# BartvLaatum/GreenLight-Gym2

Hardware: AMD Instinct MI355X
Metric: TomatoEnv env-steps/sec (higher is better)
Workload: dtype f32

## Files before the change

greenlight-gym2_amd/csrc/glgym.hip:

```cpp
#include <hip/hip_runtime.h>

#include <cmath>
#include <cstdio>
#include <cstdlib>
#include <cstring>
#include <new>
#include <string>
#include <vector>

#include "glgym.h"
#include "gl_model.hpp"
#include "gl_model_quad.hpp"
#include "gl_reward.hpp"
#include "glgym_bdf.h"
#include "glgym_rng.h"
#include "glgym_plan.h"

using namespace glm;

namespace {

thread_local std::string g_err;

#define HIPCHK(expr)                                                                                   \
    do {                                                                                               \
        hipError_t e_ = (expr);                                                                        \
        if (e_ != hipSuccess) {                                                                        \
            g_err = std::string(#expr) + ": " + hipGetErrorString(e_);                                 \
            return GLGYM_EHIP;                                                                         \
        }                                                                                              \
    } while (0)

constexpr int WAVE = 64;

#include "gl_default_const.inc"
static_assert(sizeof(ModelConst<float>) == sizeof(kDefaultConstF32_image), "regenerate gl_default_const.inc");
static_assert(sizeof(ModelConst<double>) == sizeof(kDefaultConstF64_image), "regenerate gl_default_const.inc");
template <class T> struct DefaultConst;
template <> struct DefaultConst<float> {
    static constexpr ModelConst<float> value = __builtin_bit_cast(ModelConst<float>, kDefaultConstF32_bits);
};
template <> struct DefaultConst<double> {
    static constexpr ModelConst<double> value = __builtin_bit_cast(ModelConst<double>, kDefaultConstF64_bits);
};
__constant__ const ModelConst<float> g_default_f32 = __builtin_bit_cast(ModelConst<float>, kDefaultConstF32_bits);
__constant__ const ModelConst<double> g_default_f64 = __builtin_bit_cast(ModelConst<double>, kDefaultConstF64_bits);
template <class T> __device__ __forceinline__ const ModelConst<T>& device_default();
template <> __device__ __forceinline__ const ModelConst<float>& device_default<float>() { return g_default_f32; }
template <> __device__ __forceinline__ const ModelConst<double>& device_default<double>() { return g_default_f64; }

template <class T> struct RewardConst : RewardConstBase<T> {};

template <class T> struct StepArgsT {
    int B, ld;
    T* x; T* u;
    const float* action; const T* control;
    const T* weather; int weather_rows;
    const int* w_off; int* timestep;
    const T* crop_p;
    int N;
    T* reward; T* info; unsigned char* done; float* metrics; int* step_flags;
    T dt; int n_sub;
    T gasR, tCanMin;
    int nd;
    float du, u_min[NU], u_max[NU];
    int verify;
    int pipe;
    int window;
};

template <class T> __device__ __forceinline__ T wave_sum(T v)
{
#pragma unroll
    for (int o = 32; o > 0; o >>= 1) v += __shfl_xor(v, o, WAVE);
    return v;
}

#ifndef GL_STEP_WAVES_PER_SIMD
#define GL_STEP_WAVES_PER_SIMD 1
#endif
#ifndef GL_RK4_WIN_F32
#define GL_RK4_WIN_F32 4
#endif
#ifndef GL_RK4_WIN_F64
#define GL_RK4_WIN_F64 4
#endif
template <class T> struct RK4_WINDOW { static constexpr int value = sizeof(T) == 4 ? GL_RK4_WIN_F32 : GL_RK4_WIN_F64; };
constexpr int gl_order(int sch) { return sch == 0 ? 4 : sch == 1 ? 2 : sch == 2 ? 3 : 5; }
template <class T, int SCH> struct SchemeWin { static constexpr int value = SCH == 0 ? RK4_WINDOW<T>::value : SCH == 1 ? 4 : SCH == 2 ? 3 : 2; };

template <class T, bool PER_ENV_CROP, bool DEFAULT_P, bool PIPE = false, int SCH = 0, int OCC = GL_STEP_WAVES_PER_SIMD>
__global__ __launch_bounds__(WAVE, OCC) void step_kernel(StepArgsT<T> a, ModelConst<T> m_arg, RewardConst<T> rw)
{
    const ModelConst<T>& m = DEFAULT_P ? device_default<T>() : m_arg;
    constexpr bool WBUF = OCC == 2;
    constexpr int WSTRIDE = (2 * NX + GL_N_SLOW) | 1;
    __shared__ float sh_w[WBUF ? WAVE * WSTRIDE : WAVE * NU];
    float* sh_act = sh_w;
    const int lane = threadIdx.x;
    const int b0 = blockIdx.x * WAVE;
    const int b = b0 + lane;
    const bool live = b < a.B;
    const int bb = live ? b : a.B - 1;

    T u[NU];
    if (a.action) {
        const int n_tile = min(WAVE, a.B - b0) * NU;
        for (int i = lane; i < n_tile; i += WAVE) sh_act[i] = a.action[(size_t)b0 * NU + i];
        __syncthreads();
        const int l = live ? lane : (a.B - 1 - b0);
#pragma unroll
        for (int j = 0; j < NU; ++j) {
            const float inc = sh_act[l * NU + j] * a.du;
            const T v = a.u[(size_t)j * a.ld + bb] + T(inc);
            u[j] = Math<T>::min(Math<T>::max(v, T(a.u_min[j])), T(a.u_max[j]));
        }
    } else {
#pragma unroll
        for (int j = 0; j < NU; ++j) u[j] = a.control[(size_t)j * a.ld + bb];
    }

    T x0[NX];
#pragma unroll
    for (int i = 0; i < NX; ++i) x0[i] = a.x[(size_t)i * a.ld + bb];
    const int ts = a.timestep[bb];
    int row = a.w_off[bb] + ts;
    row = row < 0 ? 0 : (row >= a.weather_rows ? a.weather_rows - 1 : row);
    T d[7];
#pragma unroll
    for (int j = 0; j < 7; ++j) d[j] = a.weather[(size_t)row * a.nd + j];

    CropConst<T> crLocal;
    if (PER_ENV_CROP) {
        T pc[NCROP];
#pragma unroll
        for (int i = 0; i < NCROP; ++i) pc[i] = a.crop_p[(size_t)i * a.ld + bb];
        make_crop_const<T, T>(pc, a.gasR, a.tCanMin, crLocal);
    }
    const CropConst<T>& cr = PER_ENV_CROP ? crLocal : m.crop;
    StepCoef<T> s_reg;
    precompute(u, d, m, cr, s_reg);
    if (PIPE) {
        const T tPipe = a.weather[(size_t)row * a.nd + 10], swOff = a.weather[(size_t)row * a.nd + 12];
        s_reg.pipeTrack = ((tPipe < T(1)) || (swOff > T(0))) ? T(0) : T(1);
        s_reg.tPipeSet = tPipe;
    }
    const StepCoef<T>& s = s_reg;
    if (live) {
#pragma unroll
        for (int j = 0; j < NU; ++j) a.u[(size_t)j * a.ld + b] = u[j];
    }
    T del_reg[WBUF ? 1 : NX];
    T* wb = reinterpret_cast<T*>(sh_w) + (size_t)lane * WSTRIDE;
    T* del = WBUF ? wb + NX + GL_N_SLOW : del_reg;
    if (WBUF) {
        __syncthreads();
#pragma unroll
        for (int i = 0; i < NX; ++i) wb[i] = x0[i];
        wb[5] = x0[3] - x0[5]; wb[7] = x0[2] - x0[7]; wb[20] = x0[2] - x0[20]; wb[6] = x0[5] - x0[6];
    }
    bool bad;
    int extra_steps, first_flags = 0;
    const int retries = rk4_delta_guarded<T, PIPE, gl_order(SCH), SchemeWin<T, SCH>::value, WBUF>(x0, s, m, cr, a.dt, a.n_sub, del, &bad, &extra_steps, a.verify != 0, &first_flags, a.window, wb);
    const T uBoil = a.u[(size_t)0 * a.ld + bb], uCo2 = a.u[(size_t)1 * a.ld + bb], uLamp = a.u[(size_t)4 * a.ld + bb];
    if (WBUF) {
#pragma unroll
        for (int i = 0; i < NX; ++i) x0[i] = a.x[(size_t)i * a.ld + bb];
    }

    T x1[NX];
#pragma unroll
    for (int i = 0; i < NX; ++i) x1[i] = bad ? x0[i] : x0[i] + del[i];
    {
        const double per_step = (double)a.dt / 86400.0;
        double t_start = (double)x0[NX - 1] - (double)ts * per_step;
        if (fabs(t_start) < 5e-4) t_start = 0.0;
        if (!bad) x1[NX - 1] = T(t_start + ((double)ts + 1.0) * per_step);
    }

    const T co2ppm = rw.kPpm * (x1[2] + T(273.15)) * x1[0];
    const T rh = Math<T>::min(Math<T>::max(T(100) * x1[15] / sat_vp_exact(x1[2]), T(0)), T(100));
    const T o3[3] = {co2ppm, x1[2], rh};
    T viol[3], pen = T(0);
#pragma unroll
    for (int i = 0; i < 3; ++i) {
        viol[i] = Math<T>::max(rw.lo[i] - o3[i], T(0)) + Math<T>::max(o3[i] - rw.hi[i], T(0));
        pen += viol[i] * rw.invMaxViol[i];
    }
    const T heat = uBoil * rw.heatK, elec = uLamp * rw.elecK, co2c = uCo2 * rw.co2K;
    const T varc = heat + co2c + elec;
    const T gains = (bad ? T(0) : del[25]) * rw.gainK;
    const T profit = gains - varc;
    const T reward = (profit - rw.minProfit) * rw.invRange - pen;
    const bool term = bad || (ts >= a.N);

    if (live) {
#pragma unroll
        for (int i = 0; i < NX; ++i) a.x[(size_t)i * a.ld + b] = x1[i];
        a.timestep[b] = ts + 1;
        a.reward[b] = reward;
        a.done[b] = term ? 1 : 0;
        if (a.step_flags) a.step_flags[b] = first_flags | (retries << 8) | (bad ? GLGYM_SF_FAILED : 0) | (min(extra_steps, 32767) << 16);
        if (a.info) {
            const T inf[GLGYM_NINFO] = {profit, gains, varc, rw.fixedCosts, co2c, heat, elec, viol[1], viol[0], viol[2], T(0)};
#pragma unroll
            for (int i = 0; i < GLGYM_NINFO; ++i) a.info[(size_t)i * a.ld + b] = inf[i];
        }
    }
    if (a.metrics) {
        const float w = live ? 1.f : 0.f;
        float mv[GLGYM_NMETRIC] = {w * (float)reward, w * (float)profit, (live && term) ? 1.f : 0.f,
                                   (live && bad) ? 1.f : 0.f, w * (float)viol[0], w * (float)viol[1],
                                   w * (float)viol[2], w, w * (float)retries, w * (float)extra_steps,
                                   (live && (first_flags & SC_FLAG_ERR)) ? 1.f : 0.f, (live && (first_flags & SC_FLAG_BRANCH)) ? 1.f : 0.f,
                                   (live && (first_flags & (SC_FLAG_CAP | SC_FLAG_NONFINITE))) ? 1.f : 0.f,
                                   (live && (first_flags & 16)) ? 1.f : 0.f};
        float* mrep = a.metrics + (size_t)(blockIdx.x % GLGYM_METRIC_REPLICAS) * GLGYM_METRIC_STRIDE;
#pragma unroll
        for (int i = 0; i < GLGYM_NMETRIC; ++i) {
            const float sum = wave_sum(mv[i]);
            if (lane == 0) atomicAdd(mrep + i, sum);
        }
    }
}


template <class T, bool DEFAULT_P, int SCH = 0, bool PIPE = false, bool CROP = false, bool PAIR = false>
__global__ __launch_bounds__(WAVE) void step_kernel_quad(StepArgsT<T> a, ModelConst<T> m_arg, RewardConst<T> rw)
{
    static_assert(!(PAIR && CROP), "the two-rungs ladder is instantiated for shared crop constants only");
    constexpr bool LDSM = sizeof(T) == 8 && !DEFAULT_P;
    __shared__ ModelConst<T> sh_m[1];
    if (LDSM) {
        static_assert(sizeof(ModelConst<T>) % 4 == 0, "word copy");
        const unsigned* src = reinterpret_cast<const unsigned*>(&m_arg);
        unsigned* dst = reinterpret_cast<unsigned*>(&sh_m[0]);
        for (int i = threadIdx.x; i < (int)(sizeof(ModelConst<T>) / 4); i += WAVE) dst[i] = src[i];
        __syncthreads();
    }
    const ModelConst<T>& m = LDSM ? sh_m[0] : DEFAULT_P ? device_default<T>() : m_arg;
    const int gl = blockIdx.x * WAVE + threadIdx.x, role = gl & 3;
    const int b = PAIR ? gl >> 3 : gl >> 2, half = PAIR ? (gl >> 2) & 1 : 0;
    const bool live = b < a.B;
    const int bb = live ? b : a.B - 1;
    T u[NU];
    if (a.action) {
#pragma unroll
        for (int j = 0; j < NU; ++j) {
            const float inc = a.action[(size_t)bb * NU + j] * a.du;
            const T v = a.u[(size_t)j * a.ld + bb] + T(inc);
            u[j] = Math<T>::min(Math<T>::max(v, T(a.u_min[j])), T(a.u_max[j]));
        }
    } else {
#pragma unroll
        for (int j = 0; j < NU; ++j) u[j] = a.control[(size_t)j * a.ld + bb];
    }
    const int ts = a.timestep[bb];
    int row = a.w_off[bb] + ts;
    row = row < 0 ? 0 : (row >= a.weather_rows ? a.weather_rows - 1 : row);
    T d[7];
#pragma unroll
    for (int j = 0; j < 7; ++j) d[j] = a.weather[(size_t)row * a.nd + j];
    constexpr bool LDSQ = sizeof(T) == 8;
    struct SRec { StepCoef<T> s; T pad[(sizeof(StepCoef<T>) / sizeof(T)) % 2 == 0 ? 1 : 2]; };
    struct KRec { LaneK<T> k; T pad[(sizeof(LaneK<T>) / sizeof(T)) % 2 == 0 ? 1 : 2]; };
    struct CRec { CropConst<T> c; T pad[(sizeof(CropConst<T>) / sizeof(T)) % 2 == 0 ? 1 : 2]; };
    __shared__ SRec sh_s[LDSQ ? WAVE / 4 : 1];
    __shared__ KRec sh_k[LDSQ ? WAVE : 1];
    __shared__ CRec sh_c[(LDSQ && CROP) ? WAVE / 4 : 1];
    StepCoef<T> s_reg;
    LaneK<T> k_reg;
    CropConst<T> cr_reg;
    if (CROP && (!LDSQ || role == 0)) {
        T pc[NCROP];
#pragma unroll
        for (int i = 0; i < NCROP; ++i) pc[i] = a.crop_p[(size_t)i * a.ld + bb];
        make_crop_const<T, T>(pc, a.gasR, a.tCanMin, cr_reg);
    }
    if (!LDSQ || role == 0) {
        precompute(u, d, m, CROP ? cr_reg : m.crop, s_reg);
        if (PIPE && a.pipe) {
            const T tPipe = a.weather[(size_t)row * a.nd + 10], swOff = a.weather[(size_t)row * a.nd + 12];
            s_reg.pipeTrack = ((tPipe < T(1)) || (swOff > T(0))) ? T(0) : T(1);
            s_reg.tPipeSet = tPipe;
            s_reg.pipeOde = T(1);
        }
    }
    if (LDSQ) {
        if (role == 0) { sh_s[threadIdx.x >> 2].s = s_reg; if (CROP) sh_c[threadIdx.x >> 2].c = cr_reg; }
        __syncthreads();
    }
    const CropConst<T>& cr = !CROP ? m.crop : LDSQ ? sh_c[threadIdx.x >> 2].c : cr_reg;
    const StepCoef<T>& s = LDSQ ? sh_s[threadIdx.x >> 2].s : s_reg;
    LaneK<T>& K = LDSQ ? sh_k[threadIdx.x].k : k_reg;
    auto X = [&](int i) { return a.x[(size_t)i * a.ld + bb]; };
    QVec<T> x0, z0, del;
#pragma unroll
    for (int i = 0; i < 6; ++i) x0.sh[i] = X(role == 0 ? gq_sh_ix(i) : role == 1 ? gq_sh_ix(i) : role == 2 ? gq_sh_ix(i) : gq_sh_ix(i));
    x0.p = gq_mk<T>(X(role == 0 ? 4 : role == 1 ? 8 : role == 2 ? 7 : 5), X(role == 0 ? 9 : role == 1 ? 17 : role == 2 ? 20 : 6));
#pragma unroll
    for (int j = 0; j < 4; ++j) {
        const int ix = role == 0 ? gq_other_ix(0, j) : role == 1 ? gq_other_ix(1, j) : role == 2 ? gq_other_ix(2, j) : gq_other_ix(3, j < 2 ? j : 1);
        x0.o[j] = X(ix);
    }
    z0 = x0;
    z0.p = gq_mk<T>(role == 2 ? x0.sh[2] - x0.p.x : role == 3 ? x0.sh[3] - x0.p.x : x0.p.x,
                    role == 2 ? x0.sh[2] - x0.p.y : role == 3 ? x0.p.x - x0.p.y : x0.p.y);
    if (live && role == 0 && half == 0) {
#pragma unroll
        for (int j = 0; j < NU; ++j) a.u[(size_t)j * a.ld + b] = u[j];
    }
    bool bad;
    int extra_steps = 0, first_flags = 0, retries = 0, mine = 1;
    constexpr bool HVU = sizeof(T) == 8 || DEFAULT_P;
    if (PAIR) {
        int bad_i;
        rk4_delta_guarded_quad_pair<T, gl_order(SCH), SchemeWin<T, SCH>::value, LDSQ, PIPE, false, true, HVU>(role, half, z0, s, K, m, cr, a.dt, a.n_sub, del, &bad_i, &mine,
                                                                                                         a.window, &retries, &extra_steps, &first_flags);
        asm volatile("" : "+v"(bad_i), "+v"(mine));
        bad = bad_i != 0;
    } else {
        retries = rk4_delta_guarded_quad<T, gl_order(SCH), SchemeWin<T, SCH>::value, LDSQ, PIPE, LDSQ && CROP, HVU>(role, z0, s, K, m, cr, a.dt, a.n_sub, del, &bad,
                                                                                                    &extra_steps, a.verify != 0, &first_flags, a.window);
    }
    P2<T> dP;
    gq_phys_pair<T>(role, del, dP);
    asm volatile("" ::: "memory");
    int gl2 = blockIdx.x * WAVE + threadIdx.x;
    asm volatile("" : "+v"(gl2));
    const int role2 = gl2 & 3, b2 = PAIR ? gl2 >> 3 : gl2 >> 2;
    const bool live2 = b2 < a.B && mine != 0;
    const int bb2 = (b2 < a.B) ? b2 : a.B - 1;
    const int ts2 = a.timestep[bb2];
    auto X2 = [&](int i) { return a.x[(size_t)i * a.ld + bb2]; };
#pragma unroll
    for (int i = 0; i < 6; ++i) x0.sh[i] = X2(gq_sh_ix(i));
    x0.p = gq_mk<T>(X2(role2 == 0 ? 4 : role2 == 1 ? 8 : role2 == 2 ? 7 : 5), X2(role2 == 0 ? 9 : role2 == 1 ? 17 : role2 == 2 ? 20 : 6));
#pragma unroll
    for (int j = 0; j < 4; ++j) {
        const int ix = role2 == 0 ? gq_other_ix(0, j) : role2 == 1 ? gq_other_ix(1, j) : role2 == 2 ? gq_other_ix(2, j) : gq_other_ix(3, j < 2 ? j : 1);
        x0.o[j] = X2(ix);
    }
#pragma unroll
    for (int j = 0; j < NU; ++j) u[j] = a.u[(size_t)j * a.ld + bb2];
    QVec<T> x1;
    x1.p = gq_mk<T>(bad ? x0.p.x : x0.p.x + dP.x, bad ? x0.p.y : x0.p.y + dP.y);
#pragma unroll
    for (int i = 0; i < 6; ++i) x1.sh[i] = bad ? x0.sh[i] : x0.sh[i] + del.sh[i];
#pragma unroll
    for (int j = 0; j < 4; ++j) x1.o[j] = bad ? x0.o[j] : x0.o[j] + del.o[j];
    if (role2 == 3) {
        const double per_step = (double)a.dt / 86400.0;
        double t_start = (double)x0.o[1] - (double)ts2 * per_step;
        if (fabs(t_start) < 5e-4) t_start = 0.0;
        if (!bad) x1.o[1] = T(t_start + ((double)ts2 + 1.0) * per_step);
    }
    const T dFruit = gq_bcast<2>(del.o[3]);
    const T co2ppm = rw.kPpm * (x1.sh[2] + T(273.15)) * x1.sh[0];
    const T rh = Math<T>::min(Math<T>::max(T(100) * x1.sh[4] / sat_vp_exact(x1.sh[2]), T(0)), T(100));
    const T o3[3] = {co2ppm, x1.sh[2], rh};
    T viol[3], pen = T(0);
#pragma unroll
    for (int i = 0; i < 3; ++i) {
        viol[i] = Math<T>::max(rw.lo[i] - o3[i], T(0)) + Math<T>::max(o3[i] - rw.hi[i], T(0));
        pen += viol[i] * rw.invMaxViol[i];
    }
    const T heat = u[0] * rw.heatK, elec = u[4] * rw.elecK, co2c = u[1] * rw.co2K;
    const T varc = heat + co2c + elec;
    const T gains = (bad ? T(0) : dFruit) * rw.gainK;
    const T profit = gains - varc;
    const T reward = (profit - rw.minProfit) * rw.invRange - pen;
    const bool term = bad || (ts2 >= a.N);
    if (live2) {
        auto W = [&](int i, T v) { a.x[(size_t)i * a.ld + b2] = v; };
        W(role2 == 0 ? 4 : role2 == 1 ? 8 : role2 == 2 ? 7 : 5, x1.p.x);
        W(role2 == 0 ? 9 : role2 == 1 ? 17 : role2 == 2 ? 20 : 6, x1.p.y);
#pragma unroll
        for (int j = 0; j < 4; ++j)
            if (role2 != 3 || j < 2) W(role2 == 0 ? gq_other_ix(0, j) : role2 == 1 ? gq_other_ix(1, j) : role2 == 2 ? gq_other_ix(2, j) : gq_other_ix(3, j < 2 ? j : 1), x1.o[j]);
        if (role2 == 0) {
#pragma unroll
            for (int i = 0; i < 6; ++i) W(gq_sh_ix(i), x1.sh[i]);
            a.timestep[b2] = ts2 + 1;
            a.reward[b2] = reward;
            a.done[b2] = term ? 1 : 0;
            if (a.step_flags) a.step_flags[b2] = first_flags | (retries << 8) | (bad ? GLGYM_SF_FAILED : 0) | (min(extra_steps, 32767) << 16);
            if (a.info) {
                const T inf[GLGYM_NINFO] = {profit, gains, varc, rw.fixedCosts, co2c, heat, elec, viol[1], viol[0], viol[2], T(0)};
#pragma unroll
                for (int i = 0; i < GLGYM_NINFO; ++i) a.info[(size_t)i * a.ld + b2] = inf[i];
            }
        }
    }
    if (a.metrics) {
        const bool cnt = live2 && role2 == 0;
        const float w = cnt ? 1.f : 0.f;
        float mv[GLGYM_NMETRIC] = {w * (float)reward, w * (float)profit, (cnt && term) ? 1.f : 0.f,
                                   (cnt && bad) ? 1.f : 0.f, w * (float)viol[0], w * (float)viol[1],
                                   w * (float)viol[2], w, w * (float)retries, w * (float)extra_steps,
                                   (cnt && (first_flags & SC_FLAG_ERR)) ? 1.f : 0.f, (cnt && (first_flags & SC_FLAG_BRANCH)) ? 1.f : 0.f,
                                   (cnt && (first_flags & (SC_FLAG_CAP | SC_FLAG_NONFINITE))) ? 1.f : 0.f,
                                   (cnt && (first_flags & 16)) ? 1.f : 0.f};
        float* mrep = a.metrics + (size_t)(blockIdx.x % GLGYM_METRIC_REPLICAS) * GLGYM_METRIC_STRIDE;
#pragma unroll
        for (int i = 0; i < GLGYM_NMETRIC; ++i) {
            const float sum = wave_sum(mv[i]);
            if (threadIdx.x == 0) atomicAdd(mrep + i, sum);
        }
    }
}

template <class T, int SCH, bool PIPE, bool CROP, bool PAIR = false>
__global__ __launch_bounds__(WAVE) void evalf_kernel_quad(const double* x, const double* u, const double* d, const double* crop, int B, T dt,
                                                          int n_sub, T gasR, T tCanMin, ModelConst<T> m_arg, double* x_next, int nd,
                                                          int* n_failed, int verify, int pipe, int window)
{
    constexpr bool LDSM = sizeof(T) == 8;
    __shared__ ModelConst<T> sh_m[1];
    if (LDSM) {
        const unsigned* src = reinterpret_cast<const unsigned*>(&m_arg);
        unsigned* dst = reinterpret_cast<unsigned*>(&sh_m[0]);
        for (int i = threadIdx.x; i < (int)(sizeof(ModelConst<T>) / 4); i += WAVE) dst[i] = src[i];
        __syncthreads();
    }
    const ModelConst<T>& m = LDSM ? sh_m[0] : m_arg;
    const int gl = blockIdx.x * WAVE + threadIdx.x, role = gl & 3, b = PAIR ? gl >> 3 : gl >> 2, half = PAIR ? (gl >> 2) & 1 : 0;
    const bool live = b < B;
    const int bb = live ? b : B - 1;
    T uu[NU], dd[7];
#pragma unroll
    for (int i = 0; i < NU; ++i) uu[i] = T(u[(size_t)bb * NU + i]);
#pragma unroll
    for (int i = 0; i < 7; ++i) dd[i] = T(d[(size_t)bb * nd + i]);
    constexpr bool LDSQ = sizeof(T) == 8;
    struct SRec { StepCoef<T> s; T pad[(sizeof(StepCoef<T>) / sizeof(T)) % 2 == 0 ? 1 : 2]; };
    struct KRec { LaneK<T> k; T pad[(sizeof(LaneK<T>) / sizeof(T)) % 2 == 0 ? 1 : 2]; };
    struct CRec { CropConst<T> c; T pad[(sizeof(CropConst<T>) / sizeof(T)) % 2 == 0 ? 1 : 2]; };
    __shared__ SRec sh_s[LDSQ ? WAVE / 4 : 1];
    __shared__ KRec sh_k[LDSQ ? WAVE : 1];
    __shared__ CRec sh_c[(LDSQ && CROP) ? WAVE / 4 : 1];
    StepCoef<T> s_reg;
    LaneK<T> k_reg;
    CropConst<T> cr_reg;
    if (CROP && (!LDSQ || role == 0)) {
        T pc[NCROP];
#pragma unroll
        for (int i = 0; i < NCROP; ++i) pc[i] = T(crop[(size_t)bb * NCROP + i]);
        make_crop_const<T, T>(pc, gasR, tCanMin, cr_reg);
    }
    if (!LDSQ || role == 0) {
        precompute(uu, dd, m, CROP ? cr_reg : m.crop, s_reg);
        if (PIPE && pipe) {
            const T tPipe = T(d[(size_t)bb * nd + 10]), swOff = T(d[(size_t)bb * nd + 12]);
            s_reg.pipeTrack = ((tPipe < T(1)) || (swOff > T(0))) ? T(0) : T(1);
            s_reg.tPipeSet = tPipe;
            s_reg.pipeOde = T(1);
        }
    }
    if (LDSQ) {
        if (role == 0) { sh_s[threadIdx.x >> 2].s = s_reg; if (CROP) sh_c[threadIdx.x >> 2].c = cr_reg; }
        __syncthreads();
    }
    const CropConst<T>& cr = !CROP ? m.crop : LDSQ ? sh_c[threadIdx.x >> 2].c : cr_reg;
    const StepCoef<T>& s = LDSQ ? sh_s[threadIdx.x >> 2].s : s_reg;
    LaneK<T>& K = LDSQ ? sh_k[threadIdx.x].k : k_reg;
    auto X = [&](int i) { return T(x[(size_t)bb * NX + i]); };
    QVec<T> x0, z0, del;
#pragma unroll
    for (int i = 0; i < 6; ++i) x0.sh[i] = X(gq_sh_ix(i));
    x0.p = gq_mk<T>(X(role == 0 ? 4 : role == 1 ? 8 : role == 2 ? 7 : 5), X(role == 0 ? 9 : role == 1 ? 17 : role == 2 ? 20 : 6));
#pragma unroll
    for (int j = 0; j < 4; ++j)
        x0.o[j] = X(role == 0 ? gq_other_ix(0, j) : role == 1 ? gq_other_ix(1, j) : role == 2 ? gq_other_ix(2, j) : gq_other_ix(3, j < 2 ? j : 1));
    z0 = x0;
    z0.p = gq_mk<T>(role == 2 ? x0.sh[2] - x0.p.x : role == 3 ? x0.sh[3] - x0.p.x : x0.p.x,
                    role == 2 ? x0.sh[2] - x0.p.y : role == 3 ? x0.p.x - x0.p.y : x0.p.y);
    bool bad;
    constexpr bool HVU = sizeof(T) == 8;
    int mine = 1;
    if (PAIR) {
        int bad_i;
        rk4_delta_guarded_quad_pair<T, gl_order(SCH), SchemeWin<T, SCH>::value, LDSQ, PIPE, LDSQ && CROP, false, HVU>(role, half, z0, s, K, m, cr, dt, n_sub, del, &bad_i, &mine, window);
        asm volatile("" : "+v"(bad_i), "+v"(mine));
        bad = bad_i != 0;
    } else {
        int extra_steps, first_flags = 0;
        rk4_delta_guarded_quad<T, gl_order(SCH), SchemeWin<T, SCH>::value, LDSQ, PIPE, LDSQ && CROP, HVU>(role, z0, s, K, m, cr, dt, n_sub, del, &bad, &extra_steps, verify != 0,
                                                                                      &first_flags, window);
    }
    P2<T> dP;
    gq_phys_pair<T>(role, del, dP);
    asm volatile("" ::: "memory");
    int gl2 = blockIdx.x * WAVE + threadIdx.x;
    asm volatile("" : "+v"(gl2));
    const int role2 = gl2 & 3, b2 = PAIR ? gl2 >> 3 : gl2 >> 2;
    if (b2 < B && mine != 0) {
        const double nan = __builtin_nan("");
        auto X2 = [&](int i) { return x[(size_t)b2 * NX + i]; };
        auto W = [&](int i, T dv) { x_next[(size_t)b2 * NX + i] = bad ? nan : X2(i) + (double)dv; };
        W(role2 == 0 ? 4 : role2 == 1 ? 8 : role2 == 2 ? 7 : 5, dP.x);
        W(role2 == 0 ? 9 : role2 == 1 ? 17 : role2 == 2 ? 20 : 6, dP.y);
#pragma unroll
        for (int j = 0; j < 4; ++j)
            if (role2 != 3 || j < 2)
                W(role2 == 0 ? gq_other_ix(0, j) : role2 == 1 ? gq_other_ix(1, j) : role2 == 2 ? gq_other_ix(2, j) : gq_other_ix(3, j < 2 ? j : 1), del.o[j]);
        if (role2 == 0) {
#pragma unroll
            for (int i = 0; i < 6; ++i) W(gq_sh_ix(i), del.sh[i]);
            if (bad) atomicAdd(n_failed, 1);
        }
    }
}

template <class T, bool PER_ENV_CROP, bool PIPE>
__global__ __launch_bounds__(WAVE) void rhs_kernel(const double* x, const double* u, const double* d, const double* crop, int B, T gasR,
                                                   T tCanMin, ModelConst<T> m, double* dx, int nd)
{
    const int b = blockIdx.x * WAVE + threadIdx.x;
    if (b >= B) return;
    T x0[NX], uu[NU], dd[7];
    for (int i = 0; i < NX; ++i) x0[i] = T(x[(size_t)b * NX + i]);
    for (int i = 0; i < NU; ++i) uu[i] = T(u[(size_t)b * NU + i]);
    for (int i = 0; i < 7; ++i) dd[i] = T(d[(size_t)b * nd + i]);
    CropConst<T> crLocal;
    if (PER_ENV_CROP) {
        T pc[NCROP];
        for (int i = 0; i < NCROP; ++i) pc[i] = T(crop[(size_t)b * NCROP + i]);
        make_crop_const<T, T>(pc, gasR, tCanMin, crLocal);
    }
    const CropConst<T>& cr = PER_ENV_CROP ? crLocal : m.crop;
    StepCoef<T> s;
    precompute(uu, dd, m, cr, s);
    if (PIPE) {
        const T tPipe = T(d[(size_t)b * nd + 10]), swOff = T(d[(size_t)b * nd + 12]);
        s.pipeTrack = ((tPipe < T(1)) || (swOff > T(0))) ? T(0) : T(1);
        s.tPipeSet = tPipe;
    }
    T k[NX];
    rhs<T, true, PIPE>(x0, s, m, cr, k);
    for (int i = 0; i < NX; ++i) dx[(size_t)b * NX + i] = (double)k[i];
}

template <class T, bool PER_ENV_CROP, bool PIPE = false, int SCH = 0>
__global__ __launch_bounds__(WAVE) void evalf_kernel(const double* x, const double* u, const double* d,
                                                     const double* crop, int B, T dt, int n_sub, T gasR, T tCanMin,
                                                     ModelConst<T> m, double* x_next, int rhs_only, int nd,
                                                     int* n_failed, int verify, int window)
{
    const int b = blockIdx.x * WAVE + threadIdx.x;
    if (b >= B) return;
    T x0[NX], uu[NU], dd[7];
    for (int i = 0; i < NX; ++i) x0[i] = T(x[(size_t)b * NX + i]);
    for (int i = 0; i < NU; ++i) uu[i] = T(u[(size_t)b * NU + i]);
    for (int i = 0; i < 7; ++i) dd[i] = T(d[(size_t)b * nd + i]);
    CropConst<T> crLocal;
    if (PER_ENV_CROP) {
        T pc[NCROP];
        for (int i = 0; i < NCROP; ++i) pc[i] = T(crop[(size_t)b * NCROP + i]);
        make_crop_const<T, T>(pc, gasR, tCanMin, crLocal);
    }
    const CropConst<T>& cr = PER_ENV_CROP ? crLocal : m.crop;
    StepCoef<T> s;
    precompute(uu, dd, m, cr, s);
    if (PIPE) {
        const T tPipe = T(d[(size_t)b * nd + 10]), swOff = T(d[(size_t)b * nd + 12]);
        s.pipeTrack = ((tPipe < T(1)) || (swOff > T(0))) ? T(0) : T(1);
        s.tPipeSet = tPipe;
    }
    if (rhs_only) {
        T k[NX];
        rhs<T, true, PIPE>(x0, s, m, cr, k);
        for (int i = 0; i < NX; ++i) x_next[(size_t)b * NX + i] = (double)k[i];
        return;
    }
    T del[NX];
    bool failed;
    rk4_delta_guarded<T, PIPE, gl_order(SCH), SchemeWin<T, SCH>::value>(x0, s, m, cr, dt, n_sub, del, &failed, nullptr, verify != 0, nullptr, window);
    for (int i = 0; i < NX; ++i)
        x_next[(size_t)b * NX + i] = failed ? __builtin_nan("") : (double)x0[i] + (double)del[i];
    if (failed) atomicAdd(n_failed, 1);
}

template <class T> struct ObsArgsT {
    int B, ld;
    const T* x; const T* u; const T* weather; int weather_rows;
    const int* w_off; const int* timestep; const float* start_day;
    int Np; float* obs; double doy_inc, hod_inc;
    const unsigned char* mask; float* term_obs;
    int nd;
    int moff[6], dim;
};

#ifndef GL_OBS_ROWS
#define GL_OBS_ROWS 16
#endif
constexpr int OBS_ROWS = GL_OBS_ROWS, OBS_NCORE = 23, OBS_MAX_NP = 128;
template <class T> __global__ __launch_bounds__(256) void obs_kernel(ObsArgsT<T> a)
{
    constexpr int ROWS = OBS_ROWS, NCORE = OBS_NCORE;
    extern __shared__ float4 span4[];
    float* span = reinterpret_cast<float*>(span4);
    const int tid = threadIdx.x;
    const int dim = a.dim;
    const float kPpm = (float)(8.3144598 / (101325.0 * 44.01e-3));
    for (int rb = blockIdx.x * ROWS; rb < a.B; rb += gridDim.x * ROWS) {
        const int nrows = min(ROWS, a.B - rb);
        if (a.mask) {
            int any = 0;
            for (int r = 0; r < nrows; ++r) any |= a.mask[rb + r];
            if (!any) continue;
        }
        int base_r[ROWS];
#pragma unroll
        for (int r = 0; r < ROWS; ++r) {
            const int b = rb + (r < nrows ? r : 0);
            const int ts = a.timestep[b];
            base_r[r] = a.w_off[b] + (ts > 0 ? ts - 1 : 0);
        }
        for (int e = tid; e < ROWS * NCORE; e += 256) {
            const int r = e / NCORE, j = e - r * NCORE;
            const int b = rb + (r < nrows ? r : 0);
            const int ts = a.timestep[b];
            const int k = ts > 0 ? ts - 1 : 0;
            int base = 0;
#pragma unroll
            for (int rr = 0; rr < ROWS; ++rr) base = (rr == r) ? base_r[rr] : base;
            base = base >= a.weather_rows ? a.weather_rows - 1 : (base < 0 ? 0 : base);
            const T* wrow = a.weather + (size_t)base * a.nd;
            const int xi = j == 0 ? 0 : j == 1 ? 2 : j == 2 ? 15 : j == 3 ? 9 : j == 4 ? 21 : j == 5 ? 25 : 26;
            const T* p1 = j < 7 ? a.x + (size_t)xi * a.ld + b
                                : (j < 13 ? a.u + (size_t)(j - 7) * a.ld + b : wrow + (j < 18 ? j - 13 : 0));
            const T* p2 = j < 13 ? a.x + (size_t)2 * a.ld + b : wrow + 1;
            const float prim = (float)*p1, aux = (float)*p2, sday = a.start_day[b];
            const float sat = 610.78f * __builtin_amdgcn_exp2f(1.44269504f * 17.2694f * aux * __builtin_amdgcn_rcpf(aux + 238.3f));
            const float rh = fminf(fmaxf(100.0f * prim * __builtin_amdgcn_rcpf(sat), 0.0f), 100.0f);
            const float ppm = kPpm * (aux + 273.15f) * prim;
            const int c = j - 18;
            const double rev = (c <= 2) ? ((double)sday + (double)ts * a.doy_inc) * (1.0 / 365.0)
                                        : (double)ts * a.hod_inc * (1.0 / 24.0);
            const float fr = (float)(rev - floor(rev));
            const float clk = (c == 1 || c == 3) ? __builtin_amdgcn_sinf(fr) : __builtin_amdgcn_cosf(fr);
            float v = prim;
            v = (j == 0 || j == 16) ? ppm : v;
            v = (j == 2 || j == 15) ? rh : v;
            v = (j == 18) ? (float)k : v;
            v = (j > 18) ? clk : v;
            const int mo = j < 4 ? a.moff[0] : j < 7 ? a.moff[1] : j < 13 ? a.moff[2] : j < 18 ? a.moff[3] : a.moff[4];
            const int jl = j < 4 ? j : j < 7 ? j - 4 : j < 13 ? j - 7 : j < 18 ? j - 13 : j - 18;
            if (r < nrows && mo >= 0) span[r * dim + mo + jl] = v;
        }
        const int nf = a.moff[5] >= 0 ? 5 * a.Np : 0;
        for (int q = tid; q < nf; q += 256) {
            const int i = q / 5, c = q - i * 5;
            float v[ROWS];
#pragma unroll
            for (int r = 0; r < ROWS; ++r) {
                int row = base_r[r] + 1 + i;
                row = row >= a.weather_rows ? a.weather_rows - 1 : (row < 0 ? 0 : row);
                v[r] = (float)a.weather[(size_t)row * a.nd + c];
            }
#pragma unroll
            for (int r = 0; r < ROWS; ++r)
                if (r < nrows) span[r * dim + a.moff[5] + q] = v[r];
        }
        __syncthreads();
        float* out = a.obs + (size_t)rb * dim;
        if (!a.mask && nrows == ROWS) {
            const int n4 = (ROWS * dim) >> 2;
            float4* out4 = reinterpret_cast<float4*>(out);
            typedef float v4f __attribute__((ext_vector_type(4)));
            const v4f* src4 = reinterpret_cast<const v4f*>(span4);
            v4f* dst4 = reinterpret_cast<v4f*>(out4);
            for (int e = tid; e < n4; e += 256) __builtin_nontemporal_store(src4[e], &dst4[e]);
        } else {
            for (int r = 0; r < nrows; ++r) {
                if (a.mask && !a.mask[rb + r]) continue;
                for (int jj = tid; jj < dim; jj += 256) {
                    const size_t e = (size_t)r * dim + jj;
                    if (a.mask && a.term_obs) a.term_obs[(size_t)rb * dim + e] = out[e];
                    out[e] = span[e];
                }
            }
        }
        __syncthreads();
    }
}

template <class T>
__global__ __launch_bounds__(256) void rule_based_kernel(glgym_rule_cfg c, int B, int ld, const T* __restrict__ x,
                                                         const T* __restrict__ weather, int weather_rows,
                                                         const int* __restrict__ w_off, const int* __restrict__ timestep,
                                                         const float* __restrict__ start_day, const double* hour,
                                                         const double* doy_in, double doy_inc, double hod_inc,
                                                         T* __restrict__ control, int nd)
{
    const int b = blockIdx.x * blockDim.x + threadIdx.x;
    if (b >= B) return;
    const int ts = timestep[b];
    int row = w_off[b] + ts;
    row = row >= weather_rows ? weather_rows - 1 : (row < 0 ? 0 : row);
    const T* w = weather + (size_t)row * nd;
    const double iGlob = (double)w[0], tOut = (double)w[1], dli = (double)w[7], isDay = (double)w[8],
                 isDaySmooth = (double)w[9];
    const double co2Air = (double)x[b], tAir = (double)x[(size_t)2 * ld + b], vpAir = (double)x[(size_t)15 * ld + b];
    const double hod = hour ? hour[b] : fmod((double)ts * hod_inc, 24.0);
    const double doy = doy_in ? doy_in[b] : (double)start_day[b] + (double)ts * doy_inc;
    auto pband = [](double v, double sp, double band, double lo, double hi) {
        return lo + (hi - lo) * (1.0 / (1.0 + exp(-2.0 / band * 4.605170185988092 * (v - sp - band * 0.5))));
    };
    const double tod = c.lamps_on <= c.lamps_off ? (double)(c.lamps_on < hod && hod < c.lamps_off)
                                                 : (double)(c.lamps_on < hod || hod < c.lamps_off);
    const double doy_ok = c.lamps_day_start <= c.lamps_day_stop
                              ? (double)(c.lamps_day_start < doy && doy < c.lamps_day_stop)
                              : (double)(c.lamps_day_start < doy || doy < c.lamps_day_stop);
    const double below_dli = (double)(dli < c.lamp_rad_sum_limit);
    const double lamp_no_cons = (double)(iGlob < c.lamps_off_sun) * below_dli * tod * doy_ok;
    const double sw_on = fmax(0.0, fmin(1.0, hod - c.lamps_on + 1.0));
    const double sw_off = fmax(0.0, fmin(1.0, c.lamps_off - hod + 1.0));
    const double both = c.lamps_on == c.lamps_off ? 0.0
                        : (c.lamps_on < c.lamps_off ? fmin(sw_on, sw_off) : fmax(sw_on, sw_off));
    const double smooth_lamp = both * below_dli * doy_ok;
    const double day_inside = fmax(smooth_lamp, isDay);
    const double heat_sp = day_inside * c.temp_setpoint_day + (1.0 - day_inside) * c.temp_setpoint_night +
                           c.heat_correction * lamp_no_cons;
    const double heat_max = heat_sp + c.heat_deadzone;
    const double co2_sp = day_inside * c.co2_day;
    const double co2_ppm = 1e6 * 8.3144598 * (tAir + 273.15) * (1e-6 * co2Air) / (101325.0 * 44.01e-3);
    const double rh_in = 100.0 * vpAir / (610.78 * exp(17.2694 * tAir / (tAir + 238.3)));
    const double vent_heat = pband(tAir, heat_max, c.vent_heat_Pband, 0, 1);
    const double vent_rh = pband(rh_in, c.rh_max + 0.0 * c.mech_dehumid_Pband, c.vent_rh_Pband, 0, 1);
    const double vent_cold = pband(tAir, heat_sp - c.t_vent_off, c.vent_cold_Pband, 1, 0);
    const double th_sp = isDay * c.thScrSpDay + (1.0 - isDay) * c.thScrSpNight;
    const double th_cold = pband(tOut, th_sp, c.thScrPband, 0, 1);
    const double th_heat = pband(tAir, heat_sp + c.thScrDeadZone, -c.thScrPband, 1, 0);
    const double th_rh = fmax(pband(rh_in, c.rhMax + c.thScrRh, c.thScrRhPband, 1, 0), 1.0 - vent_cold);
    const double lamp_on = lamp_no_cons * pband(tAir, heat_max + c.lampExtraHeat, -0.5, 0, 1) *
                           (isDaySmooth + (1.0 - isDaySmooth)) *
                           fmax(pband(rh_in, c.rhMax + c.blScrExtraRh, -0.5, 0, 1), 1.0 - vent_cold);
    control[b] = (T)pband(tAir, heat_sp, c.tHeatBand, 0, 1);
    control[(size_t)1 * ld + b] = (T)pband(co2_ppm, co2_sp, c.co2Band, 0, 1);
    control[(size_t)2 * ld + b] = (T)fmin(th_cold, fmax(th_heat, th_rh));
    control[(size_t)3 * ld + b] = (T)fmin(vent_cold, fmax(vent_heat, vent_rh));
    control[(size_t)4 * ld + b] = (T)lamp_on;
    control[(size_t)5 * ld + b] = (T)(c.useBlScr * (1.0 - isDaySmooth) * lamp_on);
}

__device__ __forceinline__ void philox4x32_10(unsigned c0, unsigned c1, unsigned c2, unsigned c3, unsigned k0,
                                              unsigned k1, unsigned* out)
{
#pragma unroll
    for (int r = 0; r < 10; ++r) {
        const unsigned long long p0 = 0xD2511F53ull * c0, p1 = 0xCD9E8D57ull * c2;
        const unsigned n0 = (unsigned)(p1 >> 32) ^ c1 ^ k0, n1 = (unsigned)p1;
        const unsigned n2 = (unsigned)(p0 >> 32) ^ c3 ^ k1, n3 = (unsigned)p0;
        c0 = n0; c1 = n1; c2 = n2; c3 = n3;
        k0 += 0x9E3779B9u; k1 += 0xBB67AE85u;
    }
    out[0] = c0; out[1] = c1; out[2] = c2; out[3] = c3;
}


template <class T>
__global__ void reset_kernel(int B, int ld, const unsigned char* mask, T* x, T* u, int* timestep, const T* weather,
                             int weather_rows, int* w_off, const int* start_rows, const float* start_days, int n_starts,
                             float* start_day, int* episode, unsigned long long seed, int nd)
{
    const int b = blockIdx.x * blockDim.x + threadIdx.x;
    if (b >= B || (mask && !mask[b])) return;
    if (start_rows && n_starts > 0) {
        const int ep = episode ? episode[b] : 0;
        unsigned rnd[4];
        philox4x32_10((unsigned)b, (unsigned)ep, 0x5eedu, 0u, (unsigned)seed, (unsigned)(seed >> 32), rnd);
        const int j = (int)(rnd[0] % (unsigned)n_starts);
        w_off[b] = start_rows[j];
        if (start_day && start_days) start_day[b] = start_days[j];
        if (episode) episode[b] = ep + 1;
    }
    int r = w_off[b];
    r = r < 0 ? 0 : (r >= weather_rows ? weather_rows - 1 : r);
    const double co2Out = (double)weather[(size_t)r * nd + 3], tSoOut = (double)weather[(size_t)r * nd + 6];
    const double tAir = 16.5;
    double xi[NX];
    xi[0] = xi[1] = co2Out;
    for (int i = 2; i <= 10; ++i) xi[i] = tAir;
    xi[4] = tAir + 4;
    xi[11] = 0.25 * (3.0 * tAir + tSoOut);
    xi[12] = 0.25 * (2.0 * tAir + 2 * tSoOut);
    xi[13] = 0.25 * (tAir + 3 * tSoOut);
    xi[14] = tSoOut;
    xi[15] = xi[16] = 90.0 / 100.0 * (610.78 * exp(17.2694 * tAir / (tAir + 238.3)));
    xi[17] = xi[18] = xi[19] = xi[20] = tAir;
    xi[21] = xi[4];
    xi[22] = 0.0; xi[23] = 9.5283e4; xi[24] = 2.5107e5; xi[25] = 5.5338e4; xi[26] = 3.0978e3; xi[27] = 0.0;
    for (int i = 0; i < NX; ++i) x[(size_t)i * ld + b] = T(xi[i]);
    for (int j = 0; j < NU; ++j) u[(size_t)j * ld + b] = T(0);
    timestep[b] = 0;
}

template <class T>
__global__ void crop_noise_kernel(T* crop_p, int B, int ld, const float* p0, float scale, unsigned long long seed,
                                  unsigned long long draw)
{
    const int b = blockIdx.x * blockDim.x + threadIdx.x;
    if (b >= B) return;
    float pn[NCROP + 2];
    for (int blk = 0; blk < 9; ++blk) {
        unsigned r[4];
        philox4x32_10((unsigned)b, (unsigned)draw, (unsigned)(draw >> 32), (unsigned)blk, (unsigned)seed,
                      (unsigned)(seed >> 32), r);
        for (int q = 0; q < 4; ++q) {
            const int i = blk * 4 + q;
            if (i < NCROP) {
                const float un = ((float)(r[q] >> 8) + 0.5f) * (1.0f / 16777216.0f);
                const float noise = (un - 0.5f) * scale;
                pn[i] = p0[i] + noise * p0[i];
            }
        }
    }
    pn[144 - CROP0] = pn[141 - CROP0] / pn[142 - CROP0];
    for (int i = 0; i < NCROP; ++i) crop_p[(size_t)i * ld + b] = T(pn[i]);
}


constexpr int VN_REP = 16;
__global__ __launch_bounds__(1024) void vecnorm_moments_kernel(const float* __restrict__ obs, int B, int dim,
                                                               double* __restrict__ acc_all)
{
    double* acc = acc_all + (size_t)(blockIdx.x % VN_REP) * 2 * dim;
    const int rows_per_block = (B + gridDim.x - 1) / gridDim.x;
    const int r0 = blockIdx.x * rows_per_block, r1 = min(B, r0 + rows_per_block);
    for (int c = threadIdx.x; c < dim; c += blockDim.x) {
        double s0 = 0.0, q0 = 0.0, s1 = 0.0, q1 = 0.0;
        int r = r0;
        for (; r + 7 < r1; r += 8) {
            float v[8];
#pragma unroll
            for (int j = 0; j < 8; ++j) v[j] = obs[(size_t)(r + j) * dim + c];
#pragma unroll
            for (int j = 0; j < 8; j += 2) {
                const double a = (double)v[j], b = (double)v[j + 1];
                s0 += a; q0 += a * a; s1 += b; q1 += b * b;
            }
        }
        for (; r < r1; ++r) { const double v = (double)obs[(size_t)r * dim + c]; s0 += v; q0 += v * v; }
        if (r1 > r0) { atomicAdd(acc + c, s0 + s1); atomicAdd(acc + dim + c, q0 + q1); }
    }
}

template <class T>
__global__ __launch_bounds__(256) void vecnorm_returns_kernel(const T* __restrict__ reward, double* __restrict__ returns,
                                                              int B, double gamma, double* __restrict__ acc2)
{
    const int b = blockIdx.x * blockDim.x + threadIdx.x;
    double v = 0.0;
    if (b < B) { v = returns[b] * gamma + (double)reward[b]; returns[b] = v; }
    double s = v, q = v * v;
#pragma unroll
    for (int o = 32; o > 0; o >>= 1) { s += __shfl_xor(s, o, WAVE); q += __shfl_xor(q, o, WAVE); }
    __shared__ double part[2][4];
    const int wv = threadIdx.x / WAVE;
    if ((threadIdx.x & (WAVE - 1)) == 0) { part[0][wv] = s; part[1][wv] = q; }
    __syncthreads();
    if (threadIdx.x == 0) {
        atomicAdd(acc2, part[0][0] + part[0][1] + part[0][2] + part[0][3]);
        atomicAdd(acc2 + 1, part[1][0] + part[1][1] + part[1][2] + part[1][3]);
    }
}

__global__ __launch_bounds__(1024) void vecnorm_merge_kernel(double* mean, double* var, double* count, const double* acc, int dim,
                                                            int B, double* ret_stats, const double* acc2, int do_obs,
                                                            int do_ret, double eps, double* scale)
{
    const double n = (double)B;
    const double cnt = *count;
    for (int c = threadIdx.x; c < dim; c += blockDim.x) {
        if (do_obs) {
            double sum = 0.0, sq = 0.0;
            for (int r = 0; r < VN_REP; ++r) { sum += acc[(size_t)r * 2 * dim + c]; sq += acc[(size_t)r * 2 * dim + dim + c]; }
            const double bm = sum / n, bv = fmax(sq / n - bm * bm, 0.0);
            const double tot = cnt + n, delta = bm - mean[c];
            const double m2 = var[c] * cnt + bv * n + delta * delta * cnt * n / tot;
            mean[c] += delta * n / tot;
            var[c] = m2 / tot;
        }
        if (scale) scale[c] = 1.0 / sqrt(var[c] + eps);
    }
    if (do_ret && threadIdx.x == 0) {
        const double bm = acc2[0] / n, bv = fmax(acc2[1] / n - bm * bm, 0.0);
        const double rc = ret_stats[2], tot = rc + n, delta = bm - ret_stats[0];
        const double m2 = ret_stats[1] * rc + bv * n + delta * delta * rc * n / tot;
        ret_stats[0] += delta * n / tot;
        ret_stats[1] = m2 / tot;
        ret_stats[2] = tot;
    }
    __syncthreads();
    if (do_obs && threadIdx.x == 0) *count = cnt + n;
}

__global__ __launch_bounds__(1024) void vecnorm_apply_kernel(const float* __restrict__ obs, float* __restrict__ out,
                                                            int B, int dim, const double* __restrict__ mean,
                                                            const double* __restrict__ scale, float clip)
{
    const int rows_per_block = (B + gridDim.x - 1) / gridDim.x;
    const int r0 = blockIdx.x * rows_per_block, r1 = min(B, r0 + rows_per_block);
    for (int c = threadIdx.x; c < dim; c += blockDim.x) {
        const double mu = mean[c], sc = scale[c];
        for (int r = r0; r < r1; ++r) {
            const size_t i = (size_t)r * dim + c;
            const float v = (float)(((double)obs[i] - mu) * sc);
            out[i] = fminf(fmaxf(v, -clip), clip);
        }
    }
}

template <class T>
__global__ void vecnorm_reward_kernel(const T* __restrict__ reward, float* __restrict__ out, double* __restrict__ returns,
                                      const unsigned char* __restrict__ done, int B, const double* ret_stats, double eps,
                                      float clip, int norm_reward)
{
    const int b = blockIdx.x * blockDim.x + threadIdx.x;
    if (b >= B) return;
    float r = (float)reward[b];
    if (norm_reward) r = fminf(fmaxf((float)((double)reward[b] / sqrt(ret_stats[1] + eps)), -clip), clip);
    out[b] = r;
    if (done && done[b]) returns[b] = 0.0;
}


__device__ __forceinline__ double w_sat_vp(double t) { return 610.78 * exp(17.2694 * t / (t + 238.3)); }

__global__ void weather_convert_kernel(int n, const double* __restrict__ time, const double* __restrict__ i_glob,
                                       const double* __restrict__ t_out, const double* __restrict__ rh,
                                       const double* __restrict__ wind, const double* __restrict__ t_sky, double co2_ppm,
                                       double* __restrict__ W)
{
    const int k = blockIdx.x * blockDim.x + threadIdx.x;
    if (k >= n) return;
    const double R = 8.3144598, C2K = 273.15, M_CO2 = 44.01e-3, M_H2O = 18.01528e-3, P_ATM = 101325.0;
    const double t = t_out[k];
    const double rho_v = (rh[k] / 100.0) * w_sat_vp(t) * M_H2O / (R * (t + C2K));
    const double rho_sat = (100.0 / 100.0) * w_sat_vp(t) * M_H2O / (R * (t + C2K));
    W[0 * (size_t)n + k] = i_glob[k];
    W[1 * (size_t)n + k] = t;
    W[2 * (size_t)n + k] = w_sat_vp(t) * (rho_v / rho_sat);
    W[3 * (size_t)n + k] = (P_ATM * 1e-6 * co2_ppm * M_CO2 / (R * (t + C2K))) * 1e6;
    W[4 * (size_t)n + k] = wind[k];
    W[5 * (size_t)n + k] = t_sky[k];
    const double year = 3600.0 * 24.0 * 365.0;
    W[6 * (size_t)n + k] = 10.0 + 5.0 * sin(2.0 * 3.14159265358979323846 * (time[k] + 0.625 * year) / year);
}

__global__ void weather_scan_kernel(int n, const double* __restrict__ time, double* __restrict__ W)
{
    if (blockIdx.x != 0 || threadIdx.x != 0 || n < 2) return;
    const double* rad = W;
    double* dli = W + 7 * (size_t)n;
    double* is_day = W + 8 * (size_t)n;
    double* smooth = W + 9 * (size_t)n;
    const double c = 86400.0, interval = time[1] - time[0];
    auto next_jump = [&](int from) {
        for (int k = from < 0 ? 0 : from; k + 1 < n; ++k)
            if (floor(time[k + 1] / c) - floor(time[k] / c) == 1.0) return k;
        return -1;
    };
    int before = 0, j = next_jump(0), after = j >= 0 ? j + 1 : n, i = 0;
    while (i < n) {
        const int seg_end = after < n ? after : n;
        double sum = 0.0;
        for (int k = before; k <= after && k < n; ++k) sum += rad[k];
        for (int k = i; k < seg_end; ++k) dli[k] = sum * interval * 1e-6;
        i = seg_end;
        if (i >= n) break;
        before = after;
        j = next_jump(before + 2);
        after = j >= 0 ? j : n;
    }
    double dt_mean = (time[n - 1] - time[0]) / (double)(n - 1);
    for (int k = 0; k < n; ++k) { is_day[k] = rad[k] > 0.0 ? 1.0 : 0.0; smooth[k] = is_day[k]; }
    const int n_tr = (int)(3600.0 / dt_mean), half = n_tr / 2;
    if (n_tr < 2) return;
    const double step = 1.0 / (double)(n_tr - 1);
    bool in_sunset = false;
    for (int k = n_tr; k < n - n_tr; ++k) {
        const double cur = is_day[k], nxt = is_day[k + 1];
        if (cur == 0.0) {
            in_sunset = false;
            if (nxt == 1.0)
                for (int q = 0; q < 2 * half && q < n_tr; ++q) {
                    const double r = (q == n_tr - 1) ? 1.0 : (double)q * step;
                    is_day[k - half + q] = r;
                    smooth[k - half + q] = 1.0 / (1.0 + exp(-10.0 * (r - 0.5)));
                }
        } else if (cur == 1.0 && nxt == 0.0 && !in_sunset) {
            for (int q = 0; q < 2 * half && q < n_tr; ++q) {
                const double r = (q == n_tr - 1) ? 1.0 : (double)q * step;
                is_day[k - half + q] = 1.0 - r;
                smooth[k - half + q] = 1.0 - 1.0 / (1.0 + exp(-10.0 * (r - 0.5)));
            }
            in_sunset = true;
        }
    }
}

__device__ __forceinline__ double w_sign(double v) { return v > 0.0 ? 1.0 : (v < 0.0 ? -1.0 : 0.0); }
__device__ __forceinline__ double pchip_edge(double h0, double h1, double m0, double m1)
{
    double d = ((2.0 * h0 + h1) * m0 - h0 * m1) / (h0 + h1);
    if (w_sign(d) != w_sign(m0)) d = 0.0;
    else if (w_sign(m0) != w_sign(m1) && fabs(d) > 3.0 * fabs(m0)) d = 3.0 * m0;
    return d;
}
__global__ void pchip_slopes_kernel(int n, int n_col, const double* __restrict__ x, const double* __restrict__ W,
                                    double* __restrict__ D)
{
    const int k = blockIdx.x * blockDim.x + threadIdx.x, col = blockIdx.y;
    if (k >= n || col >= n_col) return;
    const double* y = W + (size_t)col * n;
    auto h = [&](int i) { return x[i + 1] - x[i]; };
    auto m = [&](int i) { return (y[i + 1] - y[i]) / h(i); };
    double d;
    if (n == 2) d = m(0);
    else if (k == 0) d = pchip_edge(h(0), h(1), m(0), m(1));
    else if (k == n - 1) d = pchip_edge(h(n - 2), h(n - 3), m(n - 2), m(n - 3));
    else {
        const double m0 = m(k - 1), m1 = m(k), h0 = h(k - 1), h1 = h(k);
        if (w_sign(m0) != w_sign(m1) || m0 == 0.0 || m1 == 0.0) d = 0.0;
        else {
            const double w1 = 2.0 * h1 + h0, w2 = h1 + 2.0 * h0;
            d = 1.0 / ((w1 / m0 + w2 / m1) / (w1 + w2));
        }
    }
    D[(size_t)col * n + k] = d;
}

template <class T>
__global__ void pchip_eval_kernel(int n, int n_col, int n_out, int nd, const double* __restrict__ x,
                                  const double* __restrict__ W, const double* __restrict__ D, T* __restrict__ out)
{
    const int i = blockIdx.x * blockDim.x + threadIdx.x, col = blockIdx.y;
    if (i >= n_out || col >= n_col) return;
    const double start = x[0], stop = x[n - 1];
    const double stepo = n_out > 1 ? (stop - start) / (double)(n_out - 1) : 0.0;
    const double t = (i == n_out - 1 && n_out > 1) ? stop : (double)i * stepo + start;
    int lo = 0, hi = n - 1;
    while (hi - lo > 1) { const int mid = (lo + hi) >> 1; if (x[mid] <= t) lo = mid; else hi = mid; }
    const int k = lo > n - 2 ? n - 2 : lo;
    const double* y = W + (size_t)col * n;
    const double* d = D + (size_t)col * n;
    const double dx = x[k + 1] - x[k], slope = (y[k + 1] - y[k]) / dx;
    const double tt = (d[k] + d[k + 1] - 2.0 * slope) / dx;
    const double c0 = tt / dx, c1 = (slope - d[k]) / dx - tt, c2 = d[k], c3 = y[k];
    const double sdx = t - x[k];
    double res = 0.0, z = 1.0;
    res += c3 * z; z *= sdx;
    res += c2 * z; z *= sdx;
    res += c1 * z; z *= sdx;
    res += c0 * z;
    if (col == 0 && res < 1e-10) res = 0.0;
    out[(size_t)i * nd + col] = T(res);
}

}

struct glgym_handle_s {
    int device = 0;
    int dtype = GLGYM_F32;
    int n_sub = 256;
    double dt = 900.0;
    double p[NP];
    ModelConst<float> mf;
    ModelConst<double> md;
    glgym_reward_cfg rcfg;
    RewardConst<float> rf;
    RewardConst<double> rd;
    double max_profit = 0, min_profit = 0, fixed_costs = 0;
    float* p0_crop_dev = nullptr;
    int* fail_dev = nullptr;
    int nd = ND;
    int variant = GLGYM_ODE;
    int scheme = GLGYM_SCHEME_RK4;
    int verify_mode = GLGYM_VERIFY_AUTO;
    int use_specialised = 1;
    int window = 0;
    int layout = GLGYM_LAYOUT_AUTO;
    int occupancy = 0;
    int ladder_parallel = 1;
    int n_simd = 1024;
    float du = 0.1f, u_min[NU] = {0, 0, 0, 0, 0, 0}, u_max[NU] = {1, 1, 1, 1, 1, 1};
    int obs_modules[6] = {0, 1, 2, 3, 4, 5};
    int n_obs_modules = 6;
    hipEvent_t ev0 = nullptr, ev1 = nullptr;
    int integrator = GLGYM_INTEGRATOR_EXPLICIT;
    int step_integrator = GLGYM_INTEGRATOR_EXPLICIT;
    double rtol = 1e-6, atol = 1e-6;
    int max_steps = 10000;
    int32_t* stats_dev = nullptr;
    int stats_cap = 0;
    std::vector<int32_t> stats;
    int stats_rows = 0;
    double* scratch = nullptr;
    size_t scratch_elems = 0;
};

static void default_reward(glgym_reward_cfg& c)
{
    c.elec_price = 0.3; c.heating_price = 0.09; c.co2_price = 0.3; c.fruit_price = 1.6; c.dmfm = 0.065;
    c.fixed_greenhouse_cost = 15.0; c.fixed_co2_cost = 0.015; c.fixed_lamp_cost = 0.07; c.fixed_screen_cost = 2.0;
    c.pen_lamp = 0.1;
    c.co2_min = 300; c.co2_max = 1600; c.temp_min = 15; c.temp_max = 34; c.rh_min = 50; c.rh_max = 85;
}

static int refresh(glgym_handle h)
{
    std::memset(&h->mf, 0, sizeof h->mf);
    std::memset(&h->md, 0, sizeof h->md);
    make_model_const<float>(h->p, h->mf);
    make_model_const<double>(h->p, h->md);
    make_reward_const<float>(h->p, h->dt, h->rcfg, h->rf, &h->max_profit, &h->min_profit, &h->fixed_costs);
    make_reward_const<double>(h->p, h->dt, h->rcfg, h->rd, nullptr, nullptr, nullptr);
    float pc[NCROP];
    for (int i = 0; i < NCROP; ++i) pc[i] = (float)h->p[CROP0 + i];
    HIPCHK(hipMemcpy(h->p0_crop_dev, pc, sizeof pc, hipMemcpyHostToDevice));
    return GLGYM_OK;
}

struct DeviceGuard {
    int prev = -1;
    bool switched = false;
    explicit DeviceGuard(const glgym_handle_s* h)
    {
        if (h && hipGetDevice(&prev) == hipSuccess && prev != h->device) switched = hipSetDevice(h->device) == hipSuccess;
    }
    ~DeviceGuard() { if (switched) (void)hipSetDevice(prev); }
    DeviceGuard(const DeviceGuard&) = delete;
    DeviceGuard& operator=(const DeviceGuard&) = delete;
};

extern "C" {

#define GLGYM_STR_(v) #v
#define GLGYM_STR(v) GLGYM_STR_(v)
const char* glgym_version(void)
{
    return "glgym 0.7 (gfx950; ABI " GLGYM_STR(GLGYM_ABI_VERSION) "; stability-controlled, step-doubling-verified sub-steppers in delta form: "
           "five-stage fourth-order 2N scheme / RK4 / RK3 / midpoint; adaptive variable-order BDF for glgym_evalF)";
}
int glgym_abi_version(void) { return GLGYM_ABI_VERSION; }
const char* glgym_last_error(void) { return g_err.c_str(); }

int glgym_destroy(glgym_handle h);

int glgym_create(int nx, int nu, int nd, int np, double dt, const double* p, int dtype, int n_sub, int device,
                 glgym_handle* out)
{
    if (!out || !p || nx != NX || nu != NU || nd < ND || nd > 16 || np != NP || !(dt > 0) || n_sub < 1 ||
        (dtype != GLGYM_F32 && dtype != GLGYM_F64)) {
        g_err = "glgym_create: expected nx=28 nu=6 nd=10..16 np=208, dt>0, n_sub>=1, dtype in {F32,F64}";
        return GLGYM_EINVAL;
    }
    int n_dev = 0;
    if (hipGetDeviceCount(&n_dev) != hipSuccess || n_dev <= 0 || device < 0 || device >= n_dev) {
        g_err = "glgym_create: no usable HIP device (this library has no CPU fallback)";
        return GLGYM_ENODEV;
    }
    HIPCHK(hipSetDevice(device));
    glgym_handle h = new (std::nothrow) glgym_handle_s();
    if (!h) return GLGYM_ENOMEM;
    {
        hipDeviceProp_t prop;
        if (hipGetDeviceProperties(&prop, device) == hipSuccess && prop.multiProcessorCount > 0)
            h->n_simd = 4 * prop.multiProcessorCount;
    }
    h->device = device; h->dtype = dtype; h->n_sub = n_sub; h->dt = dt; h->nd = nd;
    std::memcpy(h->p, p, sizeof h->p);
    default_reward(h->rcfg);
    if (const char* e = std::getenv("GLGYM_GENERIC")) h->use_specialised = (e[0] == '1') ? 0 : 1;
    if (const char* e = std::getenv("GLGYM_VERIFY"))
        h->verify_mode = (e[0] == 'n') ? GLGYM_VERIFY_NEVER : (e[0] == 'a' && e[1] == 'l') ? GLGYM_VERIFY_ALWAYS : GLGYM_VERIFY_AUTO;
    if (const char* e = std::getenv("GLGYM_LAYOUT")) h->layout = (e[0] == 'q') ? GLGYM_LAYOUT_QUAD : (e[0] == 'o') ? GLGYM_LAYOUT_ONE : GLGYM_LAYOUT_AUTO;
    if (const char* e = std::getenv("GLGYM_OCC")) h->occupancy = (std::atoi(e) == 2) ? 2 : (std::atoi(e) == 1) ? 1 : 0;
    int rc = [&]() -> int {
        HIPCHK(hipMalloc(&h->p0_crop_dev, NCROP * sizeof(float)));
        HIPCHK(hipMalloc(&h->fail_dev, sizeof(int)));
        HIPCHK(hipEventCreate(&h->ev0));
        HIPCHK(hipEventCreate(&h->ev1));
        return refresh(h);
    }();
    if (rc != GLGYM_OK) {
        const std::string keep = g_err;
        (void)glgym_destroy(h);
        g_err = keep;
        return rc;
    }
    *out = h;
    return GLGYM_OK;
}

int glgym_destroy(glgym_handle h)
{
    if (!h) return GLGYM_EINVAL;
    (void)hipSetDevice(h->device);
    if (h->p0_crop_dev) (void)hipFree(h->p0_crop_dev);
    if (h->fail_dev) (void)hipFree(h->fail_dev);
    if (h->scratch) (void)hipFree(h->scratch);
    if (h->stats_dev) (void)hipFree(h->stats_dev);
    if (h->ev0) (void)hipEventDestroy(h->ev0);
    if (h->ev1) (void)hipEventDestroy(h->ev1);
    delete h;
    return GLGYM_OK;
}

int glgym_set_params(glgym_handle h, const double* p)
{
    if (!h || !p) return GLGYM_EINVAL;
    std::memcpy(h->p, p, sizeof h->p);
    return refresh(h);
}

int glgym_set_params_keep_reward_scale(glgym_handle h, const double* p)
{
    if (!h || !p) return GLGYM_EINVAL;
    const float minf = h->rf.minProfit, invf = h->rf.invRange;
    const double mind = h->rd.minProfit, invd = h->rd.invRange, maxp = h->max_profit, minp = h->min_profit;
    std::memcpy(h->p, p, sizeof h->p);
    const int rc = refresh(h);
    h->rf.minProfit = minf; h->rf.invRange = invf;
    h->rd.minProfit = mind; h->rd.invRange = invd;
    h->max_profit = maxp; h->min_profit = minp;
    return rc;
}

int glgym_set_model_variant(glgym_handle h, int variant)
{
    if (!h || (variant != GLGYM_ODE && variant != GLGYM_ODE_PIPE) || (variant == GLGYM_ODE_PIPE && h->nd < 14)) {
        g_err = "glgym_set_model_variant: GLGYM_ODE or GLGYM_ODE_PIPE (the latter needs a handle created with nd >= 14)";
        return GLGYM_EINVAL;
    }
    h->variant = variant;
    return GLGYM_OK;
}

int glgym_set_scheme(glgym_handle h, int scheme)
{
    if (!h || (scheme != GLGYM_SCHEME_RK4 && scheme != GLGYM_SCHEME_RK2 && scheme != GLGYM_SCHEME_RK3 && scheme != GLGYM_SCHEME_LS5)) {
        g_err = "glgym_set_scheme: GLGYM_SCHEME_RK4, GLGYM_SCHEME_RK2, GLGYM_SCHEME_RK3 or GLGYM_SCHEME_LS5";
        return GLGYM_EINVAL;
    }
    h->scheme = scheme;
    return GLGYM_OK;
}

int glgym_set_window(glgym_handle h, int window)
{
    if (!h || window < 0 || window > 8) { g_err = "glgym_set_window: 0 (the scheme's own) or 1..8 nominal sub-steps per window"; return GLGYM_EINVAL; }
    h->window = window;
    return GLGYM_OK;
}

int glgym_set_layout(glgym_handle h, int layout)
{
    if (!h || (layout != GLGYM_LAYOUT_AUTO && layout != GLGYM_LAYOUT_ONE && layout != GLGYM_LAYOUT_QUAD)) {
        g_err = "glgym_set_layout: GLGYM_LAYOUT_AUTO, GLGYM_LAYOUT_ONE or GLGYM_LAYOUT_QUAD";
        return GLGYM_EINVAL;
    }
    h->layout = layout;
    return GLGYM_OK;
}

int glgym_set_occupancy(glgym_handle h, int waves_per_simd)
{
    if (!h || waves_per_simd < 0 || waves_per_simd > 2) { g_err = "glgym_set_occupancy: 0 (by batch size), 1 or 2 waves per SIMD"; return GLGYM_EINVAL; }
    h->occupancy = waves_per_simd;
    return GLGYM_OK;
}

int glgym_set_ladder_parallel(glgym_handle h, int on)
{
    if (!h || (on != 0 && on != 1)) { g_err = "glgym_set_ladder_parallel: 0 or 1"; return GLGYM_EINVAL; }
    h->ladder_parallel = on;
    return GLGYM_OK;
}

int glgym_set_control_limits(glgym_handle h, const double* u_min, const double* u_max, double delta_u_max)
{
    if (!h || !u_min || !u_max || !(delta_u_max >= 0)) { g_err = "glgym_set_control_limits: bad arguments"; return GLGYM_EINVAL; }
    for (int j = 0; j < NU; ++j)
        if (!(u_min[j] <= u_max[j])) { g_err = "glgym_set_control_limits: u_min > u_max"; return GLGYM_EINVAL; }
    for (int j = 0; j < NU; ++j) { h->u_min[j] = (float)u_min[j]; h->u_max[j] = (float)u_max[j]; }
    h->du = (float)delta_u_max;
    return GLGYM_OK;
}

int glgym_set_integrator(glgym_handle h, int integrator)
{
    if (!h || (integrator != GLGYM_INTEGRATOR_EXPLICIT && integrator != GLGYM_INTEGRATOR_BDF)) {
        g_err = "glgym_set_integrator: GLGYM_INTEGRATOR_EXPLICIT or GLGYM_INTEGRATOR_BDF";
        return GLGYM_EINVAL;
    }
    h->integrator = integrator;
    return GLGYM_OK;
}

int glgym_set_step_integrator(glgym_handle h, int integrator)
{
    if (!h || (integrator != GLGYM_INTEGRATOR_EXPLICIT && integrator != GLGYM_INTEGRATOR_BDF)) {
        g_err = "glgym_set_step_integrator: GLGYM_INTEGRATOR_EXPLICIT or GLGYM_INTEGRATOR_BDF";
        return GLGYM_EINVAL;
    }
    h->step_integrator = integrator;
    return GLGYM_OK;
}

int glgym_set_tolerances(glgym_handle h, double rtol, double atol, int max_steps)
{
    if (!h || !(rtol > 0.0) || !(atol > 0.0) || !std::isfinite(rtol) || !std::isfinite(atol) || max_steps < 1) {
        g_err = "glgym_set_tolerances: rtol > 0, atol > 0 (finite), max_steps >= 1";
        return GLGYM_EINVAL;
    }
    h->rtol = rtol; h->atol = atol; h->max_steps = max_steps;
    return GLGYM_OK;
}

int glgym_get_solver_stats(glgym_handle h, int B, int32_t* stats)
{
    if (!h || !stats || B < 1 || B != h->stats_rows) {
        g_err = "glgym_get_solver_stats: B must be the batch size of the last glgym_evalF with GLGYM_INTEGRATOR_BDF";
        return GLGYM_EINVAL;
    }
    std::memcpy(stats, h->stats.data(), (size_t)B * GLGYM_NSOLVER_STAT * sizeof(int32_t));
    return GLGYM_OK;
}

int glgym_set_verify(glgym_handle h, int mode)
{
    if (!h || (mode != GLGYM_VERIFY_AUTO && mode != GLGYM_VERIFY_ALWAYS && mode != GLGYM_VERIFY_NEVER)) {
        g_err = "glgym_set_verify: GLGYM_VERIFY_AUTO, GLGYM_VERIFY_ALWAYS or GLGYM_VERIFY_NEVER";
        return GLGYM_EINVAL;
    }
    h->verify_mode = mode;
    return GLGYM_OK;
}

int glgym_set_n_sub(glgym_handle h, int n_sub)
{
    if (!h || n_sub < 1) return GLGYM_EINVAL;
    h->n_sub = n_sub;
    return GLGYM_OK;
}

int glgym_set_reward(glgym_handle h, const glgym_reward_cfg* cfg)
{
    if (!h || !cfg) return GLGYM_EINVAL;
    h->rcfg = *cfg;
    return refresh(h);
}

int glgym_get_reward_scale(glgym_handle h, double* max_profit, double* min_profit, double* fixed_costs)
{
    if (!h) return GLGYM_EINVAL;
    if (max_profit) *max_profit = h->max_profit;
    if (min_profit) *min_profit = h->min_profit;
    if (fixed_costs) *fixed_costs = h->fixed_costs;
    return GLGYM_OK;
}

}

static int ensure_scratch(glgym_handle h, size_t elems)
{
    if (h->scratch_elems >= elems) return GLGYM_OK;
    if (h->scratch) (void)hipFree(h->scratch);
    h->scratch = nullptr; h->scratch_elems = 0;
    HIPCHK(hipMalloc(&h->scratch, elems * sizeof(double)));
    h->scratch_elems = elems;
    return GLGYM_OK;
}

template <class T, int SCH>
static void launch_evalf_sch(glgym_handle h, const ModelConst<T>& m, const double* p_used, const double* dx, const double* du,
                             const double* dd, const double* dcrop, int B, double* dout, dim3 grid, dim3 block)
{
    const int verify = h->verify_mode != GLGYM_VERIFY_NEVER;
    const bool pair = verify && h->ladder_parallel && !dcrop && (size_t)8 * B <= (size_t)WAVE * h->n_simd &&
                      (sizeof(T) == 8 || h->layout != GLGYM_LAYOUT_ONE);
    if constexpr (sizeof(T) == 8) {
        const dim3 qgrid((4 * B + WAVE - 1) / WAVE), pgrid((8 * B + WAVE - 1) / WAVE);
        const int pipe = h->variant == GLGYM_ODE_PIPE ? 1 : 0;
        if (pair) hipLaunchKernelGGL((evalf_kernel_quad<T, SCH, true, false, true>), pgrid, block, 0, (hipStream_t)0, dx, du, dd, dcrop, B, T(h->dt), h->n_sub,
                                     T(p_used[39]), T(p_used[162]), m, dout, h->nd, h->fail_dev, verify, pipe, h->window);
        else if (dcrop) hipLaunchKernelGGL((evalf_kernel_quad<T, SCH, true, true>), qgrid, block, 0, (hipStream_t)0, dx, du, dd, dcrop, B, T(h->dt), h->n_sub,
                                      T(p_used[39]), T(p_used[162]), m, dout, h->nd, h->fail_dev, verify, pipe, h->window);
        else hipLaunchKernelGGL((evalf_kernel_quad<T, SCH, true, false>), qgrid, block, 0, (hipStream_t)0, dx, du, dd, dcrop, B, T(h->dt), h->n_sub,
                                T(p_used[39]), T(p_used[162]), m, dout, h->nd, h->fail_dev, verify, pipe, h->window);
    } else {
        const dim3 pgrid((8 * B + WAVE - 1) / WAVE);
        if (pair) hipLaunchKernelGGL((evalf_kernel_quad<T, SCH, false, false, true>), pgrid, block, 0, (hipStream_t)0, dx, du, dd, dcrop, B, T(h->dt), h->n_sub,
                                     T(p_used[39]), T(p_used[162]), m, dout, h->nd, h->fail_dev, verify, 0, h->window);
        else if (!dcrop && (h->layout == GLGYM_LAYOUT_QUAD || (h->layout == GLGYM_LAYOUT_AUTO && B <= 4 * h->n_simd * 4)))
            hipLaunchKernelGGL((evalf_kernel_quad<T, SCH, false, false, false>), dim3((4 * B + WAVE - 1) / WAVE), block, 0, (hipStream_t)0, dx, du, dd, dcrop, B,
                               T(h->dt), h->n_sub, T(p_used[39]), T(p_used[162]), m, dout, h->nd, h->fail_dev, verify, 0, h->window);
        else if (dcrop) hipLaunchKernelGGL((evalf_kernel<T, true, false, SCH>), grid, block, 0, (hipStream_t)0, dx, du, dd, dcrop, B, T(h->dt), h->n_sub,
                                      T(p_used[39]), T(p_used[162]), m, dout, 0, h->nd, h->fail_dev, verify, h->window);
        else hipLaunchKernelGGL((evalf_kernel<T, false, false, SCH>), grid, block, 0, (hipStream_t)0, dx, du, dd, dcrop, B, T(h->dt), h->n_sub,
                                T(p_used[39]), T(p_used[162]), m, dout, 0, h->nd, h->fail_dev, verify, h->window);
    }
}

template <class T>
static int run_evalf(glgym_handle h, const ModelConst<T>& m, const double* p_used, const double* dx, const double* du,
                     const double* dd, const double* dcrop, int B, double* dout, int rhs_only)
{
    const dim3 grid((B + WAVE - 1) / WAVE), block(WAVE);
    const bool pipe = h->variant == GLGYM_ODE_PIPE;
    if (rhs_only) {
        if (pipe) hipLaunchKernelGGL((rhs_kernel<T, false, true>), grid, block, 0, (hipStream_t)0, dx, du, dd, dcrop, B, T(p_used[39]), T(p_used[162]), m, dout, h->nd);
        else if (dcrop) hipLaunchKernelGGL((rhs_kernel<T, true, false>), grid, block, 0, (hipStream_t)0, dx, du, dd, dcrop, B, T(p_used[39]), T(p_used[162]), m, dout, h->nd);
        else hipLaunchKernelGGL((rhs_kernel<T, false, false>), grid, block, 0, (hipStream_t)0, dx, du, dd, dcrop, B, T(p_used[39]), T(p_used[162]), m, dout, h->nd);
        HIPCHK(hipGetLastError());
        return GLGYM_OK;
    }
    if (pipe) {
        if (dcrop || h->scheme != GLGYM_SCHEME_RK4) {
            g_err = "glgym_evalF: GLGYM_ODE_PIPE supports neither per-row parameter blocks nor schemes other than GLGYM_SCHEME_RK4";
            return GLGYM_EINVAL;
        }
        if constexpr (sizeof(T) == 8) {
            launch_evalf_sch<T, GLGYM_SCHEME_RK4>(h, m, p_used, dx, du, dd, dcrop, B, dout, grid, block);
        } else {
            const int verify = h->verify_mode != GLGYM_VERIFY_NEVER;
            hipLaunchKernelGGL((evalf_kernel<T, false, true>), grid, block, 0, (hipStream_t)0, dx, du, dd, dcrop, B, T(h->dt), h->n_sub,
                               T(p_used[39]), T(p_used[162]), m, dout, 0, h->nd, h->fail_dev, verify, h->window);
        }
    } else if (h->scheme == GLGYM_SCHEME_RK2) {
        launch_evalf_sch<T, GLGYM_SCHEME_RK2>(h, m, p_used, dx, du, dd, dcrop, B, dout, grid, block);
    } else if (h->scheme == GLGYM_SCHEME_RK3) {
        launch_evalf_sch<T, GLGYM_SCHEME_RK3>(h, m, p_used, dx, du, dd, dcrop, B, dout, grid, block);
    } else if (h->scheme == GLGYM_SCHEME_LS5) {
        launch_evalf_sch<T, GLGYM_SCHEME_LS5>(h, m, p_used, dx, du, dd, dcrop, B, dout, grid, block);
    } else {
        launch_evalf_sch<T, GLGYM_SCHEME_RK4>(h, m, p_used, dx, du, dd, dcrop, B, dout, grid, block);
    }
    HIPCHK(hipGetLastError());
    return GLGYM_OK;
}

static int evalf_impl(glgym_handle h, const double* x, const double* u, const double* d, const double* p, int p_rows,
                      int B, double* out, int rhs_only)
{
    if (!h || !x || !u || !d || !out || B < 1 || (p && p_rows != 1 && p_rows != B)) {
        g_err = "glgym_evalF: bad arguments";
        return GLGYM_EINVAL;
    }
    HIPCHK(hipSetDevice(h->device));
    const bool bdf = !rhs_only && h->integrator == GLGYM_INTEGRATOR_BDF;
    if (bdf && h->variant == GLGYM_ODE_PIPE) {
        g_err = "glgym_evalF: GLGYM_INTEGRATOR_BDF does not support GLGYM_ODE_PIPE";
        return GLGYM_EINVAL;
    }
    const double* p_used = p ? p : h->p;
    bool per_row = p && p_rows == B && B > 1;
    if (per_row) {
        for (int b = 1; b < B && per_row; ++b)
            for (int i = 0; i < NP; ++i)
                if ((i < CROP0 || i >= CROP0 + NCROP) && p[(size_t)b * NP + i] != p[i]) {
                    std::vector<int32_t> st(bdf ? (size_t)B * GLGYM_NSOLVER_STAT : 0);
                    for (int r = 0; r < B; ++r) {
                        const int rc = evalf_impl(h, x + (size_t)r * NX, u + (size_t)r * NU, d + (size_t)r * h->nd,
                                                  p + (size_t)r * NP, 1, 1, out + (size_t)r * NX, rhs_only);
                        if (bdf && h->stats_rows == 1)
                            std::memcpy(&st[(size_t)r * GLGYM_NSOLVER_STAT], h->stats.data(), sizeof(int32_t) * GLGYM_NSOLVER_STAT);
                        if (rc != GLGYM_OK) return rc;
                    }
                    if (bdf) { h->stats = st; h->stats_rows = B; }
                    return GLGYM_OK;
                }
    }
    const size_t n_in = (size_t)B * (NX + NU + h->nd + (per_row ? NCROP : 0));
    int rc = ensure_scratch(h, n_in + (size_t)B * NX);
    if (rc != GLGYM_OK) return rc;
    double* dx = h->scratch; double* du = dx + (size_t)B * NX; double* dd = du + (size_t)B * NU;
    double* dcrop = per_row ? dd + (size_t)B * h->nd : nullptr;
    double* dout = h->scratch + n_in;
    HIPCHK(hipMemcpy(dx, x, (size_t)B * NX * sizeof(double), hipMemcpyHostToDevice));
    HIPCHK(hipMemcpy(du, u, (size_t)B * NU * sizeof(double), hipMemcpyHostToDevice));
    HIPCHK(hipMemcpy(dd, d, (size_t)B * h->nd * sizeof(double), hipMemcpyHostToDevice));
    if (per_row) {
        std::vector<double> crop((size_t)B * NCROP);
        for (int b = 0; b < B; ++b)
            for (int i = 0; i < NCROP; ++i) crop[(size_t)b * NCROP + i] = p[(size_t)b * NP + CROP0 + i];
        HIPCHK(hipMemcpy(dcrop, crop.data(), crop.size() * sizeof(double), hipMemcpyHostToDevice));
    }
    HIPCHK(hipMemset(h->fail_dev, 0, sizeof(int)));
    HIPCHK(hipMemset(dout, 0xFF, (size_t)B * NX * sizeof(double)));
    if (bdf) {
        if (h->stats_cap < B) {
            if (h->stats_dev) (void)hipFree(h->stats_dev);
            h->stats_dev = nullptr; h->stats_cap = 0;
            HIPCHK(hipMalloc(&h->stats_dev, (size_t)B * GLGYM_NSOLVER_STAT * sizeof(int32_t)));
            h->stats_cap = B;
        }
        h->stats_rows = 0;
        ModelConst<double> m = h->md;
        if (p) make_model_const<double>(p_used, m);
        HIPCHK(bdf_launch(dx, du, dd, dcrop, B, h->nd, h->dt, h->rtol, h->atol, h->max_steps, m, p_used[39], p_used[162], dout,
                          h->stats_dev, h->fail_dev));
        h->stats.resize((size_t)B * GLGYM_NSOLVER_STAT);
        HIPCHK(hipMemcpy(h->stats.data(), h->stats_dev, h->stats.size() * sizeof(int32_t), hipMemcpyDeviceToHost));
        h->stats_rows = B;
    } else if (h->dtype == GLGYM_F32) {
        ModelConst<float> m = h->mf;
        if (p) make_model_const<float>(p_used, m);
        rc = run_evalf<float>(h, m, p_used, dx, du, dd, dcrop, B, dout, rhs_only);
    } else {
        ModelConst<double> m = h->md;
        if (p) make_model_const<double>(p_used, m);
        rc = run_evalf<double>(h, m, p_used, dx, du, dd, dcrop, B, dout, rhs_only);
    }
    if (rc != GLGYM_OK) return rc;
    HIPCHK(hipMemcpy(out, dout, (size_t)B * NX * sizeof(double), hipMemcpyDeviceToHost));
    int n_failed = 0;
    HIPCHK(hipMemcpy(&n_failed, h->fail_dev, sizeof(int), hipMemcpyDeviceToHost));
    if (n_failed > 0) {
        g_err = "glgym_evalF: the integration failed for " + std::to_string(n_failed) + " of " + std::to_string(B) +
                (bdf ? " rows (BDF: step limit, right-hand-side limit, step-size underflow or a non-finite value)"
                     : " rows (no two consecutive attempts of the n_sub, 2x, 4x, 8x ladder agreed)") + "; their rows of x_next are NaN";
        return GLGYM_EODE;
    }
    if (!rhs_only) {
        for (int b = 0; b < B; ++b)
            for (int i = 0; i < NX; ++i)
                if (std::isnan(out[(size_t)b * NX + i])) {
                    g_err = "glgym_evalF: row " + std::to_string(b) + " of " + std::to_string(B) + " came back unwritten (state " + std::to_string(i) +
                            " is NaN although no integration was reported as failed): internal error of the kernel's row-writing lane selection";
                    return GLGYM_EHIP;
                }
    }
    return GLGYM_OK;
}

extern "C" {

int glgym_evalF(glgym_handle h, const double* x, const double* u, const double* d, const double* p, int p_rows, int B,
                double* x_next)
{
    return evalf_impl(h, x, u, d, p, p_rows, B, x_next, 0);
}

int glgym_rhs(glgym_handle h, const double* x, const double* u, const double* d, int B, double* dx)
{
    return evalf_impl(h, x, u, d, nullptr, 1, B, dx, 1);
}

}

template <int SCH>
static void launch_step_sch(const glgym_step_args* a, const StepArgsT<float>& k, const ModelConst<float>& m, const RewardConst<float>& rw,
                            dim3 grid, dim3 block, hipStream_t st, bool def, bool occ2)
{
    using T = float;
    if (occ2) {
        hipLaunchKernelGGL((step_kernel<T, false, true, false, SCH, 2>), grid, block, 0, st, k, m, rw);
        return;
    }
    if (a->crop_p) {
        if (def) hipLaunchKernelGGL((step_kernel<T, true, true, false, SCH>), grid, block, 0, st, k, m, rw);
        else hipLaunchKernelGGL((step_kernel<T, true, false, false, SCH>), grid, block, 0, st, k, m, rw);
    } else {
        if (def) hipLaunchKernelGGL((step_kernel<T, false, true, false, SCH>), grid, block, 0, st, k, m, rw);
        else hipLaunchKernelGGL((step_kernel<T, false, false, false, SCH>), grid, block, 0, st, k, m, rw);
    }
}

template <class T, int SCH>
static void launch_quad_sch(const glgym_step_args* a, const StepArgsT<T>& k, const ModelConst<T>& m, const RewardConst<T>& rw,
                            dim3 qgrid, dim3 block, hipStream_t st, bool def, bool pair)
{
    const dim3 pgrid((8 * (size_t)a->B + WAVE - 1) / WAVE);
    if constexpr (sizeof(T) == 8) {
        if (pair) hipLaunchKernelGGL((step_kernel_quad<T, false, SCH, true, false, true>), pgrid, block, 0, st, k, m, rw);
        else if (a->crop_p) hipLaunchKernelGGL((step_kernel_quad<T, false, SCH, true, true>), qgrid, block, 0, st, k, m, rw);
        else hipLaunchKernelGGL((step_kernel_quad<T, false, SCH, true, false>), qgrid, block, 0, st, k, m, rw);
    } else {
        if (pair && def) hipLaunchKernelGGL((step_kernel_quad<T, true, SCH, false, false, true>), pgrid, block, 0, st, k, m, rw);
        else if (pair) hipLaunchKernelGGL((step_kernel_quad<T, false, SCH, false, false, true>), pgrid, block, 0, st, k, m, rw);
        else if (def) hipLaunchKernelGGL((step_kernel_quad<T, true, SCH, false, false>), qgrid, block, 0, st, k, m, rw);
        else hipLaunchKernelGGL((step_kernel_quad<T, false, SCH, false, false>), qgrid, block, 0, st, k, m, rw);
    }
}

template <class T>
static int launch_step(glgym_handle h, const glgym_step_args* a, const ModelConst<T>& m, const RewardConst<T>& rw,
                       hipStream_t st)
{
    StepArgsT<T> k;
    k.B = a->B; k.ld = a->ld;
    k.x = (T*)a->x; k.u = (T*)a->u; k.action = a->action; k.control = (const T*)a->control;
    k.weather = (const T*)a->weather; k.weather_rows = a->weather_rows;
    k.w_off = a->w_off; k.timestep = a->timestep; k.crop_p = (const T*)a->crop_p; k.N = a->N;
    k.reward = (T*)a->reward; k.info = (T*)a->info; k.done = a->done; k.metrics = a->metrics; k.step_flags = a->step_flags;
    k.dt = T(h->dt); k.n_sub = h->n_sub; k.gasR = T(h->p[39]); k.tCanMin = T(h->p[162]); k.nd = h->nd;
    k.du = h->du;
    for (int j = 0; j < NU; ++j) { k.u_min[j] = h->u_min[j]; k.u_max[j] = h->u_max[j]; }
    k.pipe = h->variant == GLGYM_ODE_PIPE ? 1 : 0;
    k.window = h->window;
    k.verify = h->verify_mode == GLGYM_VERIFY_ALWAYS || (h->verify_mode == GLGYM_VERIFY_AUTO && (!a->action || h->du > 0.1001f));
    const dim3 grid((a->B + WAVE - 1) / WAVE), block(WAVE), qgrid((4 * a->B + WAVE - 1) / WAVE);
    const bool pipe = h->variant == GLGYM_ODE_PIPE;
    if (pipe && (a->crop_p || h->scheme != GLGYM_SCHEME_RK4)) {
        g_err = "glgym_step: GLGYM_ODE_PIPE supports neither per-env crop parameters nor schemes other than GLGYM_SCHEME_RK4";
        return GLGYM_EINVAL;
    }
    const bool def = h->use_specialised && std::memcmp(&m, &DefaultConst<T>::value, sizeof m) == 0;
    const bool pair = k.verify && h->ladder_parallel && !a->crop_p && (size_t)8 * a->B <= (size_t)WAVE * h->n_simd;
    if constexpr (sizeof(T) == 8) {
        if (h->scheme == GLGYM_SCHEME_RK2) launch_quad_sch<T, GLGYM_SCHEME_RK2>(a, k, m, rw, qgrid, block, st, def, pair);
        else if (h->scheme == GLGYM_SCHEME_RK3) launch_quad_sch<T, GLGYM_SCHEME_RK3>(a, k, m, rw, qgrid, block, st, def, pair);
        else if (h->scheme == GLGYM_SCHEME_LS5) launch_quad_sch<T, GLGYM_SCHEME_LS5>(a, k, m, rw, qgrid, block, st, def, pair);
        else launch_quad_sch<T, GLGYM_SCHEME_RK4>(a, k, m, rw, qgrid, block, st, def, pair);
        HIPCHK(hipGetLastError());
        return GLGYM_OK;
    } else {
        const int layout_env = h->layout;
        const bool quad_ok = !pipe && !a->crop_p;
        const int b_small = 4 * h->n_simd * 4;
        if (quad_ok && (layout_env == 2 || (layout_env == 0 && a->B <= b_small))) {
            if (h->scheme == GLGYM_SCHEME_RK2) launch_quad_sch<T, GLGYM_SCHEME_RK2>(a, k, m, rw, qgrid, block, st, def, pair);
            else if (h->scheme == GLGYM_SCHEME_RK3) launch_quad_sch<T, GLGYM_SCHEME_RK3>(a, k, m, rw, qgrid, block, st, def, pair);
            else if (h->scheme == GLGYM_SCHEME_LS5) launch_quad_sch<T, GLGYM_SCHEME_LS5>(a, k, m, rw, qgrid, block, st, def, pair);
            else launch_quad_sch<T, GLGYM_SCHEME_RK4>(a, k, m, rw, qgrid, block, st, def, pair);
            HIPCHK(hipGetLastError());
            return GLGYM_OK;
        }
        if (pipe) {
            hipLaunchKernelGGL((step_kernel<T, false, false, true>), grid, block, 0, st, k, m, rw);
            HIPCHK(hipGetLastError());
            return GLGYM_OK;
        }
        const bool occ2 = def && !a->crop_p && (h->occupancy == 2 || (h->occupancy == 0 && (size_t)a->B >= (size_t)2 * WAVE * h->n_simd));
        if (h->scheme == GLGYM_SCHEME_RK2) launch_step_sch<GLGYM_SCHEME_RK2>(a, k, m, rw, grid, block, st, def, occ2);
        else if (h->scheme == GLGYM_SCHEME_RK3) launch_step_sch<GLGYM_SCHEME_RK3>(a, k, m, rw, grid, block, st, def, occ2);
        else if (h->scheme == GLGYM_SCHEME_LS5) launch_step_sch<GLGYM_SCHEME_LS5>(a, k, m, rw, grid, block, st, def, occ2);
        else launch_step_sch<GLGYM_SCHEME_RK4>(a, k, m, rw, grid, block, st, def, occ2);
        HIPCHK(hipGetLastError());
        return GLGYM_OK;
    }
}

template <class T>
static int launch_step_bdf(glgym_handle h, const glgym_step_args* a, const RewardConst<T>& rw, hipStream_t st)
{
    if (h->variant == GLGYM_ODE_PIPE) {
        g_err = "glgym_step: GLGYM_INTEGRATOR_BDF does not support GLGYM_ODE_PIPE";
        return GLGYM_EINVAL;
    }
    glbdf::BdfEnvArgs<T> k;
    k.ld = a->ld;
    k.x = (T*)a->x; k.u = (T*)a->u; k.action = a->action; k.control = (const T*)a->control;
    k.weather = (const T*)a->weather; k.weather_rows = a->weather_rows; k.nd = h->nd;
    k.w_off = a->w_off; k.timestep = a->timestep; k.crop_p = (const T*)a->crop_p; k.N = a->N;
    k.reward = (T*)a->reward; k.info = (T*)a->info; k.done = a->done; k.step_flags = a->step_flags;
    k.dt = h->dt; k.rtol = h->rtol; k.atol = h->atol; k.max_steps = h->max_steps;
    k.gasR = h->p[39]; k.tCanMin = h->p[162];
    k.du = h->du;
    for (int j = 0; j < NU; ++j) { k.u_min[j] = h->u_min[j]; k.u_max[j] = h->u_max[j]; }
    HIPCHK(bdf_env_launch<T>(k, a->B, h->md, rw, a->metrics, st));
    return GLGYM_OK;
}

extern "C" int glgym_step(glgym_handle h, const glgym_step_args* a, void* stream)
{
    if (!h || !a) { g_err = "glgym_step: null handle / arguments"; return GLGYM_EINVAL; }
    if (a->struct_size != (int32_t)sizeof(glgym_step_args)) {
        g_err = "glgym_step: glgym_step_args.struct_size is " + std::to_string(a->struct_size) + ", this library expects " +
                std::to_string(sizeof(glgym_step_args)) + " (ABI " + std::to_string(GLGYM_ABI_VERSION) + "): rebuild against include/glgym.h";
        return GLGYM_EINVAL;
    }
    if (a->B < 1 || a->ld < a->B || !a->x || !a->u || !a->weather || !a->w_off || !a->timestep ||
        !a->reward || !a->done || (!a->action) == (!a->control) || a->weather_rows < 1) {
        g_err = "glgym_step: bad arguments (exactly one of action/control, ld >= B, non-null state/outputs)";
        return GLGYM_EINVAL;
    }
    if (h->step_integrator == GLGYM_INTEGRATOR_BDF) {
        DeviceGuard dev_guard(h);
        return h->dtype == GLGYM_F32 ? launch_step_bdf<float>(h, a, h->rf, (hipStream_t)stream)
                                     : launch_step_bdf<double>(h, a, h->rd, (hipStream_t)stream);
    }
    if (h->integrator != GLGYM_INTEGRATOR_EXPLICIT) {
        g_err = "glgym_step: GLGYM_INTEGRATOR_BDF is available to glgym_evalF only; set GLGYM_INTEGRATOR_EXPLICIT for env-steps";
        return GLGYM_EINVAL;
    }
    DeviceGuard dev_guard(h);
    hipStream_t st = (hipStream_t)stream;
    return h->dtype == GLGYM_F32 ? launch_step<float>(h, a, h->mf, h->rf, st)
                                 : launch_step<double>(h, a, h->md, h->rd, st);
}

static const int OBS_MODULE_SIZE[6] = {4, 3, 6, 5, 5, 0};

template <class T> static int launch_obs(glgym_handle h, const glgym_obs_args* a, hipStream_t st)
{
    ObsArgsT<T> k;
    k.B = a->B; k.ld = a->ld; k.x = (const T*)a->x; k.u = (const T*)a->u; k.weather = (const T*)a->weather;
    k.weather_rows = a->weather_rows; k.w_off = a->w_off; k.timestep = a->timestep; k.start_day = a->start_day;
    k.Np = a->Np; k.obs = a->obs; k.mask = a->mask; k.term_obs = a->term_obs; k.doy_inc = std::fmod(h->dt / 86400.0, 365.0); k.hod_inc = h->dt / 3600.0; k.nd = h->nd;
    int blocks = (a->B + OBS_ROWS - 1) / OBS_ROWS;
    static const int cap = [] { const char* e = std::getenv("GLGYM_OBS_BLOCKS"); return e ? std::atoi(e) : 4096; }();
    if (blocks > cap) blocks = cap;
    for (int m = 0; m < 6; ++m) k.moff[m] = -1;
    k.dim = 0;
    for (int i = 0; i < h->n_obs_modules; ++i) {
        const int m = h->obs_modules[i];
        k.moff[m] = k.dim;
        k.dim += m == GLGYM_OBS_FORECAST ? 5 * a->Np : OBS_MODULE_SIZE[m];
    }
    const size_t lds = (size_t)OBS_ROWS * k.dim * sizeof(float);
    hipLaunchKernelGGL((obs_kernel<T>), dim3(blocks), dim3(256), lds, st, k);
    HIPCHK(hipGetLastError());
    return GLGYM_OK;
}



extern "C" int glgym_weather(glgym_handle h, const glgym_weather_args* a, void* stream)
{
    DeviceGuard dev_guard(h);
    if (!h || !a || a->n_raw < 3 || a->n_out < 1 || a->nd < ND || !a->time || !a->i_glob || !a->t_out || !a->rh || !a->wind ||
        !a->t_sky || !a->out || !a->workspace) {
        g_err = "glgym_weather: bad arguments (>= 3 raw samples, nd >= 10, non-null device pointers)";
        return GLGYM_EINVAL;
    }
    hipStream_t st = (hipStream_t)stream;
    const int n = a->n_raw;
    double* W = a->workspace;
    double* D = a->workspace + (size_t)10 * n;
    hipLaunchKernelGGL(weather_convert_kernel, dim3((n + 255) / 256), dim3(256), 0, st, n, a->time, a->i_glob, a->t_out,
                       a->rh, a->wind, a->t_sky, a->co2_ppm, W);
    hipLaunchKernelGGL(weather_scan_kernel, dim3(1), dim3(64), 0, st, n, a->time, W);
    hipLaunchKernelGGL(pchip_slopes_kernel, dim3((n + 255) / 256, 10), dim3(256), 0, st, n, 10, a->time, W, D);
    if (a->nd > ND) {
        HIPCHK(hipMemsetAsync(a->out, 0, (size_t)a->n_out * a->nd * (h->dtype == GLGYM_F32 ? 4 : 8), st));
    }
    const dim3 grid((a->n_out + 255) / 256, 10);
    if (h->dtype == GLGYM_F32)
        hipLaunchKernelGGL((pchip_eval_kernel<float>), grid, dim3(256), 0, st, n, 10, a->n_out, a->nd, a->time, W, D,
                           (float*)a->out);
    else
        hipLaunchKernelGGL((pchip_eval_kernel<double>), grid, dim3(256), 0, st, n, 10, a->n_out, a->nd, a->time, W, D,
                           (double*)a->out);
    HIPCHK(hipGetLastError());
    return GLGYM_OK;
}

extern "C" int glgym_vecnorm(glgym_handle h, const glgym_vecnorm_args* a, void* stream)
{
    DeviceGuard dev_guard(h);
    if (!h || !a || a->B < 1 || a->dim < 1 || !a->obs || !a->obs_out || !a->obs_mean || !a->obs_var || !a->obs_count ||
        !a->workspace || (a->reward && (!a->reward_out || !a->ret_stats || !a->returns))) {
        g_err = "glgym_vecnorm: bad arguments";
        return GLGYM_EINVAL;
    }
    hipStream_t st = (hipStream_t)stream;
    const int B = a->B, dim = a->dim;
    double* acc = a->workspace;
    double* acc2 = a->workspace + (size_t)VN_REP * 2 * dim;
    HIPCHK(hipMemsetAsync(a->workspace, 0, ((size_t)VN_REP * 2 * dim + 2) * sizeof(double), st));
    const int do_obs = a->training && a->norm_obs, do_ret = a->training && a->reward != nullptr;
    int col_threads = (dim + WAVE - 1) / WAVE * WAVE;
    if (col_threads > 1024) col_threads = 1024;
    if (do_obs) {
        int blocks = (B + 63) / 64;
        if (blocks > 1024) blocks = 1024;
        hipLaunchKernelGGL(vecnorm_moments_kernel, dim3(blocks), dim3(col_threads), 0, st, a->obs, B, dim, acc);
    }
    if (do_ret) {
        if (h->dtype == GLGYM_F32)
            hipLaunchKernelGGL((vecnorm_returns_kernel<float>), dim3((B + 255) / 256), dim3(256), 0, st,
                               (const float*)a->reward, a->returns, B, a->gamma, acc2);
        else
            hipLaunchKernelGGL((vecnorm_returns_kernel<double>), dim3((B + 255) / 256), dim3(256), 0, st,
                               (const double*)a->reward, a->returns, B, a->gamma, acc2);
    }
    double* scale = acc;
    if (do_obs || do_ret || a->norm_obs)
        hipLaunchKernelGGL(vecnorm_merge_kernel, dim3(1), dim3(1024), 0, st, a->obs_mean, a->obs_var, a->obs_count, acc, dim, B,
                           a->ret_stats, acc2, do_obs, do_ret, a->epsilon, a->norm_obs ? scale : nullptr);
    const size_t total = (size_t)B * dim;
    if (a->norm_obs) {
        int blocks = (B + 15) / 16;
        if (blocks > 8192) blocks = 8192;
        hipLaunchKernelGGL(vecnorm_apply_kernel, dim3(blocks), dim3(col_threads), 0, st, a->obs, a->obs_out, B, dim,
                           a->obs_mean, scale, a->clip_obs);
    } else if (a->obs_out != a->obs) {
        HIPCHK(hipMemcpyAsync(a->obs_out, a->obs, total * sizeof(float), hipMemcpyDeviceToDevice, st));
    }
    if (a->reward) {
        if (h->dtype == GLGYM_F32)
            hipLaunchKernelGGL((vecnorm_reward_kernel<float>), dim3((B + 255) / 256), dim3(256), 0, st,
                               (const float*)a->reward, a->reward_out, a->returns, a->done, B, a->ret_stats, a->epsilon,
                               a->clip_reward, a->norm_reward);
        else
            hipLaunchKernelGGL((vecnorm_reward_kernel<double>), dim3((B + 255) / 256), dim3(256), 0, st,
                               (const double*)a->reward, a->reward_out, a->returns, a->done, B, a->ret_stats, a->epsilon,
                               a->clip_reward, a->norm_reward);
    }
    HIPCHK(hipGetLastError());
    return GLGYM_OK;
}

extern "C" {

int glgym_obs(glgym_handle h, const glgym_obs_args* a, void* stream)
{
    DeviceGuard dev_guard(h);
    if (!h || !a || a->B < 1 || a->ld < a->B || !a->x || !a->u || !a->weather || !a->w_off || !a->timestep ||
        !a->start_day || !a->obs || a->Np < 0 || a->Np > OBS_MAX_NP) {
        g_err = "glgym_obs: bad arguments (null pointer, ld < B, or Np outside 0..128)";
        return GLGYM_EINVAL;
    }
    hipStream_t st = (hipStream_t)stream;
    return h->dtype == GLGYM_F32 ? launch_obs<float>(h, a, st) : launch_obs<double>(h, a, st);
}

int glgym_set_obs_modules(glgym_handle h, const int32_t* modules, int n)
{
    if (!h || !modules || n < 1 || n > 6) { g_err = "glgym_set_obs_modules: 1..6 module ids expected"; return GLGYM_EINVAL; }
    int seen = 0;
    for (int i = 0; i < n; ++i) {
        if (modules[i] < 0 || modules[i] > 5 || (seen >> modules[i] & 1)) {
            g_err = "glgym_set_obs_modules: ids must be distinct GLGYM_OBS_* values";
            return GLGYM_EINVAL;
        }
        seen |= 1 << modules[i];
    }
    for (int i = 0; i < n; ++i) h->obs_modules[i] = modules[i];
    h->n_obs_modules = n;
    return GLGYM_OK;
}

int glgym_obs_dim(glgym_handle h, int Np)
{
    if (!h || Np < 0 || Np > OBS_MAX_NP) return GLGYM_EINVAL;
    int dim = 0;
    for (int i = 0; i < h->n_obs_modules; ++i)
        dim += h->obs_modules[i] == GLGYM_OBS_FORECAST ? 5 * Np : OBS_MODULE_SIZE[h->obs_modules[i]];
    return dim;
}

int glgym_reset(glgym_handle h, const glgym_reset_args* a, void* stream)
{
    DeviceGuard dev_guard(h);
    if (!h || !a || a->B < 1 || a->ld < a->B || !a->x || !a->u || !a->timestep || !a->weather || !a->w_off) {
        g_err = "glgym_reset: bad arguments";
        return GLGYM_EINVAL;
    }
    hipStream_t st = (hipStream_t)stream;
    const dim3 grid((a->B + 255) / 256), block(256);
    if (h->dtype == GLGYM_F32)
        hipLaunchKernelGGL((reset_kernel<float>), grid, block, 0, st, a->B, a->ld, a->mask, (float*)a->x, (float*)a->u,
                           a->timestep, (const float*)a->weather, a->weather_rows, a->w_off, a->start_rows, a->start_days,
                           a->n_starts, a->start_day, a->episode, (unsigned long long)a->seed, h->nd);
    else
        hipLaunchKernelGGL((reset_kernel<double>), grid, block, 0, st, a->B, a->ld, a->mask, (double*)a->x,
                           (double*)a->u, a->timestep, (const double*)a->weather, a->weather_rows, a->w_off,
                           a->start_rows, a->start_days, a->n_starts, a->start_day, a->episode,
                           (unsigned long long)a->seed, h->nd);
    HIPCHK(hipGetLastError());
    return GLGYM_OK;
}

int glgym_crop_noise(glgym_handle h, void* crop_p, int B, int ld, double scale, uint64_t seed, uint64_t draw_index,
                     void* stream)
{
    DeviceGuard dev_guard(h);
    if (!h || !crop_p || B < 1 || ld < B) return GLGYM_EINVAL;
    hipStream_t st = (hipStream_t)stream;
    const dim3 grid((B + 255) / 256), block(256);
    if (h->dtype == GLGYM_F32)
        hipLaunchKernelGGL((crop_noise_kernel<float>), grid, block, 0, st, (float*)crop_p, B, ld, h->p0_crop_dev,
                           (float)scale, (unsigned long long)seed, (unsigned long long)draw_index);
    else
        hipLaunchKernelGGL((crop_noise_kernel<double>), grid, block, 0, st, (double*)crop_p, B, ld, h->p0_crop_dev,
                           (float)scale, (unsigned long long)seed, (unsigned long long)draw_index);
    HIPCHK(hipGetLastError());
    return GLGYM_OK;
}

int glgym_rng_crop_noise(glgym_handle h, void* crop_p, int B, int ld, double scale, uint64_t* rng_state, void* stream)
{
    DeviceGuard dev_guard(h);
    if (!h || !rng_state || B < 1 || ld < B || !(scale >= 0.0)) {
        g_err = "glgym_rng_crop_noise: bad arguments (null handle or stream buffer, ld < B, or a negative scale)";
        return GLGYM_EINVAL;
    }
    hipStream_t st = (hipStream_t)stream;
    if (h->dtype == GLGYM_F32) HIPCHK(rng_crop_noise_launch<float>((float*)crop_p, B, ld, h->p0_crop_dev, scale, rng_state, st));
    else HIPCHK(rng_crop_noise_launch<double>((double*)crop_p, B, ld, h->p0_crop_dev, scale, rng_state, st));
    return GLGYM_OK;
}

int glgym_rng_reset_draw(glgym_handle h, int B, int ld, const unsigned char* mask, uint64_t* rng_state, int n_years, int n_days,
                         const int32_t* start_rows, const float* start_days, int32_t* w_off, float* start_day, void* stream)
{
    DeviceGuard dev_guard(h);
    if (!h || !rng_state || B < 1 || ld < B || n_years < 1 || n_days < 1 || !start_rows || !w_off) {
        g_err = "glgym_rng_reset_draw: bad arguments (null pointer, ld < B, or an empty start grid)";
        return GLGYM_EINVAL;
    }
    HIPCHK(rng_reset_draw_launch(B, ld, mask, rng_state, n_years, n_days, start_rows, start_days, w_off, start_day, (hipStream_t)stream));
    return GLGYM_OK;
}

static bool plan_size_ok(const char* who, int32_t got, size_t want)
{
    if (got == (int32_t)want) return true;
    g_err = std::string(who) + ": struct_size is " + std::to_string(got) + ", this library expects " + std::to_string(want) +
            " (ABI " + std::to_string(GLGYM_ABI_VERSION) + "): rebuild against include/glgym.h";
    return false;
}

int glgym_plan_fork(glgym_handle h, const glgym_plan_fork_args* a, void* stream)
{
    if (!h || !a) { g_err = "glgym_plan_fork: null handle / arguments"; return GLGYM_EINVAL; }
    if (!plan_size_ok("glgym_plan_fork", a->struct_size, sizeof *a)) return GLGYM_EINVAL;
    if (a->n_children < 1 || a->n_parents < 1 || a->ld_parent < a->n_parents || a->ld_child < a->n_children ||
        (!a->parent && (a->K < 1 || (int64_t)a->n_parents * a->K < a->n_children)) ||
        !a->x_parent || !a->u_parent || !a->timestep_parent || !a->w_off_parent || !a->x || !a->u || !a->timestep || !a->w_off ||
        !a->ret || !a->viol || !a->n_steps || !a->alive || !a->failed) {
        g_err = "glgym_plan_fork: bad arguments (null pointer, ld < batch, or without a parent table K < 1 or fewer than C = P * K slots)";
        return GLGYM_EINVAL;
    }
    DeviceGuard dev_guard(h);
    hipStream_t st = (hipStream_t)stream;
    if (h->dtype == GLGYM_F32) HIPCHK(plan_fork_launch<float>(*a, st));
    else HIPCHK(plan_fork_launch<double>(*a, st));
    return GLGYM_OK;
}

int glgym_plan_accumulate(glgym_handle h, const glgym_plan_accumulate_args* a, void* stream)
{
    if (!h || !a) { g_err = "glgym_plan_accumulate: null handle / arguments"; return GLGYM_EINVAL; }
    if (!plan_size_ok("glgym_plan_accumulate", a->struct_size, sizeof *a)) return GLGYM_EINVAL;
    if (a->B < 1 || a->ld < a->B || !a->reward || !a->info || !a->done || !a->ret || !a->viol || !a->n_steps || !a->alive || !a->failed) {
        g_err = "glgym_plan_accumulate: bad arguments (null pointer or ld < B)";
        return GLGYM_EINVAL;
    }
    DeviceGuard dev_guard(h);
    hipStream_t st = (hipStream_t)stream;
    if (h->dtype == GLGYM_F32) HIPCHK(plan_accumulate_launch<float>(*a, st));
    else HIPCHK(plan_accumulate_launch<double>(*a, st));
    return GLGYM_OK;
}

int glgym_plan_rollout(glgym_handle h, const glgym_plan_rollout_args* a, void* stream)
{
    if (!h || !a) { g_err = "glgym_plan_rollout: null handle / arguments"; return GLGYM_EINVAL; }
    if (!plan_size_ok("glgym_plan_rollout", a->struct_size, sizeof *a)) return GLGYM_EINVAL;
    if (a->H < 1 || !(a->gamma >= 0.0) || !std::isfinite(a->gamma) || (!a->actions) == (!a->controls) || a->step.B < 1 ||
        a->step.ld < a->step.B || !a->step.reward || !a->step.info || !a->step.done || !a->ret || !a->viol || !a->n_steps ||
        !a->alive || !a->failed) {
        g_err = "glgym_plan_rollout: bad arguments (H < 1, gamma, exactly one of actions / controls, ld >= B, non-null reward / info / done / accumulators)";
        return GLGYM_EINVAL;
    }
    glgym_step_args s = a->step;
    s.metrics = nullptr;
    glgym_plan_accumulate_args acc;
    acc.struct_size = (int32_t)sizeof acc;
    acc.B = s.B; acc.ld = s.ld; acc.reward = s.reward; acc.info = s.info; acc.done = s.done; acc.step_flags = s.step_flags;
    acc.ret = a->ret; acc.viol = a->viol; acc.n_steps = a->n_steps; acc.alive = a->alive; acc.failed = a->failed;
    const size_t plane = (size_t)NU * (size_t)s.ld * (h->dtype == GLGYM_F32 ? sizeof(float) : sizeof(double));
    double w = 1.0;
    for (int k = 0; k < a->H; ++k) {
        s.action = a->actions ? a->actions + (size_t)k * (size_t)s.B * NU : nullptr;
        s.control = a->controls ? (const void*)((const char*)a->controls + (size_t)k * plane) : nullptr;
        const int rc = glgym_step(h, &s, stream);
        if (rc != GLGYM_OK) return rc;
        acc.w = w;
        const int ra = glgym_plan_accumulate(h, &acc, stream);
        if (ra != GLGYM_OK) return ra;
        w = w * a->gamma;
    }
    return GLGYM_OK;
}

int glgym_plan_select(glgym_handle h, const glgym_plan_select_args* a, void* stream)
{
    if (!h || !a) { g_err = "glgym_plan_select: null handle / arguments"; return GLGYM_EINVAL; }
    if (!plan_size_ok("glgym_plan_select", a->struct_size, sizeof *a)) return GLGYM_EINVAL;
    const bool wants_actions = a->best_action || a->best_sequence || a->mean_sequence;
    if (a->P < 1 || a->K < 1 || a->H < 1 || a->H > 65535 || (int64_t)a->P * a->K > INT32_MAX || !a->ret || !a->failed || !a->best_k ||
        !a->best_ret || (wants_actions && !a->actions) || (a->mean_sequence && !(a->temperature > 0.0 && std::isfinite(a->temperature)))) {
        g_err = "glgym_plan_select: bad arguments (P, K, H < 1, H > 65 535, null pointer, action outputs without actions, or mean_sequence "
                "without a finite temperature > 0)";
        return GLGYM_EINVAL;
    }
    DeviceGuard dev_guard(h);
    HIPCHK(plan_select_launch(*a, (hipStream_t)stream));
    return GLGYM_OK;
}

int glgym_rule_based(glgym_handle h, const glgym_rule_cfg* cfg, const glgym_rule_args* a, void* stream)
{
    DeviceGuard dev_guard(h);
    if (!h || !cfg || !a || a->B < 1 || a->ld < a->B || !a->x || !a->weather || !a->w_off || !a->timestep || !a->control ||
        a->weather_rows < 1 || (!a->start_day && !a->doy) || cfg->vent_heat_Pband == 0 || cfg->vent_rh_Pband == 0 ||
        cfg->vent_cold_Pband == 0 || cfg->thScrPband == 0 || cfg->thScrRhPband == 0 || cfg->tHeatBand == 0 ||
        cfg->co2Band == 0) {
        g_err = "glgym_rule_based: bad arguments (null pointer, ld < B, or a zero proportional band)";
        return GLGYM_EINVAL;
    }
    hipStream_t st = (hipStream_t)stream;
    const dim3 grid((a->B + 255) / 256), block(256);
    const double doy_inc = std::fmod(h->dt / 86400.0, 365.0), hod_inc = h->dt / 3600.0;
    if (h->dtype == GLGYM_F32)
        hipLaunchKernelGGL((rule_based_kernel<float>), grid, block, 0, st, *cfg, a->B, a->ld, (const float*)a->x,
                           (const float*)a->weather, a->weather_rows, a->w_off, a->timestep, a->start_day, a->hour, a->doy,
                           doy_inc, hod_inc, (float*)a->control, h->nd);
    else
        hipLaunchKernelGGL((rule_based_kernel<double>), grid, block, 0, st, *cfg, a->B, a->ld, (const double*)a->x,
                           (const double*)a->weather, a->weather_rows, a->w_off, a->timestep, a->start_day, a->hour,
                           a->doy, doy_inc, hod_inc, (double*)a->control, h->nd);
    HIPCHK(hipGetLastError());
    return GLGYM_OK;
}

int glgym_timer_start(glgym_handle h, void* stream)
{
    DeviceGuard dev_guard(h);
    if (!h) return GLGYM_EINVAL;
    HIPCHK(hipEventRecord(h->ev0, (hipStream_t)stream));
    return GLGYM_OK;
}

int glgym_timer_stop(glgym_handle h, void* stream, float* elapsed_ms)
{
    DeviceGuard dev_guard(h);
    if (!h || !elapsed_ms) return GLGYM_EINVAL;
    HIPCHK(hipEventRecord(h->ev1, (hipStream_t)stream));
    HIPCHK(hipEventSynchronize(h->ev1));
    HIPCHK(hipEventElapsedTime(elapsed_ms, h->ev0, h->ev1));
    return GLGYM_OK;
}

}
```

greenlight-gym2_amd/gl_gym_amd/_lib.py:

```python
from __future__ import annotations

import ctypes as C
import os
from pathlib import Path

_HERE = Path(__file__).resolve().parent
LIB_PATH = Path(os.environ.get("GLGYM_LIB", _HERE / "libglgym.so"))

NX, NU, ND, NP, NCROP, NINFO, NMETRIC = 28, 6, 10, 208, 34, 11, 14
METRIC_REPLICAS, METRIC_STRIDE = 64, 32
F32, F64 = 0, 1
ODE, ODE_PIPE = 0, 1
SCHEME_RK4, SCHEME_RK2 = 0, 1
SCHEME_RK3 = 2
SCHEME_LS5 = 3
SCHEMES = {"rk4": SCHEME_RK4, "rk2": SCHEME_RK2, "rk3": SCHEME_RK3, "ls5": SCHEME_LS5}
ABI_VERSION = 7
INTEGRATORS = {"explicit": 0, "bdf": 1}
NSOLVER_STAT = 5
SOLVER_STAT_KEYS = ("steps", "rhs_evals", "jacobians", "factorisations", "order")
LAYOUTS = {"auto": 0, "one": 1, "quad": 2}
DEFAULT_N_SUB = {"rk4": 240, "rk2": 336, "rk3": 270, "ls5": 128}
DEFAULT_SCHEME = "ls5"
VERIFY_MODES = {"auto": 0, "always": 1, "never": 2}
N_SUB_MULTIPLE = {"rk4": 4, "rk2": 4, "rk3": 3, "ls5": 2}
PRESETS = {"throughput": {k: (v, 0) for k, v in DEFAULT_N_SUB.items()},
           "parity": {"ls5": (192, 1), "rk4": (640, 0), "rk3": (720, 0), "rk2": (896, 0)}}


def preset_n_sub(scheme: str, dt: float, preset: str = "throughput"):
    n0, window = PRESETS[preset][scheme]
    n = n0 * float(dt) / 900.0
    mult = window if window > 0 else N_SUB_MULTIPLE[scheme]
    return max(mult, int(-(-n // mult) * mult)), window


def resolve_scheme(scheme, variant: str = "ode") -> str:
    if variant not in ("ode", "ode_pipe"):
        raise ValueError("variant must be 'ode' or 'ode_pipe'")
    if scheme is None:
        return "rk4" if variant == "ode_pipe" else DEFAULT_SCHEME
    if scheme not in SCHEMES:
        raise ValueError("scheme must be 'ls5', 'rk4', 'rk3' or 'rk2'")
    if variant == "ode_pipe" and scheme != "rk4":
        raise ValueError(f"variant 'ode_pipe' is built for scheme 'rk4' only (got {scheme!r}): leave scheme unset or pass scheme='rk4'")
    return scheme


def default_n_sub(scheme: str, dt: float) -> int:
    return preset_n_sub(scheme, dt, "throughput")[0]
OK, EINVAL, ENODEV, EHIP, ENOMEM, EODE = 0, -1, -2, -3, -4, -5

INFO_KEYS = ("EPI", "revenue", "variable_costs", "fixed_costs", "co2_cost", "heat_cost", "elec_cost",
             "temp_violation", "co2_violation", "rh_violation", "lamp_violation")
METRIC_KEYS = ("sum_reward", "sum_EPI", "n_done", "n_ode_fail", "sum_co2_violation", "sum_temp_violation",
               "sum_rh_violation", "n_env_steps", "n_guard_retries", "n_refined_substeps", "n_flag_err", "n_flag_branch",
               "n_flag_cap", "n_flag_heavy")


class GlgymError(RuntimeError):
    pass


class GlgymOdeError(GlgymError):
    """glgym_evalF: the integration failed for at least one row (GLGYM_EODE) -- the counterpart of the RuntimeError the
    reference's evalF raises when CVODES fails (greenlight_model.cpp:110, caught at tomato_env.py:119-123)."""


class RewardCfg(C.Structure):
    _fields_ = [(n, C.c_double) for n in (
        "elec_price", "heating_price", "co2_price", "fruit_price", "dmfm", "fixed_greenhouse_cost", "fixed_co2_cost",
        "fixed_lamp_cost", "fixed_screen_cost", "pen_lamp", "co2_min", "co2_max", "temp_min", "temp_max", "rh_min",
        "rh_max")]


class StepArgs(C.Structure):
    _fields_ = [("struct_size", C.c_int32), ("B", C.c_int32), ("ld", C.c_int32), ("x", C.c_void_p), ("u", C.c_void_p), ("action", C.c_void_p),
                ("control", C.c_void_p), ("weather", C.c_void_p), ("weather_rows", C.c_int32), ("w_off", C.c_void_p),
                ("timestep", C.c_void_p), ("crop_p", C.c_void_p), ("N", C.c_int32), ("reward", C.c_void_p),
                ("info", C.c_void_p), ("done", C.c_void_p), ("metrics", C.c_void_p), ("step_flags", C.c_void_p)]


def make_step_args(*args, **kw):
    return StepArgs(C.sizeof(StepArgs), *args, **kw)


SF_FIRST_MASK, SF_ACCEPT_AGREE_FLAGGED, SF_ACCEPT_LAST_ALONE, SF_FAILED = 31, 32, 64, 128
SF_BDF = 2048
METRIC_BDF = 14
BDF_METRIC_KEYS = ("bdf_steps", "bdf_rhs_evals", "bdf_jacobians", "bdf_factorisations")


class ObsArgs(C.Structure):
    _fields_ = [("B", C.c_int32), ("ld", C.c_int32), ("x", C.c_void_p), ("u", C.c_void_p), ("weather", C.c_void_p),
                ("weather_rows", C.c_int32), ("w_off", C.c_void_p), ("timestep", C.c_void_p), ("start_day", C.c_void_p),
                ("Np", C.c_int32), ("obs", C.c_void_p), ("mask", C.c_void_p), ("term_obs", C.c_void_p)]


class ResetArgs(C.Structure):
    _fields_ = [("B", C.c_int32), ("ld", C.c_int32), ("mask", C.c_void_p), ("x", C.c_void_p), ("u", C.c_void_p),
                ("timestep", C.c_void_p), ("weather", C.c_void_p), ("weather_rows", C.c_int32), ("w_off", C.c_void_p),
                ("start_rows", C.c_void_p), ("start_days", C.c_void_p), ("n_starts", C.c_int32),
                ("start_day", C.c_void_p), ("episode", C.c_void_p), ("seed", C.c_uint64)]


class VecNormArgs(C.Structure):
    _fields_ = [("B", C.c_int32), ("dim", C.c_int32), ("obs", C.c_void_p), ("obs_out", C.c_void_p),
                ("reward", C.c_void_p), ("reward_out", C.c_void_p), ("done", C.c_void_p), ("obs_mean", C.c_void_p),
                ("obs_var", C.c_void_p), ("obs_count", C.c_void_p), ("ret_stats", C.c_void_p), ("returns", C.c_void_p),
                ("workspace", C.c_void_p), ("gamma", C.c_double), ("epsilon", C.c_double), ("clip_obs", C.c_float),
                ("clip_reward", C.c_float), ("training", C.c_int32), ("norm_obs", C.c_int32),
                ("norm_reward", C.c_int32)]


class PlanForkArgs(C.Structure):
    _fields_ = [("struct_size", C.c_int32), ("n_children", C.c_int32), ("n_parents", C.c_int32), ("K", C.c_int32),
                ("ld_parent", C.c_int32), ("ld_child", C.c_int32), ("parent", C.c_void_p), ("x_parent", C.c_void_p),
                ("u_parent", C.c_void_p), ("timestep_parent", C.c_void_p), ("w_off_parent", C.c_void_p),
                ("start_day_parent", C.c_void_p), ("crop_parent", C.c_void_p), ("x", C.c_void_p), ("u", C.c_void_p),
                ("timestep", C.c_void_p), ("w_off", C.c_void_p), ("start_day", C.c_void_p), ("crop", C.c_void_p),
                ("ret", C.c_void_p), ("viol", C.c_void_p), ("n_steps", C.c_void_p), ("alive", C.c_void_p), ("failed", C.c_void_p)]


class PlanAccumulateArgs(C.Structure):
    _fields_ = [("struct_size", C.c_int32), ("B", C.c_int32), ("ld", C.c_int32), ("w", C.c_double), ("reward", C.c_void_p),
                ("info", C.c_void_p), ("done", C.c_void_p), ("step_flags", C.c_void_p), ("ret", C.c_void_p), ("viol", C.c_void_p),
                ("n_steps", C.c_void_p), ("alive", C.c_void_p), ("failed", C.c_void_p)]


class PlanRolloutArgs(C.Structure):
    _fields_ = [("struct_size", C.c_int32), ("H", C.c_int32), ("gamma", C.c_double), ("step", StepArgs), ("actions", C.c_void_p),
                ("controls", C.c_void_p), ("ret", C.c_void_p), ("viol", C.c_void_p), ("n_steps", C.c_void_p), ("alive", C.c_void_p),
                ("failed", C.c_void_p)]


class PlanSelectArgs(C.Structure):
    _fields_ = [("struct_size", C.c_int32), ("P", C.c_int32), ("K", C.c_int32), ("H", C.c_int32), ("ret", C.c_void_p),
                ("failed", C.c_void_p), ("actions", C.c_void_p), ("best_k", C.c_void_p), ("best_ret", C.c_void_p),
                ("best_action", C.c_void_p), ("best_sequence", C.c_void_p), ("temperature", C.c_double),
                ("mean_sequence", C.c_void_p)]


def make_plan_args(cls, *args, **kw):
    return cls(C.sizeof(cls), *args, **kw)


RULE_FIELDS = ("lamps_on", "lamps_off", "lamps_day_start", "lamps_day_stop", "lamps_off_sun", "lamp_rad_sum_limit",
               "temp_setpoint_day", "temp_setpoint_night", "heat_correction", "heat_deadzone", "co2_day",
               "vent_heat_Pband", "rh_max", "mech_dehumid_Pband", "vent_rh_Pband", "t_vent_off", "vent_cold_Pband",
               "thScrSpDay", "thScrSpNight", "thScrPband", "thScrDeadZone", "thScrRh", "thScrRhPband", "lampExtraHeat",
               "blScrExtraRh", "rhMax", "tHeatBand", "co2Band", "useBlScr")


class RuleCfg(C.Structure):
    _fields_ = [(n, C.c_double) for n in RULE_FIELDS]


class RuleArgs(C.Structure):
    _fields_ = [("B", C.c_int32), ("ld", C.c_int32), ("x", C.c_void_p), ("weather", C.c_void_p),
                ("weather_rows", C.c_int32), ("w_off", C.c_void_p), ("timestep", C.c_void_p), ("start_day", C.c_void_p),
                ("hour", C.c_void_p), ("doy", C.c_void_p), ("control", C.c_void_p)]


class WeatherArgs(C.Structure):
    _fields_ = [("n_raw", C.c_int32), ("time", C.c_void_p), ("i_glob", C.c_void_p), ("t_out", C.c_void_p),
                ("rh", C.c_void_p), ("wind", C.c_void_p), ("t_sky", C.c_void_p), ("co2_ppm", C.c_double),
                ("n_out", C.c_int32), ("nd", C.c_int32), ("out", C.c_void_p), ("workspace", C.c_void_p)]


_DP = C.POINTER(C.c_double)
PROTOTYPES = {
    "glgym_version": (C.c_char_p, []),
    "glgym_abi_version": (C.c_int, []),
    "glgym_set_window": (C.c_int, [C.c_void_p, C.c_int]),
    "glgym_set_layout": (C.c_int, [C.c_void_p, C.c_int]),
    "glgym_set_occupancy": (C.c_int, [C.c_void_p, C.c_int]),
    "glgym_set_ladder_parallel": (C.c_int, [C.c_void_p, C.c_int]),
    "glgym_last_error": (C.c_char_p, []),
    "glgym_create": (C.c_int, [C.c_int, C.c_int, C.c_int, C.c_int, C.c_double, _DP, C.c_int, C.c_int, C.c_int,
                               C.POINTER(C.c_void_p)]),
    "glgym_destroy": (C.c_int, [C.c_void_p]),
    "glgym_set_params": (C.c_int, [C.c_void_p, _DP]),
    "glgym_set_params_keep_reward_scale": (C.c_int, [C.c_void_p, _DP]),
    "glgym_set_n_sub": (C.c_int, [C.c_void_p, C.c_int]),
    "glgym_set_model_variant": (C.c_int, [C.c_void_p, C.c_int]),
    "glgym_set_scheme": (C.c_int, [C.c_void_p, C.c_int]),
    "glgym_set_verify": (C.c_int, [C.c_void_p, C.c_int]),
    "glgym_set_reward": (C.c_int, [C.c_void_p, C.POINTER(RewardCfg)]),
    "glgym_get_reward_scale": (C.c_int, [C.c_void_p, _DP, _DP, _DP]),
    "glgym_evalF": (C.c_int, [C.c_void_p, _DP, _DP, _DP, _DP, C.c_int, C.c_int, _DP]),
    "glgym_rhs": (C.c_int, [C.c_void_p, _DP, _DP, _DP, C.c_int, _DP]),
    "glgym_set_integrator": (C.c_int, [C.c_void_p, C.c_int]),
    "glgym_set_tolerances": (C.c_int, [C.c_void_p, C.c_double, C.c_double, C.c_int]),
    "glgym_get_solver_stats": (C.c_int, [C.c_void_p, C.c_int, C.POINTER(C.c_int32)]),
    "glgym_set_step_integrator": (C.c_int, [C.c_void_p, C.c_int]),
    "glgym_step": (C.c_int, [C.c_void_p, C.POINTER(StepArgs), C.c_void_p]),
    "glgym_obs": (C.c_int, [C.c_void_p, C.POINTER(ObsArgs), C.c_void_p]),
    "glgym_set_obs_modules": (C.c_int, [C.c_void_p, C.POINTER(C.c_int32), C.c_int]),
    "glgym_obs_dim": (C.c_int, [C.c_void_p, C.c_int]),
    "glgym_set_control_limits": (C.c_int, [C.c_void_p, _DP, _DP, C.c_double]),
    "glgym_reset": (C.c_int, [C.c_void_p, C.POINTER(ResetArgs), C.c_void_p]),
    "glgym_crop_noise": (C.c_int, [C.c_void_p, C.c_void_p, C.c_int, C.c_int, C.c_double, C.c_uint64, C.c_uint64,
                                   C.c_void_p]),
    "glgym_rng_crop_noise": (C.c_int, [C.c_void_p, C.c_void_p, C.c_int, C.c_int, C.c_double, C.c_void_p, C.c_void_p]),
    "glgym_rng_reset_draw": (C.c_int, [C.c_void_p, C.c_int, C.c_int, C.c_void_p, C.c_void_p, C.c_int, C.c_int, C.c_void_p,
                                       C.c_void_p, C.c_void_p, C.c_void_p, C.c_void_p]),
    "glgym_plan_fork": (C.c_int, [C.c_void_p, C.POINTER(PlanForkArgs), C.c_void_p]),
    "glgym_plan_accumulate": (C.c_int, [C.c_void_p, C.POINTER(PlanAccumulateArgs), C.c_void_p]),
    "glgym_plan_rollout": (C.c_int, [C.c_void_p, C.POINTER(PlanRolloutArgs), C.c_void_p]),
    "glgym_plan_select": (C.c_int, [C.c_void_p, C.POINTER(PlanSelectArgs), C.c_void_p]),
    "glgym_rule_based": (C.c_int, [C.c_void_p, C.POINTER(RuleCfg), C.POINTER(RuleArgs), C.c_void_p]),
    "glgym_vecnorm": (C.c_int, [C.c_void_p, C.POINTER(VecNormArgs), C.c_void_p]),
    "glgym_weather": (C.c_int, [C.c_void_p, C.POINTER(WeatherArgs), C.c_void_p]),
    "glgym_timer_start": (C.c_int, [C.c_void_p, C.c_void_p]),
    "glgym_timer_stop": (C.c_int, [C.c_void_p, C.c_void_p, C.POINTER(C.c_float)]),
}

_lib = None


def load():
    global _lib
    if _lib is None:
        if not LIB_PATH.exists():
            raise GlgymError(f"{LIB_PATH} not found: build it with `python -c 'import __graft_entry__ as g; g.build()'` "
                             "(hipcc --offload-arch=gfx950).  There is no CPU fallback.")
        try:
            import torch
        except Exception:
            pass
        lib = C.CDLL(str(LIB_PATH))
        for name, (res, args) in PROTOTYPES.items():
            fn = getattr(lib, name)
            fn.restype, fn.argtypes = res, args
        if lib.glgym_abi_version() != ABI_VERSION:
            raise GlgymError(f"{LIB_PATH} has ABI {lib.glgym_abi_version()}, this binding expects {ABI_VERSION}: rebuild the library")
        _lib = lib
    return _lib


def check(rc: int, what: str = "glgym"):
    if rc != OK:
        msg = load().glgym_last_error().decode() or {EINVAL: "invalid argument", ENODEV: "no HIP device",
                                                       EHIP: "HIP error", ENOMEM: "out of memory"}.get(rc, "")
        raise (GlgymOdeError if rc == EODE else GlgymError)(f"{what} failed (status {rc}): {msg}")
```

greenlight-gym2_amd/gl_gym_amd/tomato_env.py:

```python
from __future__ import annotations

import ctypes as C
import os
from typing import Any, Dict, List, Optional, Sequence

import numpy as np

from . import _lib as L
from . import np_stream
from .greenlight_model import _check_integrator, _check_tolerances
from .parameters import init_default_params
from .utils import synthetic_weather

try:
    from gymnasium import spaces as _spaces

    def _box(low, high, shape, dtype=np.float32):
        return _spaces.Box(low=low, high=high, shape=shape, dtype=dtype)
except Exception:
    class _Box:
        def __init__(self, low, high, shape, dtype):
            self.low = np.broadcast_to(np.asarray(low, dtype=dtype), shape).copy()
            self.high = np.broadcast_to(np.asarray(high, dtype=dtype), shape).copy()
            self.shape, self.dtype = tuple(shape), np.dtype(dtype)
            self._rng = np.random.default_rng()

        def seed(self, seed=None):
            self._rng = np.random.default_rng(seed)

        def sample(self):
            return self._rng.uniform(self.low, self.high).astype(self.dtype)

        def contains(self, v):
            v = np.asarray(v)
            return v.shape == self.shape and bool(np.all(v >= self.low) and np.all(v <= self.high))

    def _box(low, high, shape, dtype=np.float32):
        return _Box(low, high, shape, dtype)

DEFAULT_REWARD = dict(fixed_greenhouse_cost=15., fixed_co2_cost=0.015, fixed_lamp_cost=0.07, fixed_screen_cost=2.,
                      elec_price=0.3, heating_price=0.09, co2_price=0.3, fruit_price=1.6, dmfm=0.065,
                      pen_weights=[4.e-4, 5.e-3, 7.e-4], pen_lamp=0.1)
DEFAULT_CONSTRAINTS = dict(co2_min=300., co2_max=1600., temp_min=15., temp_max=34., rh_min=50., rh_max=85.)


def _torch():
    import torch
    return torch


RNGS = ("philox", "numpy")


def _check_rng(rng, start_grid, n_starts):
    if rng not in RNGS:
        raise ValueError("rng must be 'philox' or 'numpy'")
    if start_grid is None:
        return rng, ((1, int(n_starts)) if rng == "numpy" else None)
    grid = tuple(int(v) for v in start_grid)
    if len(grid) != 2 or grid[0] < 1 or grid[1] < 1 or grid[0] * grid[1] != int(n_starts):
        raise ValueError(f"start_grid must be (n_years, n_days) with n_years * n_days = len(start_rows) = {n_starts}, got {start_grid!r}")
    return rng, grid


def _observation_modules(Np, names):
    return observation_modules(Np, names)


class ObservationModule:

    def __init__(self, name, obs_names, low=-1e-4, high=1e4):
        self.name, self.obs_names, self.n_obs, self.low, self.high = name, list(obs_names), len(obs_names), low, high

    def __repr__(self):
        return f"{self.name}({self.n_obs})"


OBSERVATION_MODULE_IDS = {"IndoorClimateObservations": 0, "BasicCropObservations": 1, "ControlObservations": 2,
                          "WeatherObservations": 3, "TimeObservations": 4, "WeatherForecastObservations": 5}
DEFAULT_OBSERVATION_MODULES = ["IndoorClimateObservations", "BasicCropObservations", "ControlObservations",
                               "WeatherObservations", "TimeObservations", "WeatherForecastObservations"]


def observation_modules(Np: int, names: Optional[Sequence[str]] = None):
    wx = ["glob_rad", "temp_out", "rh_out", "co2_out", "wind_speed"]
    table = {"IndoorClimateObservations": (["co2_air", "temp_air", "rh_air", "pipe_temp"],),
             "BasicCropObservations": (["24CanTemp", "cFruit", "tSum"],),
             "ControlObservations": (["uBoil", "uCo2", "uThScr", "uVent", "uLamp", "uBlScr"], 0.0, 1.0),
             "WeatherObservations": (wx,),
             "TimeObservations": (["timestep", "day of year sin", "day of year cos", "hour of day sin",
                                   "hour of day cos"],),
             "WeatherForecastObservations": (wx * Np,)}
    names = DEFAULT_OBSERVATION_MODULES if names is None else list(names)
    for n in names:
        if n == "StateObservations":
            raise NotImplementedError("StateObservations cannot be built by the reference's TomatoEnv either "
                                      "(observations.py:42: __init__ takes no env) and returns random numbers (:57)")
        if n not in table:
            raise KeyError(f"unknown observation module {n!r}; known: {sorted(table)}")
    if len(set(names)) != len(names) or not names:
        raise ValueError("observation_modules must be a non-empty list without repeats")
    return [ObservationModule(n, *table[n]) for n in names]


class LazyInfos:

    def __init__(self, keys, info_rows, controls, dones, term_obs, step_flags=None):
        self._keys, self._rows, self._ctrl, self._dones, self._term = keys, info_rows, controls, dones, term_obs
        self._flags = step_flags
        self._cache = {}

    def __len__(self):
        return len(self._rows)

    def _make(self, b):
        d = dict(zip(self._keys, self._rows[b].tolist()))
        d["controls"] = self._ctrl[b]
        d["TimeLimit.truncated"] = False
        if self._flags is not None:
            d["integration"] = int(self._flags[b])
        if self._term is not None and self._dones[b]:
            d["terminal_observation"] = self._term[b]
        return d

    def __getitem__(self, b):
        if isinstance(b, slice):
            return [self[i] for i in range(*b.indices(len(self)))]
        b = int(b)
        if b < 0:
            b += len(self)
        if b not in self._cache:
            self._cache[b] = self._make(b)
        return self._cache[b]

    def __setitem__(self, b, value):
        self._cache[int(b)] = value

    def __iter__(self):
        return (self[i] for i in range(len(self)))


class TomatoVecEnv:
    def __init__(self, num_envs: int, weather: Optional[np.ndarray] = None, params: Optional[np.ndarray] = None,
                 dt: float = 900.0, season_length: float = 60, pred_horizon: float = 0.5, dtype: str = "float32",
                 n_sub: Optional[int] = None, device: str = "cuda:0", seed: int = 0, uncertainty_scale: float = 0.0,
                 start_rows: Optional[Sequence[int]] = None, start_days: Optional[Sequence[float]] = None,
                 reward_params: Optional[Dict[str, Any]] = None, constraints: Optional[Dict[str, float]] = None,
                 auto_reset: bool = True, collect_metrics: bool = True, lazy_infos: Optional[bool] = None,
                 model_variant: str = "ode", scheme: Optional[str] = None, window: Optional[int] = None,
                 preset: Optional[str] = None,
                 observation_modules: Optional[Sequence[str]] = None, u_min: Optional[Sequence[float]] = None,
                 u_max: Optional[Sequence[float]] = None, delta_u_max: float = 0.1, integration_info: bool = True,
                 integrator: str = "explicit", rtol: float = 1e-6, atol: float = 1e-6, max_steps: int = 10000,
                 rng: str = "philox", start_grid: Optional[Sequence[int]] = None, env_index_offset: int = 0):
        _check_integrator(integrator, model_variant)
        _check_tolerances(rtol, atol, max_steps)
        _check_rng(rng, start_grid, 1 if start_rows is None else len(start_rows))
        torch = _torch()
        if not torch.cuda.is_available():
            raise L.GlgymError("TomatoVecEnv needs a HIP device (torch.cuda.is_available() is False); "
                               "there is no CPU fallback")
        self._lib = L.load()
        self.torch = torch
        self.device = torch.device(device)
        torch.cuda.set_device(self.device)
        self.num_envs = self.B = int(num_envs)
        self.ld = (self.B + 63) // 64 * 64
        self.dt = float(dt)
        self.c = 86400
        self.nx, self.nu, self.num_params = L.NX, L.NU, L.NP
        weather_is_tensor = weather is not None and hasattr(weather, "data_ptr")
        self.nd = L.ND if weather is None else int(np.shape(weather)[1])
        if model_variant not in ("ode", "ode_pipe"):
            raise ValueError("model_variant must be 'ode' or 'ode_pipe'")
        self.model_variant = model_variant
        self.season_length = season_length
        self.N = int(season_length * self.c / self.dt)
        self.Np = int(pred_horizon * self.c / self.dt)
        self.observation_modules = _observation_modules(self.Np, observation_modules)
        if self.observation_modules[0].name != "IndoorClimateObservations":
            raise NotImplementedError("observation_modules must start with IndoorClimateObservations: the reference's "
                                      "GreenhouseReward takes co2 / temperature / humidity from obs[0:3]")
        self.obs_dim = sum(m.n_obs for m in self.observation_modules)
        self.f64 = str(dtype) in ("float64", "f64", "double")
        self.tdtype = torch.float64 if self.f64 else torch.float32
        scheme = L.resolve_scheme(scheme, model_variant)
        self.preset = ("parity" if self.f64 else "throughput") if preset is None else preset
        if self.preset not in L.PRESETS:
            raise ValueError("preset must be 'throughput' or 'parity'")
        self.scheme = scheme
        n_def, w_def = L.preset_n_sub(scheme, self.dt, self.preset)
        self.n_sub = int(n_def if n_sub is None else n_sub)
        self.window = int((w_def if n_sub is None else 0) if window is None else window)
        self.uncertainty_scale = float(uncertainty_scale)
        self.auto_reset = auto_reset
        self.lazy_infos = (int(num_envs) > 4096) if lazy_infos is None else bool(lazy_infos)
        self.integration_info = bool(integration_info)
        self.seed_value = int(seed)

        self._p = np.asarray(init_default_params(L.NP) if params is None else params, dtype=np.float32)
        self._h = C.c_void_p()
        p64 = np.ascontiguousarray(self.p, dtype=np.float64)
        L.check(self._lib.glgym_create(L.NX, L.NU, self.nd, L.NP, self.dt, p64.ctypes.data_as(L._DP),
                                       L.F64 if self.f64 else L.F32, self.n_sub, self.device.index or 0,
                                       C.byref(self._h)), "glgym_create")
        self._env_at_create = tuple(os.environ.get(k) for k in ("GLGYM_LAYOUT", "GLGYM_OCC", "GLGYM_VERIFY"))
        if model_variant == "ode_pipe":
            L.check(self._lib.glgym_set_model_variant(self._h, L.ODE_PIPE), "glgym_set_model_variant")
        L.check(self._lib.glgym_set_scheme(self._h, L.SCHEMES[scheme]), "glgym_set_scheme")
        L.check(self._lib.glgym_set_window(self._h, self.window), "glgym_set_window")
        self.rtol, self.atol, self.max_steps = float(rtol), float(atol), int(max_steps)
        self.set_integrator(integrator)
        self.u_min = np.asarray([0.0] * L.NU if u_min is None else u_min, dtype=np.float32)
        self.u_max = np.asarray([1.0] * L.NU if u_max is None else u_max, dtype=np.float32)
        self.delta_u_max = np.ones(L.NU, dtype=np.float32) * np.float32(delta_u_max)
        if self.u_min.shape != (L.NU,) or self.u_max.shape != (L.NU,):
            raise ValueError("u_min / u_max must have 6 entries")
        lo64, hi64 = self.u_min.astype(np.float64), self.u_max.astype(np.float64)
        L.check(self._lib.glgym_set_control_limits(self._h, lo64.ctypes.data_as(L._DP), hi64.ctypes.data_as(L._DP),
                                                   float(delta_u_max)), "glgym_set_control_limits")
        ids = (C.c_int32 * len(self.observation_modules))(*[OBSERVATION_MODULE_IDS[m.name] for m in self.observation_modules])
        L.check(self._lib.glgym_set_obs_modules(self._h, ids, len(ids)), "glgym_set_obs_modules")
        assert self._lib.glgym_obs_dim(self._h, self.Np) == self.obs_dim
        rp = dict(DEFAULT_REWARD, **(reward_params or {}))
        cs = dict(DEFAULT_CONSTRAINTS, **(constraints or {}))
        self.reward_params, self.constraints = rp, cs
        cfg = L.RewardCfg(rp["elec_price"], rp["heating_price"], rp["co2_price"], rp["fruit_price"], rp["dmfm"],
                          rp["fixed_greenhouse_cost"], rp["fixed_co2_cost"], rp["fixed_lamp_cost"],
                          rp["fixed_screen_cost"], rp["pen_lamp"], cs["co2_min"], cs["co2_max"], cs["temp_min"],
                          cs["temp_max"], cs["rh_min"], cs["rh_max"])
        L.check(self._lib.glgym_set_reward(self._h, C.byref(cfg)), "glgym_set_reward")
        mx, mn, fx = C.c_double(), C.c_double(), C.c_double()
        L.check(self._lib.glgym_get_reward_scale(self._h, C.byref(mx), C.byref(mn), C.byref(fx)))
        self.max_profit, self.min_profit, self.fixed_costs = mx.value, mn.value, fx.value

        if weather is None:
            weather = synthetic_weather(dt=self.dt)
        self._weather_data = (weather.detach().double().cpu().numpy() if weather_is_tensor
                              else np.ascontiguousarray(weather, dtype=np.float64))
        self.weather_rows = int(self._weather_data.shape[0])
        need = self.N + 1 + self.Np + 1
        if self.weather_rows < need:
            raise ValueError(f"weather tensor has {self.weather_rows} rows, an episode needs {need}")
        if start_rows is None:
            start_rows = [0]
        self.start_rows = np.asarray(start_rows, dtype=np.int64)
        if np.any(self.start_rows + need > self.weather_rows) or np.any(self.start_rows < 0):
            raise ValueError("start_rows + episode length exceeds the weather tensor")
        self.start_days = np.asarray(start_days if start_days is not None
                                     else self.start_rows * self.dt / self.c, dtype=np.float32)
        self.rng, self.start_grid = _check_rng(rng, start_grid, len(self.start_rows))
        self.env_index_offset = int(env_index_offset)

        dev, T = self.device, self.tdtype
        z = lambda *s, dtype=T: torch.zeros(*s, dtype=dtype, device=dev)
        self.weather_t = (weather.to(device=dev, dtype=T).contiguous() if weather_is_tensor
                          else torch.as_tensor(self.weather_data, dtype=T, device=dev).contiguous())
        self.x_T, self.u_T = z(L.NX, self.ld), z(L.NU, self.ld)
        self.ctrl_T = z(L.NU, self.ld)
        self.info_T = z(L.NINFO, self.ld)
        self.reward_t = z(self.ld)
        self.done_t = z(self.B, dtype=torch.uint8)
        self.timestep_t = z(self.B, dtype=torch.int32)
        self.w_off_t = z(self.B, dtype=torch.int32)
        self.start_day_t = z(self.B, dtype=torch.float32)
        self.action_t = z(self.B, L.NU, dtype=torch.float32)
        self.obs_t = z(self.B, self.obs_dim, dtype=torch.float32)
        self.term_obs_t = z(self.B, self.obs_dim, dtype=torch.float32)
        self.metrics_t = z(L.METRIC_REPLICAS, L.METRIC_STRIDE, dtype=torch.float32) if collect_metrics else None
        self.step_flags_t = z(self.B, dtype=torch.int32)
        self.crop_T = z(L.NCROP, self.ld) if self.uncertainty_scale > 0 else None
        self._start_rows_t = torch.as_tensor(self.start_rows, dtype=torch.int32, device=dev)
        self._start_days_t = torch.as_tensor(self.start_days, dtype=torch.float32, device=dev)
        self.episode_t = z(self.B, dtype=torch.int32)
        self._draw = 0
        self.rng_state_t = z(np_stream.NWORD, self.ld, dtype=torch.int64) if self.rng == "numpy" else None
        if self.rng == "numpy":
            self._seed_streams(self.seed_value)
        self.x, self.u = self.x_T[:, :self.B].t(), self.u_T[:, :self.B].t()

        lo = np.concatenate([np.full(m.n_obs, m.low, np.float32) for m in self.observation_modules])
        hi = np.concatenate([np.full(m.n_obs, m.high, np.float32) for m in self.observation_modules])
        self.observation_space = _box(lo, hi, (self.obs_dim,), np.float32)
        self.action_space = _box(-1.0, 1.0, (L.NU,), np.float32)
        self._actions = None
        self._keep_applied_u, self._u_applied_T = False, None
        self.reset_infos: List[dict] = [{} for _ in range(self.B)]
        self._obs_host = [torch.empty(self.B, self.obs_dim, dtype=torch.float32).pin_memory() for _ in range(2)]
        self._obs_flip = 0

    def _obs_to_host(self, obs_t):
        buf = self._obs_host[self._obs_flip]
        self._obs_flip ^= 1
        buf.copy_(obs_t, non_blocking=True)
        self.torch.cuda.current_stream(self.device).synchronize()
        return buf.numpy()

    def _stream(self):
        return C.c_void_p(self.torch.cuda.current_stream(self.device).cuda_stream)

    def _seed_streams(self, seed: int):
        first = int(seed) + self.env_index_offset
        self.set_rng_state(np_stream.seed_states(range(first, first + self.B)))

    def get_rng_state(self) -> List[dict]:
        if self.rng_state_t is None:
            raise L.GlgymError("get_rng_state: this environment was built with rng='philox' (stateless, keyed by seed and counters)")
        return np_stream.unpack_states(self.rng_state_t[:, :self.B].cpu().numpy().view(np.uint64))

    def set_rng_state(self, states):
        if self.rng_state_t is None:
            raise L.GlgymError("set_rng_state: this environment was built with rng='philox'")
        words = states if isinstance(states, np.ndarray) else np_stream.pack_states(states)
        if words.shape != (np_stream.NWORD, self.B):
            raise ValueError(f"set_rng_state: expected {self.B} states, got an array of shape {words.shape}")
        self.rng_state_t[:, :self.B].copy_(self.torch.as_tensor(np.ascontiguousarray(words, dtype=np.uint64).view(np.int64)))

    _STATE_TENSORS = ("x_T", "u_T", "timestep_t", "w_off_t", "start_day_t", "episode_t", "crop_T", "rng_state_t", "obs_t", "done_t")

    def get_state(self) -> Dict[str, Any]:
        state: Dict[str, Any] = {k: (None if getattr(self, k) is None else getattr(self, k).clone()) for k in self._STATE_TENSORS}
        state.update(_draw=int(self._draw), seed_value=int(self.seed_value), num_envs=self.B, dtype=str(self.tdtype), rng=self.rng)
        return state

    def set_state(self, state: Dict[str, Any]):
        missing = [k for k in self._STATE_TENSORS + ("_draw", "seed_value", "num_envs", "dtype", "rng") if k not in state]
        if missing:
            raise ValueError(f"set_state: not a get_state() snapshot (missing {missing})")
        if state["num_envs"] != self.B or state["dtype"] != str(self.tdtype) or state["rng"] != self.rng:
            raise ValueError(f"set_state: snapshot of {state['num_envs']} envs, {state['dtype']}, rng={state['rng']!r} does not fit "
                             f"this environment ({self.B} envs, {self.tdtype}, rng={self.rng!r})")
        for k in self._STATE_TENSORS:
            mine, theirs = getattr(self, k), state[k]
            if (mine is None) != (theirs is None) or (mine is not None and (mine.shape != theirs.shape or mine.dtype != theirs.dtype)):
                raise ValueError(f"set_state: {k} of the snapshot does not fit this environment")
        for k in self._STATE_TENSORS:
            if getattr(self, k) is not None:
                getattr(self, k).copy_(state[k])
        self._draw, self.seed_value = int(state["_draw"]), int(state["seed_value"])

    def planner(self, n_candidates: int, horizon: int, gamma: float = 1.0, crop: str = "nominal"):
        from .planner import Planner
        return Planner(self, n_candidates, horizon, gamma=gamma, crop=crop)

    def _launch_reset(self, mask_t):
        mask_ptr = mask_t.data_ptr() if mask_t is not None else None
        if self.rng == "numpy":
            L.check(self._lib.glgym_rng_reset_draw(self._h, self.B, self.ld, mask_ptr, self.rng_state_t.data_ptr(), self.start_grid[0],
                                                   self.start_grid[1], self._start_rows_t.data_ptr(), self._start_days_t.data_ptr(),
                                                   self.w_off_t.data_ptr(), self.start_day_t.data_ptr(), self._stream()),
                    "glgym_rng_reset_draw")
            a = L.ResetArgs(self.B, self.ld, mask_ptr, self.x_T.data_ptr(), self.u_T.data_ptr(), self.timestep_t.data_ptr(),
                            self.weather_t.data_ptr(), self.weather_rows, self.w_off_t.data_ptr(), None, None, 0,
                            self.start_day_t.data_ptr(), self.episode_t.data_ptr(), self.seed_value)
            L.check(self._lib.glgym_reset(self._h, C.byref(a), self._stream()), "glgym_reset")
            return
        a = L.ResetArgs(self.B, self.ld, mask_t.data_ptr() if mask_t is not None else None, self.x_T.data_ptr(),
                        self.u_T.data_ptr(), self.timestep_t.data_ptr(), self.weather_t.data_ptr(), self.weather_rows,
                        self.w_off_t.data_ptr(), self._start_rows_t.data_ptr(), self._start_days_t.data_ptr(),
                        len(self.start_rows), self.start_day_t.data_ptr(), self.episode_t.data_ptr(), self.seed_value)
        L.check(self._lib.glgym_reset(self._h, C.byref(a), self._stream()), "glgym_reset")

    def _launch_obs(self, out_t, mask_t=None, term_t=None):
        a = L.ObsArgs(self.B, self.ld, self.x_T.data_ptr(), self.u_T.data_ptr(), self.weather_t.data_ptr(),
                      self.weather_rows, self.w_off_t.data_ptr(), self.timestep_t.data_ptr(),
                      self.start_day_t.data_ptr(), self.Np, out_t.data_ptr(),
                      mask_t.data_ptr() if mask_t is not None else None,
                      term_t.data_ptr() if term_t is not None else None)
        L.check(self._lib.glgym_obs(self._h, C.byref(a), self._stream()), "glgym_obs")

    def _launch_step(self, raw_control: bool):
        if self._env_at_create is not None and tuple(os.environ.get(k) for k in ("GLGYM_LAYOUT", "GLGYM_OCC", "GLGYM_VERIFY")) != self._env_at_create:
            import warnings
            warnings.warn("GLGYM_LAYOUT / GLGYM_OCC / GLGYM_VERIFY changed after this TomatoVecEnv was created: they are read once, at glgym_create, "
                          "and have no effect on an existing handle -- use set_layout() / set_occupancy() / set_verify()", RuntimeWarning, stacklevel=3)
            self._env_at_create = None
        if self.rng == "numpy":
            if not getattr(self, "freeze_crop_noise", False):
                L.check(self._lib.glgym_rng_crop_noise(self._h, self.crop_T.data_ptr() if self.crop_T is not None else None, self.B, self.ld,
                                                       self.uncertainty_scale, self.rng_state_t.data_ptr(), self._stream()),
                        "glgym_rng_crop_noise")
        elif self.crop_T is not None and not getattr(self, "freeze_crop_noise", False):
            L.check(self._lib.glgym_crop_noise(self._h, self.crop_T.data_ptr(), self.B, self.ld,
                                               self.uncertainty_scale, self.seed_value, self._draw, self._stream()),
                    "glgym_crop_noise")
            self._draw += 1
        a = L.make_step_args(self.B, self.ld, self.x_T.data_ptr(), self.u_T.data_ptr(),
                       None if raw_control else getattr(self, "_action_src", self.action_t).data_ptr(),
                       self.ctrl_T.data_ptr() if raw_control else None, self.weather_t.data_ptr(), self.weather_rows,
                       self.w_off_t.data_ptr(), self.timestep_t.data_ptr(),
                       self.crop_T.data_ptr() if self.crop_T is not None else None, self.N,
                       self.reward_t.data_ptr(), self.info_T.data_ptr(), self.done_t.data_ptr(),
                       self.metrics_t.data_ptr() if self.metrics_t is not None else None, self.step_flags_t.data_ptr())
        L.check(self._lib.glgym_step(self._h, C.byref(a), self._stream()), "glgym_step")

    def reset_tensor(self, seed: Optional[int] = None):
        if seed is not None:
            self.seed_value = int(seed)
            self.episode_t.zero_()
            if self.rng == "numpy":
                self._seed_streams(self.seed_value)
        self._launch_reset(None)
        self._launch_obs(self.obs_t)
        return self.obs_t

    def _launch_rule_based(self, controller, hour_t=None, doy_t=None):
        cfg = L.RuleCfg(*[float(getattr(controller, n)) for n in L.RULE_FIELDS])
        if hour_t is None and (self.dt / 3600) * 8 != round((self.dt / 3600) * 8):
            hour_t = self.hour_of_day()
        a = L.RuleArgs(self.B, self.ld, self.x_T.data_ptr(), self.weather_t.data_ptr(), self.weather_rows,
                       self.w_off_t.data_ptr(), self.timestep_t.data_ptr(), self.start_day_t.data_ptr(),
                       hour_t.data_ptr() if hour_t is not None else None,
                       doy_t.data_ptr() if doy_t is not None else None, self.ctrl_T.data_ptr())
        L.check(self._lib.glgym_rule_based(self._h, C.byref(cfg), C.byref(a), self._stream()), "glgym_rule_based")

    def step_tensor(self, actions_t=None, controls_t=None, want_obs: bool = True, controller=None):
        if (actions_t is not None) + (controls_t is not None) + (controller is not None) != 1:
            raise ValueError("give exactly one of actions_t / controls_t / controller")
        self._action_src = self.action_t
        if actions_t is not None:
            if (actions_t.dtype == self.torch.float32 and actions_t.is_cuda and actions_t.device == self.device and
                    actions_t.is_contiguous() and actions_t.numel() == self.B * L.NU):
                self._action_src = actions_t
            else:
                self.action_t.copy_(actions_t.reshape(self.B, L.NU))
        elif controls_t is not None:
            self.ctrl_T[:, :self.B].copy_(controls_t.reshape(self.B, L.NU).t())
        else:
            self._launch_rule_based(controller)
        self._launch_step(raw_control=actions_t is None)
        if want_obs:
            self._launch_obs(self.obs_t)
        if self.auto_reset:
            if self._keep_applied_u:
                if self._u_applied_T is None:
                    self._u_applied_T = self.torch.empty_like(self.u_T)
                self._u_applied_T.copy_(self.u_T)
                self._u_applied_valid = True
            else:
                self._u_applied_valid = False
            self._launch_reset(self.done_t)
            if want_obs:
                self._launch_obs(self.obs_t, self.done_t, self.term_obs_t)
        return self.obs_t, self.reward_t[:self.B], self.done_t, self.info_T[:, :self.B]

    def reset(self):
        return self._obs_to_host(self.reset_tensor())

    def seed(self, seed: Optional[int] = None):
        if seed is not None:
            self.seed_value = int(seed)
            if self.rng == "numpy":
                self._seed_streams(self.seed_value)
        return [seed] * self.B

    def step_async(self, actions):
        self._actions = np.asarray(actions, dtype=np.float32)

    def step_wait(self):
        self._keep_applied_u = True
        try:
            return self._host_result(self.step_tensor(self.torch.as_tensor(self._actions, device=self.device)))
        finally:
            self._keep_applied_u = False

    def _host_result(self, out):
        obs_t, r_t, d_t, info_T = out
        obs, rew = self._obs_to_host(obs_t), r_t.float().cpu().numpy()
        dones, infos = self.host_infos(d_t, info_T)
        return obs, rew, dones, infos

    def host_infos(self, d_t, info_T, term_obs=None):
        dones = d_t.cpu().numpy().astype(bool)
        rows = info_T.double().t().cpu().numpy()
        applied = self._u_applied_T if (self.auto_reset and getattr(self, "_u_applied_valid", False)) else self.u_T
        ctrl = applied[:, :self.B].t().double().cpu().numpy()
        term = None
        if self.auto_reset and dones.any():
            term = self.term_obs_t.cpu().numpy() if term_obs is None else term_obs
        flags = self.step_flags_t.cpu().numpy() if self.integration_info else None
        if self.lazy_infos:
            infos = LazyInfos(L.INFO_KEYS, rows, ctrl, dones, term, flags)
        else:
            infos = [dict(zip(L.INFO_KEYS, row), controls=c) for row, c in zip(rows.tolist(), ctrl)]
            for d in infos:
                d["TimeLimit.truncated"] = False
            if flags is not None:
                for d, f in zip(infos, flags.tolist()):
                    d["integration"] = f
            if term is not None:
                for b in np.nonzero(dones)[0]:
                    infos[b]["terminal_observation"] = term[b]
        return dones, infos

    def step(self, actions):
        self.step_async(actions)
        return self.step_wait()

    def step_raw_control(self, controls):
        torch = self.torch
        obs_t, r_t, d_t, info_T = self.step_tensor(controls_t=torch.as_tensor(np.asarray(controls), dtype=self.tdtype,
                                                                              device=self.device))
        return self._obs_to_host(obs_t), r_t.float().cpu().numpy(), d_t.cpu().numpy().astype(bool), info_T.cpu().numpy()

    def step_raw_control_pipeinput(self, controls):
        torch = self.torch
        _, _, d_t, _ = self.step_tensor(controls_t=torch.as_tensor(np.asarray(controls), dtype=self.tdtype,
                                                                   device=self.device), want_obs=False)
        return self.x.double().cpu().numpy(), d_t.cpu().numpy().astype(bool)

    def _indices(self, indices):
        if indices is None:
            return list(range(self.B))
        return [indices] if isinstance(indices, int) else list(indices)

    def get_attr(self, attr_name: str, indices=None):
        idx = self._indices(indices)
        per_env = {"x": lambda b: self.x[b].double().cpu().numpy(), "u": lambda b: self.u[b].double().cpu().numpy(),
                   "timestep": lambda b: int(self.timestep_t[b]), "start_day": lambda b: float(self.start_day_t[b]),
                   "w_off": lambda b: int(self.w_off_t[b])}
        if attr_name == "growth_year" and getattr(self, "start_years", None) is not None:
            w_off = self.w_off_t.cpu().numpy()
            return [int(self.start_years[int(np.searchsorted(self.start_rows, w_off[b], side="right")) - 1]) for b in idx]
        if attr_name in per_env:
            return [per_env[attr_name](b) for b in idx]
        return [getattr(self, attr_name) for _ in idx]

    def set_attr(self, attr_name: str, value, indices=None):
        setattr(self, attr_name, value)

    def env_method(self, method_name: str, *args, indices=None, **kwargs):
        return [getattr(self, method_name)(*args, **kwargs) for _ in self._indices(indices)]

    def env_is_wrapped(self, wrapper_class, indices=None):
        return [False for _ in self._indices(indices)]

    def get_obs_names(self):
        return [n for m in self.observation_modules for n in m.obs_names]

    def set_seed(self, seed: int):
        self.seed_value = int(seed)
        self.episode_t.zero_()
        if self.rng == "numpy":
            self._seed_streams(self.seed_value)

    def current_weather(self):
        idx = (self.w_off_t + self.timestep_t).long().clamp_(0, self.weather_rows - 1)
        return self.weather_t[idx]

    @property
    def weather_data(self):
        return self._weather_data

    @weather_data.setter
    def weather_data(self, table):
        torch = self.torch
        table = np.ascontiguousarray(table.detach().double().cpu().numpy() if hasattr(table, "detach") else table, dtype=np.float64)
        if table.ndim != 2 or table.shape[1] != self._weather_data.shape[1]:
            raise ValueError(f"weather_data: expected [rows, {self._weather_data.shape[1]}] like the table this env was built with, got {table.shape}")
        need = self.N + 1 + self.Np + 1
        if table.shape[0] < need:
            raise ValueError(f"weather_data has {table.shape[0]} rows, an episode needs {need}")
        self._weather_data = table
        self.weather_rows = int(table.shape[0])
        self.weather_t = torch.as_tensor(table, dtype=self.tdtype, device=self.device).contiguous()
        self.start_rows = np.zeros(1, dtype=np.int64)
        self.start_days = np.asarray(self.start_days[:1], dtype=np.float32)
        self._start_rows_t = torch.as_tensor(self.start_rows, dtype=torch.int32, device=self.device)
        self._start_days_t = torch.as_tensor(self.start_days, dtype=torch.float32, device=self.device)
        if self.rng == "numpy":
            self.start_grid = (1, 1)
        self.w_off_t.zero_()

    @property
    def p(self):
        return self._p

    @p.setter
    def p(self, value):
        value = np.asarray(value, dtype=np.float32)
        if value.shape != (L.NP,):
            raise ValueError(f"p: expected {L.NP} parameters, got an array of shape {value.shape}")
        p64 = np.ascontiguousarray(value, dtype=np.float64)
        L.check(self._lib.glgym_set_params_keep_reward_scale(self._h, p64.ctypes.data_as(L._DP)), "glgym_set_params_keep_reward_scale")
        self._p = value

    def _hod_table(self):
        if getattr(self, "_hod_table_t", None) is None:
            t = np.empty(self.N + 4, dtype=np.float64)
            h = 0.0
            for k in range(len(t)):
                t[k] = h
                h = (h + self.dt / 3600) % 24
            self._hod_table_t = self.torch.as_tensor(t, device=self.device)
        return self._hod_table_t

    def hour_of_day(self):
        return self._hod_table()[self.timestep_t.long().clamp_(0, self.N + 3)]

    def day_of_year(self):
        return self.start_day_t.double() + self.timestep_t.double() * ((self.dt / self.c) % 365)

    def rule_based_controls(self, controller):
        self._launch_rule_based(controller)
        return self.ctrl_T[:, :self.B].t().clone()

    def step_rule_based(self, controller):
        return self._host_result(self.step_tensor(controller=controller))

    def metrics(self) -> Dict[str, float]:
        if self.metrics_t is None:
            return {}
        v = self.metrics_t.double().sum(dim=0)[:L.NMETRIC].cpu().numpy()
        return {k: float(v[i]) for i, k in enumerate(L.METRIC_KEYS)}

    def capture_step_graph(self, want_obs: bool = True):
        if self.crop_T is not None and self.rng != "numpy":
            raise L.GlgymError("capture_step_graph: per-step crop noise carries a host-side draw counter; use step_tensor")
        torch = self.torch
        static_a = torch.zeros(self.B, L.NU, dtype=torch.float32, device=self.device)

        def seq():
            self.action_t.copy_(static_a)
            self._action_src = self.action_t
            self._launch_step(raw_control=False)
            if want_obs:
                self._launch_obs(self.obs_t)
            if self.auto_reset:
                self._launch_reset(self.done_t)
                if want_obs:
                    self._launch_obs(self.obs_t, self.done_t, self.term_obs_t)

        state = [self.x_T, self.u_T, self.timestep_t, self.w_off_t, self.start_day_t, self.episode_t, self.obs_t]
        if self.rng == "numpy":
            state += [self.rng_state_t] + ([self.crop_T] if self.crop_T is not None else [])
        keep = [b.clone() for b in state]
        metrics = None if self.metrics_t is None else self.metrics_t.clone()
        side = torch.cuda.Stream(device=self.device)
        side.wait_stream(torch.cuda.current_stream(self.device))
        with torch.cuda.stream(side):
            seq()
        torch.cuda.current_stream(self.device).wait_stream(side)
        for b, k in zip(state, keep):
            b.copy_(k)
        if metrics is not None:
            self.metrics_t.copy_(metrics)
        graph = torch.cuda.CUDAGraph()
        with torch.cuda.graph(graph):
            seq()
        for b, k in zip(state, keep):
            b.copy_(k)
        if metrics is not None:
            self.metrics_t.copy_(metrics)

        def replay(actions_t):
            static_a.copy_(actions_t.reshape(self.B, L.NU))
            graph.replay()
            return self.obs_t, self.reward_t[:self.B], self.done_t, self.info_T[:, :self.B]
        replay.graph = graph
        return replay

    def set_scheme(self, scheme: str, n_sub: Optional[int] = None, window: Optional[int] = None):
        if scheme not in L.SCHEMES:
            raise ValueError("scheme must be 'ls5', 'rk4', 'rk3' or 'rk2'")
        L.check(self._lib.glgym_set_scheme(self._h, L.SCHEMES[scheme]), "glgym_set_scheme")
        self.scheme = scheme
        n_def, w_def = L.preset_n_sub(scheme, self.dt, self.preset)
        self.set_n_sub(n_def if n_sub is None else n_sub)
        self.set_window((w_def if n_sub is None else 0) if window is None else window)

    def set_integrator(self, name: str, rtol: Optional[float] = None, atol: Optional[float] = None,
                       max_steps: Optional[int] = None):
        rtol = self.rtol if rtol is None else rtol
        atol = self.atol if atol is None else atol
        max_steps = self.max_steps if max_steps is None else max_steps
        _check_integrator(name, self.model_variant)
        _check_tolerances(rtol, atol, max_steps)
        L.check(self._lib.glgym_set_tolerances(self._h, float(rtol), float(atol), int(max_steps)), "glgym_set_tolerances")
        L.check(self._lib.glgym_set_step_integrator(self._h, L.INTEGRATORS[name]), "glgym_set_step_integrator")
        self.integrator, self.rtol, self.atol, self.max_steps = name, float(rtol), float(atol), int(max_steps)

    def solver_metrics(self) -> Dict[str, float]:
        if self.metrics_t is None:
            return {}
        v = self.metrics_t.double().sum(dim=0)[L.METRIC_BDF:L.METRIC_BDF + len(L.BDF_METRIC_KEYS)].cpu().numpy()
        return {k: float(v[i]) for i, k in enumerate(L.BDF_METRIC_KEYS)}

    def set_window(self, window: int):
        self.window = int(window)
        L.check(self._lib.glgym_set_window(self._h, self.window), "glgym_set_window")

    def set_layout(self, layout: str):
        L.check(self._lib.glgym_set_layout(self._h, L.LAYOUTS[layout]), "glgym_set_layout")

    def set_occupancy(self, waves_per_simd: int):
        L.check(self._lib.glgym_set_occupancy(self._h, int(waves_per_simd)), "glgym_set_occupancy")

    def set_ladder_parallel(self, on: bool):
        L.check(self._lib.glgym_set_ladder_parallel(self._h, int(bool(on))), "glgym_set_ladder_parallel")

    def set_n_sub(self, n_sub: int):
        self.n_sub = int(n_sub)
        L.check(self._lib.glgym_set_n_sub(self._h, self.n_sub), "glgym_set_n_sub")

    def set_verify(self, mode: str):
        L.check(self._lib.glgym_set_verify(self._h, L.VERIFY_MODES[mode]), "glgym_set_verify")

    def timer_start(self):
        L.check(self._lib.glgym_timer_start(self._h, self._stream()))

    def timer_stop(self) -> float:
        ms = C.c_float()
        L.check(self._lib.glgym_timer_stop(self._h, self._stream(), C.byref(ms)))
        return float(ms.value)

    def close(self):
        if getattr(self, "_h", None) is not None and self._h.value:
            self.torch.cuda.synchronize(self.device)
            self._lib.glgym_destroy(self._h)
            self._h = C.c_void_p()

    def __del__(self):
        try:
            self.close()
        except Exception:
            pass


class TomatoEnv:

    def __init__(self, weather=None, params=None, dt=900.0, season_length=60, pred_horizon=0.5, dtype="float64",
                 n_sub=None, device="cuda:0", uncertainty_scale=0.0, start_day=0.0, growth_year=2010,
                 reward_params=None, constraints=None, location="synthetic", training=True, model_variant="ode",
                 scheme="rk4", observation_modules=None, u_min=None, u_max=None, delta_u_max=0.1, integrator="explicit", rtol=1e-6,
                 atol=1e-6, max_steps=10000, rng="philox"):
        self.vec = TomatoVecEnv(1, rng=rng, model_variant=model_variant, scheme=scheme, observation_modules=observation_modules,
                                u_min=u_min, u_max=u_max, delta_u_max=delta_u_max, integrator=integrator, rtol=rtol, atol=atol,
                                max_steps=max_steps,
                                weather=weather, params=params, dt=dt, season_length=season_length,
                                pred_horizon=pred_horizon, dtype=dtype, n_sub=n_sub, device=device,
                                uncertainty_scale=uncertainty_scale, start_rows=[0], start_days=[start_day],
                                reward_params=reward_params, constraints=constraints, auto_reset=False)
        v = self.vec
        self.nx, self.nu, self.nd, self.num_params, self.dt, self.c = v.nx, v.nu, v.nd, v.num_params, v.dt, v.c
        self.N, self.Np = v.N, v.Np
        self.observation_space, self.action_space = v.observation_space, v.action_space
        self.start_day, self.growth_year, self.location, self.training = start_day, growth_year, location, training
        self.u_min, self.u_max, self.delta_u_max = v.u_min, v.u_max, v.delta_u_max
        self.terminated = False

    def _set_x(self, value):
        value = np.asarray(value, dtype=np.float64).reshape(L.NX)
        self.vec.x_T[:, 0] = self.vec.torch.as_tensor(value, dtype=self.vec.tdtype, device=self.vec.device)

    x = property(lambda self: self.vec.x[0].double().cpu().numpy(), _set_x)
    weather_data = property(lambda self: self.vec.weather_data, lambda self, table: setattr(self.vec, "weather_data", table))
    u = property(lambda self: self.vec.u[0].double().cpu().numpy())
    p = property(lambda self: self.vec.p, lambda self, value: setattr(self.vec, "p", value))
    timestep = property(lambda self: int(self.vec.timestep_t[0]))
    day_of_year = property(lambda self: self.start_day + self.timestep * ((self.dt / self.c) % 365))
    hour_of_day = property(lambda self: float(self.vec.hour_of_day()[0]))

    def reset(self, seed: Optional[int] = None):
        obs = self.vec.reset_tensor(seed)
        self.terminated = False
        return obs[0].double().cpu().numpy(), {}

    def action_to_control(self, action):
        return np.clip(self.u + np.asarray(action) * self.delta_u_max, self.u_min, self.u_max)

    def _finish(self, out):
        obs_t, r_t, d_t, info_T = out
        info = {k: float(info_T[i, 0]) for i, k in enumerate(L.INFO_KEYS)}
        info["controls"] = self.u
        self.terminated = bool(d_t[0])
        return obs_t[0].double().cpu().numpy(), float(r_t[0]), self.terminated, False, info

    def step(self, action):
        t = self.vec.torch
        return self._finish(self.vec.step_tensor(t.as_tensor(np.asarray(action, dtype=np.float32).reshape(1, 6),
                                                             device=self.vec.device)))

    def step_raw_control(self, control):
        t = self.vec.torch
        return self._finish(self.vec.step_tensor(controls_t=t.as_tensor(np.asarray(control).reshape(1, 6),
                                                                        dtype=self.vec.tdtype, device=self.vec.device)))

    def step_raw_control_pipeinput(self, control):
        x, term = self.vec.step_raw_control_pipeinput(np.asarray(control).reshape(1, 6))
        self.terminated = bool(term[0])
        return x[0], self.terminated

    def set_crop_state(self, cBuf, cLeaf, cStem, cFruit, tCanSum):
        for i, v in zip((22, 23, 24, 25, 26), (cBuf, cLeaf, cStem, cFruit, tCanSum)):
            self.vec.x_T[i, 0] = v

    def get_state(self):
        return dict(self.vec.get_state(), terminated=self.terminated)

    def set_state(self, state):
        self.vec.set_state(state)
        self.terminated = bool(state.get("terminated", False))

    def get_obs_names(self):
        return self.vec.get_obs_names()

    def close(self):
        self.vec.close()
```

include/glgym.h:

```cpp
#ifndef GLGYM_H
#define GLGYM_H

#include <stddef.h>
#include <stdint.h>

#ifdef __cplusplus
extern "C" {
#endif

#define GLGYM_NX 28
#define GLGYM_NU 6
#define GLGYM_ND 10
#define GLGYM_NP 208
#define GLGYM_NCROP 34
#define GLGYM_NINFO 11
#define GLGYM_NMETRIC 14
#define GLGYM_METRIC_BDF 14
#define GLGYM_METRIC_REPLICAS 64
#define GLGYM_METRIC_STRIDE 32

typedef struct glgym_handle_s* glgym_handle;

typedef enum { GLGYM_F32 = 0, GLGYM_F64 = 1 } glgym_dtype;

typedef enum { GLGYM_ODE = 0, GLGYM_ODE_PIPE = 1 } glgym_variant;

typedef enum { GLGYM_SCHEME_RK4 = 0, GLGYM_SCHEME_RK2 = 1, GLGYM_SCHEME_RK3 = 2, GLGYM_SCHEME_LS5 = 3 } glgym_scheme;

typedef enum { GLGYM_VERIFY_AUTO = 0, GLGYM_VERIFY_ALWAYS = 1, GLGYM_VERIFY_NEVER = 2 } glgym_verify;

typedef enum {
    GLGYM_OK = 0,
    GLGYM_EINVAL = -1,
    GLGYM_ENODEV = -2,
    GLGYM_EHIP = -3,
    GLGYM_ENOMEM = -4,
    GLGYM_EODE = -5
} glgym_status;

typedef struct {
    double elec_price, heating_price, co2_price, fruit_price, dmfm;
    double fixed_greenhouse_cost, fixed_co2_cost, fixed_lamp_cost, fixed_screen_cost;
    double pen_lamp;
    double co2_min, co2_max, temp_min, temp_max, rh_min, rh_max;
} glgym_reward_cfg;

#define GLGYM_ABI_VERSION 7

typedef struct {
    int32_t struct_size;
    int32_t B;
    int32_t ld;
    void* x;
    void* u;
    const float* action;
    const void* control;
    const void* weather;
    int32_t weather_rows;
    const int32_t* w_off;
    int32_t* timestep;
    const void* crop_p;
    int32_t N;
    void* reward;
    void* info;
    uint8_t* done;
    float* metrics;
    int32_t* step_flags;
} glgym_step_args;

#define GLGYM_SF_ACCEPT_AGREE_FLAGGED 32
#define GLGYM_SF_ACCEPT_LAST_ALONE 64
#define GLGYM_SF_FAILED 128
#define GLGYM_SF_BDF 2048

typedef struct {
    int32_t B, ld;
    const void* x;
    const void* u;
    const void* weather;
    int32_t weather_rows;
    const int32_t* w_off;
    const int32_t* timestep;
    const float* start_day;
    int32_t Np;
    float* obs;
    const uint8_t* mask;
    float* term_obs;
} glgym_obs_args;

typedef struct {
    int32_t B, ld;
    const uint8_t* mask;
    void* x;
    void* u;
    int32_t* timestep;
    const void* weather;
    int32_t weather_rows;
    int32_t* w_off;
    const int32_t* start_rows;
    const float* start_days;
    int32_t n_starts;
    float* start_day;
    int32_t* episode;
    uint64_t seed;
} glgym_reset_args;

const char* glgym_version(void);
int glgym_abi_version(void);
const char* glgym_last_error(void);

int glgym_create(int nx, int nu, int nd, int np, double dt, const double* p, int dtype, int n_sub, int device,
                 glgym_handle* out);
int glgym_destroy(glgym_handle h);
int glgym_set_params(glgym_handle h, const double* p);
int glgym_set_params_keep_reward_scale(glgym_handle h, const double* p);
int glgym_set_n_sub(glgym_handle h, int n_sub);
int glgym_set_scheme(glgym_handle h, int scheme);
int glgym_set_window(glgym_handle h, int window);
typedef enum { GLGYM_LAYOUT_AUTO = 0, GLGYM_LAYOUT_ONE = 1, GLGYM_LAYOUT_QUAD = 2 } glgym_layout;
int glgym_set_layout(glgym_handle h, int layout);
int glgym_set_occupancy(glgym_handle h, int waves_per_simd);
int glgym_set_ladder_parallel(glgym_handle h, int on);
int glgym_set_verify(glgym_handle h, int mode);
int glgym_set_control_limits(glgym_handle h, const double* u_min , const double* u_max , double delta_u_max);
int glgym_set_model_variant(glgym_handle h, int variant);
int glgym_set_reward(glgym_handle h, const glgym_reward_cfg* cfg);
int glgym_get_reward_scale(glgym_handle h, double* max_profit, double* min_profit, double* fixed_costs);

int glgym_evalF(glgym_handle h, const double* x, const double* u, const double* d, const double* p, int p_rows,
                int B, double* x_next);
int glgym_rhs(glgym_handle h, const double* x, const double* u, const double* d, int B, double* dx);

typedef enum { GLGYM_INTEGRATOR_EXPLICIT = 0, GLGYM_INTEGRATOR_BDF = 1 } glgym_integrator;
int glgym_set_integrator(glgym_handle h, int integrator);
int glgym_set_step_integrator(glgym_handle h, int integrator);
int glgym_set_tolerances(glgym_handle h, double rtol, double atol, int max_steps);
#define GLGYM_NSOLVER_STAT 5
int glgym_get_solver_stats(glgym_handle h, int B, int32_t* stats);

enum { GLGYM_OBS_INDOOR = 0,
       GLGYM_OBS_CROP = 1,
       GLGYM_OBS_CONTROL = 2,
       GLGYM_OBS_WEATHER = 3,
       GLGYM_OBS_TIME = 4,
       GLGYM_OBS_FORECAST = 5    };
int glgym_set_obs_modules(glgym_handle h, const int32_t* modules, int n);
int glgym_obs_dim(glgym_handle h, int Np);

int glgym_step(glgym_handle h, const glgym_step_args* a, void* stream);
int glgym_obs(glgym_handle h, const glgym_obs_args* a, void* stream);
int glgym_reset(glgym_handle h, const glgym_reset_args* a, void* stream);
int glgym_crop_noise(glgym_handle h, void* crop_p, int B, int ld, double scale, uint64_t seed, uint64_t draw_index,
                     void* stream);

int glgym_rng_crop_noise(glgym_handle h, void* crop_p, int B, int ld, double scale, uint64_t* rng_state, void* stream);
int glgym_rng_reset_draw(glgym_handle h, int B, int ld, const unsigned char* mask, uint64_t* rng_state, int n_years, int n_days,
                         const int32_t* start_rows, const float* start_days, int32_t* w_off, float* start_day, void* stream);

typedef struct {
    int32_t struct_size;
    int32_t n_children;
    int32_t n_parents;
    int32_t K;
    int32_t ld_parent, ld_child;
    const int32_t* parent;
    const void* x_parent;
    const void* u_parent;
    const int32_t* timestep_parent;
    const int32_t* w_off_parent;
    const float* start_day_parent;
    const void* crop_parent;
    void* x;
    void* u;
    int32_t* timestep;
    int32_t* w_off;
    float* start_day;
    void* crop;
    double* ret;
    double* viol;
    int32_t* n_steps;
    uint8_t* alive;
    uint8_t* failed;
} glgym_plan_fork_args;

typedef struct {
    int32_t struct_size;
    int32_t B, ld;
    double w;
    const void* reward;
    const void* info;
    const uint8_t* done;
    const int32_t* step_flags;
    double* ret;
    double* viol;
    int32_t* n_steps;
    uint8_t* alive;
    uint8_t* failed;
} glgym_plan_accumulate_args;

typedef struct {
    int32_t struct_size;
    int32_t H;
    double gamma;
    glgym_step_args step;
    const float* actions;
    const void* controls;
    double* ret;
    double* viol;
    int32_t* n_steps;
    uint8_t* alive;
    uint8_t* failed;
} glgym_plan_rollout_args;

typedef struct {
    int32_t struct_size;
    int32_t P, K, H;
    const double* ret;
    const uint8_t* failed;
    const float* actions;
    int32_t* best_k;
    double* best_ret;
    float* best_action;
    float* best_sequence;
    double temperature;
    float* mean_sequence;
} glgym_plan_select_args;

int glgym_plan_fork(glgym_handle h, const glgym_plan_fork_args* a, void* stream);
int glgym_plan_accumulate(glgym_handle h, const glgym_plan_accumulate_args* a, void* stream);
int glgym_plan_rollout(glgym_handle h, const glgym_plan_rollout_args* a, void* stream);
int glgym_plan_select(glgym_handle h, const glgym_plan_select_args* a, void* stream);

typedef struct {
    double lamps_on, lamps_off, lamps_day_start, lamps_day_stop, lamps_off_sun, lamp_rad_sum_limit;
    double temp_setpoint_day, temp_setpoint_night, heat_correction, heat_deadzone, co2_day;
    double vent_heat_Pband, rh_max, mech_dehumid_Pband, vent_rh_Pband, t_vent_off, vent_cold_Pband;
    double thScrSpDay, thScrSpNight, thScrPband, thScrDeadZone, thScrRh, thScrRhPband, lampExtraHeat;
    double blScrExtraRh, rhMax, tHeatBand, co2Band, useBlScr;
} glgym_rule_cfg;

typedef struct {
    int32_t B, ld;
    const void* x;
    const void* weather;
    int32_t weather_rows;
    const int32_t* w_off;
    const int32_t* timestep;
    const float* start_day;
    const double* hour;
    const double* doy;
    void* control;
} glgym_rule_args;

int glgym_rule_based(glgym_handle h, const glgym_rule_cfg* cfg, const glgym_rule_args* a, void* stream);

typedef struct {
    int32_t B, dim;
    const float* obs;
    float* obs_out;
    const void* reward;
    float* reward_out;
    const uint8_t* done;
    double* obs_mean;
    double* obs_var;
    double* obs_count;
    double* ret_stats;
    double* returns;
    double* workspace;
    double gamma, epsilon;
    float clip_obs, clip_reward;
    int32_t training, norm_obs, norm_reward;
} glgym_vecnorm_args;

int glgym_vecnorm(glgym_handle h, const glgym_vecnorm_args* a, void* stream);

typedef struct {
    int32_t n_raw;
    const double* time;
    const double* i_glob;
    const double* t_out;
    const double* rh;
    const double* wind;
    const double* t_sky;
    double co2_ppm;
    int32_t n_out;
    int32_t nd;
    void* out;
    double* workspace;
} glgym_weather_args;

int glgym_weather(glgym_handle h, const glgym_weather_args* a, void* stream);

int glgym_timer_start(glgym_handle h, void* stream);
int glgym_timer_stop(glgym_handle h, void* stream, float* elapsed_ms);

#ifdef __cplusplus
}
#endif
#endif
```

Before: 100.3 million.

## Fuse observation construction into the step kernel epilogue

Adds an observation epilogue to the fp32 step kernel. It computes the core observation features from registers (the new state and controls) and stages rows in shared memory, including forecast weather, then writes them with vectorized nontemporal stores. A new glgym_step_obs entry point and Python-side token logic skip the separate obs kernel launch when step and obs arguments match. This removes one kernel launch and a re-read of state, controls and weather per step, at the cost of more LDS use and more work in the step kernel, which could hurt occupancy.

```diff
diff --git a/greenlight-gym2_amd/csrc/glgym.hip b/greenlight-gym2_amd/csrc/glgym.hip
--- a/greenlight-gym2_amd/csrc/glgym.hip
+++ b/greenlight-gym2_amd/csrc/glgym.hip
@@ -76,6 +76,45 @@
     return v;
 }
 
+constexpr int OBS_NCORE = 23;
+__device__ __forceinline__ float obs_core_feature(int j, float prim, float aux, float sday, int ts, double doy_inc, double hod_inc)
+{
+#pragma clang fp contract(off)
+    const float kPpm = (float)(8.3144598 / (101325.0 * 44.01e-3));
+    const int k = ts > 0 ? ts - 1 : 0;
+    const float sat = 610.78f * __builtin_amdgcn_exp2f(1.44269504f * 17.2694f * aux * __builtin_amdgcn_rcpf(aux + 238.3f));
+    const float rh = fminf(fmaxf(100.0f * prim * __builtin_amdgcn_rcpf(sat), 0.0f), 100.0f);
+    const float ppm = kPpm * (aux + 273.15f) * prim;
+    const int c = j - 18;
+    const double rev = (c <= 2) ? __builtin_fma((double)ts, doy_inc, (double)sday) * (1.0 / 365.0)
+                                : (double)ts * hod_inc * (1.0 / 24.0);
+    const float fr = (float)(rev - floor(rev));
+    const float clk = (c == 1 || c == 3) ? __builtin_amdgcn_sinf(fr) : __builtin_amdgcn_cosf(fr);
+    float v = prim;
+    v = (j == 0 || j == 16) ? ppm : v;
+    v = (j == 2 || j == 15) ? rh : v;
+    v = (j == 18) ? (float)k : v;
+    v = (j > 18) ? clk : v;
+    return v;
+}
+__device__ __forceinline__ constexpr int obs_core_module(int j) { return j < 4 ? 0 : j < 7 ? 1 : j < 13 ? 2 : j < 18 ? 3 : 4; }
+__device__ __forceinline__ constexpr int obs_core_col(int j) { return j < 4 ? j : j < 7 ? j - 4 : j < 13 ? j - 7 : j < 18 ? j - 13 : j - 18; }
+
+#ifndef GL_OBS_ROWS
+#define GL_OBS_ROWS 16
+#endif
+constexpr int OBS_ROWS = GL_OBS_ROWS, OBS_MAX_NP = 128;
+struct StepObsArgs {
+    float* obs; const float* start_day;
+    double doy_inc, hod_inc;
+    int Np, dim, moff[6];
+};
+constexpr int STEP_OBS_MAX_DIM_OCC2 = WAVE * ((2 * NX + GL_N_SLOW) | 1) / OBS_ROWS, STEP_OBS_MAX_DIM_OCC1 = 512;
+struct StepNoObs {};
+constexpr int GL_SCH_OBS = 8;
+template <bool OBS> struct StepObsSel { using type = StepNoObs; };
+template <> struct StepObsSel<true> { using type = StepObsArgs; };
+
 #ifndef GL_STEP_WAVES_PER_SIMD
 #define GL_STEP_WAVES_PER_SIMD 1
 #endif
@@ -89,13 +128,17 @@
 constexpr int gl_order(int sch) { return sch == 0 ? 4 : sch == 1 ? 2 : sch == 2 ? 3 : 5; }
 template <class T, int SCH> struct SchemeWin { static constexpr int value = SCH == 0 ? RK4_WINDOW<T>::value : SCH == 1 ? 4 : SCH == 2 ? 3 : 2; };
 
-template <class T, bool PER_ENV_CROP, bool DEFAULT_P, bool PIPE = false, int SCH = 0, int OCC = GL_STEP_WAVES_PER_SIMD>
-__global__ __launch_bounds__(WAVE, OCC) void step_kernel(StepArgsT<T> a, ModelConst<T> m_arg, RewardConst<T> rw)
-{
+template <class T, bool PER_ENV_CROP, bool DEFAULT_P, bool PIPE = false, int SCHX = 0, int OCC = GL_STEP_WAVES_PER_SIMD>
+__global__ __launch_bounds__(WAVE, OCC) void step_kernel(StepArgsT<T> a, ModelConst<T> m_arg, RewardConst<T> rw,
+                                                         typename StepObsSel<(SCHX & GL_SCH_OBS) != 0>::type o)
+{
+    constexpr bool OBS = (SCHX & GL_SCH_OBS) != 0;
+    constexpr int SCH = SCHX & (GL_SCH_OBS - 1);
+    static_assert(!OBS || (sizeof(T) == 4 && !PIPE), "observation epilogue: fp32, default ODE");
     const ModelConst<T>& m = DEFAULT_P ? device_default<T>() : m_arg;
     constexpr bool WBUF = OCC == 2;
     constexpr int WSTRIDE = (2 * NX + GL_N_SLOW) | 1;
-    __shared__ float sh_w[WBUF ? WAVE * WSTRIDE : WAVE * NU];
+    alignas(16) __shared__ float sh_w[WBUF ? WAVE * WSTRIDE : WAVE * NU];
     float* sh_act = sh_w;
     const int lane = threadIdx.x;
     const int b0 = blockIdx.x * WAVE;
@@ -220,6 +263,76 @@
         for (int i = 0; i < GLGYM_NMETRIC; ++i) {
             const float sum = wave_sum(mv[i]);
             if (lane == 0) atomicAdd(mrep + i, sum);
+        }
+    }
+    if constexpr (OBS) {
+        typedef float v4f __attribute__((ext_vector_type(4)));
+        float* span;
+        if constexpr (WBUF) {
+            span = sh_w;
+        } else {
+            __shared__ float4 sh_obs4[OBS_ROWS * STEP_OBS_MAX_DIM_OCC1 / 4];
+            span = reinterpret_cast<float*>(sh_obs4);
+        }
+        const int dim = o.dim;
+        const int ts1 = ts + 1;
+        const int base = a.w_off[bb] + (ts1 > 0 ? ts1 - 1 : 0);
+        const int basec = base >= a.weather_rows ? a.weather_rows - 1 : (base < 0 ? 0 : base);
+        const T* wrow = a.weather + (size_t)basec * a.nd;
+        float wv[5];
+#pragma unroll
+        for (int j = 0; j < 5; ++j) wv[j] = wrow[j];
+        const float sday = o.start_day[bb];
+        const float uo[NU] = {uBoil, uCo2, a.u[(size_t)2 * a.ld + bb], a.u[(size_t)3 * a.ld + bb], uLamp, a.u[(size_t)5 * a.ld + bb]};
+        float f[OBS_NCORE];
+#pragma unroll
+        for (int j = 0; j < OBS_NCORE; ++j) {
+            const int xi = j == 0 ? 0 : j == 1 ? 2 : j == 2 ? 15 : j == 3 ? 9 : j == 4 ? 21 : j == 5 ? 25 : 26;
+            const float prim = j < 7 ? x1[xi] : (j < 13 ? uo[(j >= 7 && j < 13) ? j - 7 : 0] : wv[j < 18 ? j - 13 : 0]);
+            const float aux = j < 13 ? x1[2] : wv[1];
+            f[j] = obs_core_feature(j, prim, aux, sday, ts1, o.doy_inc, o.hod_inc);
+        }
+        const int n_live = min(WAVE, a.B - b0);
+        const int nf = o.moff[5] >= 0 ? 5 * o.Np : 0;
+        __syncthreads();
+        for (int s0 = 0; s0 < n_live; s0 += OBS_ROWS) {
+            const int nrows = min(OBS_ROWS, n_live - s0);
+            const int r_me = lane - s0;
+            if (r_me >= 0 && r_me < nrows) {
+#pragma unroll
+                for (int j = 0; j < OBS_NCORE; ++j) {
+                    const int mo = o.moff[obs_core_module(j)];
+                    if (mo >= 0) span[r_me * dim + mo + obs_core_col(j)] = f[j];
+                }
+            }
+            int base_r[OBS_ROWS];
+#pragma unroll
+            for (int r = 0; r < OBS_ROWS; ++r) base_r[r] = __builtin_amdgcn_readlane(base, s0 + r);
+            for (int q = lane; q < nf; q += WAVE) {
+                const int i = q / 5, c = q - i * 5;
+                float v[OBS_ROWS];
+#pragma unroll
+                for (int r = 0; r < OBS_ROWS; ++r) {
+                    int row = base_r[r] + 1 + i;
+                    row = row >= a.weather_rows ? a.weather_rows - 1 : (row < 0 ? 0 : row);
+                    v[r] = (float)a.weather[(size_t)row * a.nd + c];
+                }
+#pragma unroll
+                for (int r = 0; r < OBS_ROWS; ++r)
+                    if (r < nrows) span[r * dim + o.moff[5] + q] = v[r];
+            }
+            __syncthreads();
+            float* out = o.obs + (size_t)(b0 + s0) * dim;
+            if (nrows == OBS_ROWS) {
+                const int n4 = (OBS_ROWS * dim) >> 2;
+                const v4f* src4 = reinterpret_cast<const v4f*>(span);
+                v4f* dst4 = reinterpret_cast<v4f*>(out);
+                for (int e = lane; e < n4; e += WAVE) __builtin_nontemporal_store(src4[e], &dst4[e]);
+            } else {
+                for (int r = 0; r < nrows; ++r)
+                    for (int jj = lane; jj < dim; jj += WAVE) out[(size_t)r * dim + jj] = span[(size_t)r * dim + jj];
+            }
+            __syncthreads();
         }
     }
 }
@@ -591,10 +704,6 @@
     int moff[6], dim;
 };
 
-#ifndef GL_OBS_ROWS
-#define GL_OBS_ROWS 16
-#endif
-constexpr int OBS_ROWS = GL_OBS_ROWS, OBS_NCORE = 23, OBS_MAX_NP = 128;
 template <class T> __global__ __launch_bounds__(256) void obs_kernel(ObsArgsT<T> a)
 {
     constexpr int ROWS = OBS_ROWS, NCORE = OBS_NCORE;
@@ -602,7 +711,6 @@
     float* span = reinterpret_cast<float*>(span4);
     const int tid = threadIdx.x;
     const int dim = a.dim;
-    const float kPpm = (float)(8.3144598 / (101325.0 * 44.01e-3));
     for (int rb = blockIdx.x * ROWS; rb < a.B; rb += gridDim.x * ROWS) {
         const int nrows = min(ROWS, a.B - rb);
         if (a.mask) {
@@ -621,7 +729,6 @@
             const int r = e / NCORE, j = e - r * NCORE;
             const int b = rb + (r < nrows ? r : 0);
             const int ts = a.timestep[b];
-            const int k = ts > 0 ? ts - 1 : 0;
             int base = 0;
 #pragma unroll
             for (int rr = 0; rr < ROWS; ++rr) base = (rr == r) ? base_r[rr] : base;
@@ -632,19 +739,7 @@
                                 : (j < 13 ? a.u + (size_t)(j - 7) * a.ld + b : wrow + (j < 18 ? j - 13 : 0));
             const T* p2 = j < 13 ? a.x + (size_t)2 * a.ld + b : wrow + 1;
             const float prim = (float)*p1, aux = (float)*p2, sday = a.start_day[b];
-            const float sat = 610.78f * __builtin_amdgcn_exp2f(1.44269504f * 17.2694f * aux * __builtin_amdgcn_rcpf(aux + 238.3f));
-            const float rh = fminf(fmaxf(100.0f * prim * __builtin_amdgcn_rcpf(sat), 0.0f), 100.0f);
-            const float ppm = kPpm * (aux + 273.15f) * prim;
-            const int c = j - 18;
-            const double rev = (c <= 2) ? ((double)sday + (double)ts * a.doy_inc) * (1.0 / 365.0)
-                                        : (double)ts * a.hod_inc * (1.0 / 24.0);
-            const float fr = (float)(rev - floor(rev));
-            const float clk = (c == 1 || c == 3) ? __builtin_amdgcn_sinf(fr) : __builtin_amdgcn_cosf(fr);
-            float v = prim;
-            v = (j == 0 || j == 16) ? ppm : v;
-            v = (j == 2 || j == 15) ? rh : v;
-            v = (j == 18) ? (float)k : v;
-            v = (j > 18) ? clk : v;
+            const float v = obs_core_feature(j, prim, aux, sday, ts, a.doy_inc, a.hod_inc);
             const int mo = j < 4 ? a.moff[0] : j < 7 ? a.moff[1] : j < 13 ? a.moff[2] : j < 18 ? a.moff[3] : a.moff[4];
             const int jl = j < 4 ? j : j < 7 ? j - 4 : j < 13 ? j - 7 : j < 18 ? j - 13 : j - 18;
             if (r < nrows && mo >= 0) span[r * dim + mo + jl] = v;
@@ -1553,21 +1648,47 @@
 
 }
 
+static const int OBS_MODULE_SIZE[6] = {4, 3, 6, 5, 5, 0};
+static void obs_layout(glgym_handle h, int Np, int moff[6], int* dim)
+{
+    for (int m = 0; m < 6; ++m) moff[m] = -1;
+    *dim = 0;
+    for (int i = 0; i < h->n_obs_modules; ++i) {
+        const int m = h->obs_modules[i];
+        moff[m] = *dim;
+        *dim += m == GLGYM_OBS_FORECAST ? 5 * Np : OBS_MODULE_SIZE[m];
+    }
+}
+static void obs_clock_increments(glgym_handle h, double* doy_inc, double* hod_inc)
+{
+    *doy_inc = std::fmod(h->dt / 86400.0, 365.0);
+    *hod_inc = h->dt / 3600.0;
+}
 template <int SCH>
 static void launch_step_sch(const glgym_step_args* a, const StepArgsT<float>& k, const ModelConst<float>& m, const RewardConst<float>& rw,
-                            dim3 grid, dim3 block, hipStream_t st, bool def, bool occ2)
+                            dim3 grid, dim3 block, hipStream_t st, bool def, bool occ2, const StepObsArgs* o)
 {
     using T = float;
+    const StepNoObs no;
+    constexpr int SCHO = SCH | GL_SCH_OBS;
+    if (o) {
+        if (occ2) hipLaunchKernelGGL((step_kernel<T, false, true, false, SCHO, 2>), grid, block, 0, st, k, m, rw, *o);
+        else if (a->crop_p && def) hipLaunchKernelGGL((step_kernel<T, true, true, false, SCHO>), grid, block, 0, st, k, m, rw, *o);
+        else if (a->crop_p) hipLaunchKernelGGL((step_kernel<T, true, false, false, SCHO>), grid, block, 0, st, k, m, rw, *o);
+        else if (def) hipLaunchKernelGGL((step_kernel<T, false, true, false, SCHO>), grid, block, 0, st, k, m, rw, *o);
+        else hipLaunchKernelGGL((step_kernel<T, false, false, false, SCHO>), grid, block, 0, st, k, m, rw, *o);
+        return;
+    }
     if (occ2) {
-        hipLaunchKernelGGL((step_kernel<T, false, true, false, SCH, 2>), grid, block, 0, st, k, m, rw);
+        hipLaunchKernelGGL((step_kernel<T, false, true, false, SCH, 2>), grid, block, 0, st, k, m, rw, no);
         return;
     }
     if (a->crop_p) {
-        if (def) hipLaunchKernelGGL((step_kernel<T, true, true, false, SCH>), grid, block, 0, st, k, m, rw);
-        else hipLaunchKernelGGL((step_kernel<T, true, false, false, SCH>), grid, block, 0, st, k, m, rw);
+        if (def) hipLaunchKernelGGL((step_kernel<T, true, true, false, SCH>), grid, block, 0, st, k, m, rw, no);
+        else hipLaunchKernelGGL((step_kernel<T, true, false, false, SCH>), grid, block, 0, st, k, m, rw, no);
     } else {
-        if (def) hipLaunchKernelGGL((step_kernel<T, false, true, false, SCH>), grid, block, 0, st, k, m, rw);
-        else hipLaunchKernelGGL((step_kernel<T, false, false, false, SCH>), grid, block, 0, st, k, m, rw);
+        if (def) hipLaunchKernelGGL((step_kernel<T, false, true, false, SCH>), grid, block, 0, st, k, m, rw, no);
+        else hipLaunchKernelGGL((step_kernel<T, false, false, false, SCH>), grid, block, 0, st, k, m, rw, no);
     }
 }
 
@@ -1590,7 +1711,7 @@
 
 template <class T>
 static int launch_step(glgym_handle h, const glgym_step_args* a, const ModelConst<T>& m, const RewardConst<T>& rw,
-                       hipStream_t st)
+                       hipStream_t st, const glgym_obs_args* oa = nullptr, bool* fused = nullptr)
 {
     StepArgsT<T> k;
     k.B = a->B; k.ld = a->ld;
@@ -1632,16 +1753,27 @@
             return GLGYM_OK;
         }
         if (pipe) {
-            hipLaunchKernelGGL((step_kernel<T, false, false, true>), grid, block, 0, st, k, m, rw);
+            hipLaunchKernelGGL((step_kernel<T, false, false, true>), grid, block, 0, st, k, m, rw, StepNoObs{});
             HIPCHK(hipGetLastError());
             return GLGYM_OK;
         }
         const bool occ2 = def && !a->crop_p && (h->occupancy == 2 || (h->occupancy == 0 && (size_t)a->B >= (size_t)2 * WAVE * h->n_simd));
-        if (h->scheme == GLGYM_SCHEME_RK2) launch_step_sch<GLGYM_SCHEME_RK2>(a, k, m, rw, grid, block, st, def, occ2);
-        else if (h->scheme == GLGYM_SCHEME_RK3) launch_step_sch<GLGYM_SCHEME_RK3>(a, k, m, rw, grid, block, st, def, occ2);
-        else if (h->scheme == GLGYM_SCHEME_LS5) launch_step_sch<GLGYM_SCHEME_LS5>(a, k, m, rw, grid, block, st, def, occ2);
-        else launch_step_sch<GLGYM_SCHEME_RK4>(a, k, m, rw, grid, block, st, def, occ2);
+        StepObsArgs ob;
+        const StepObsArgs* o = nullptr;
+        if (oa && !oa->mask && oa->B == a->B && oa->ld == a->ld && oa->x == a->x && oa->u == a->u && oa->weather == a->weather &&
+            oa->weather_rows == a->weather_rows && oa->w_off == a->w_off && oa->timestep == a->timestep &&
+            ((uintptr_t)oa->obs & 15) == 0) {
+            ob.obs = oa->obs; ob.start_day = oa->start_day; ob.Np = oa->Np;
+            obs_clock_increments(h, &ob.doy_inc, &ob.hod_inc);
+            obs_layout(h, oa->Np, ob.moff, &ob.dim);
+            if (ob.dim > 0 && ob.dim <= (occ2 ? STEP_OBS_MAX_DIM_OCC2 : STEP_OBS_MAX_DIM_OCC1)) o = &ob;
+        }
+        if (h->scheme == GLGYM_SCHEME_RK2) launch_step_sch<GLGYM_SCHEME_RK2>(a, k, m, rw, grid, block, st, def, occ2, o);
+        else if (h->scheme == GLGYM_SCHEME_RK3) launch_step_sch<GLGYM_SCHEME_RK3>(a, k, m, rw, grid, block, st, def, occ2, o);
+        else if (h->scheme == GLGYM_SCHEME_LS5) launch_step_sch<GLGYM_SCHEME_LS5>(a, k, m, rw, grid, block, st, def, occ2, o);
+        else launch_step_sch<GLGYM_SCHEME_RK4>(a, k, m, rw, grid, block, st, def, occ2, o);
         HIPCHK(hipGetLastError());
+        if (o && fused) *fused = true;
         return GLGYM_OK;
     }
 }
@@ -1667,7 +1799,7 @@
     return GLGYM_OK;
 }
 
-extern "C" int glgym_step(glgym_handle h, const glgym_step_args* a, void* stream)
+static int step_impl(glgym_handle h, const glgym_step_args* a, void* stream, const glgym_obs_args* oa, bool* fused)
 {
     if (!h || !a) { g_err = "glgym_step: null handle / arguments"; return GLGYM_EINVAL; }
     if (a->struct_size != (int32_t)sizeof(glgym_step_args)) {
@@ -1691,28 +1823,26 @@
     }
     DeviceGuard dev_guard(h);
     hipStream_t st = (hipStream_t)stream;
-    return h->dtype == GLGYM_F32 ? launch_step<float>(h, a, h->mf, h->rf, st)
+    return h->dtype == GLGYM_F32 ? launch_step<float>(h, a, h->mf, h->rf, st, oa, fused)
                                  : launch_step<double>(h, a, h->md, h->rd, st);
 }
 
-static const int OBS_MODULE_SIZE[6] = {4, 3, 6, 5, 5, 0};
+extern "C" int glgym_step(glgym_handle h, const glgym_step_args* a, void* stream)
+{
+    return step_impl(h, a, stream, nullptr, nullptr);
+}
 
 template <class T> static int launch_obs(glgym_handle h, const glgym_obs_args* a, hipStream_t st)
 {
     ObsArgsT<T> k;
     k.B = a->B; k.ld = a->ld; k.x = (const T*)a->x; k.u = (const T*)a->u; k.weather = (const T*)a->weather;
     k.weather_rows = a->weather_rows; k.w_off = a->w_off; k.timestep = a->timestep; k.start_day = a->start_day;
-    k.Np = a->Np; k.obs = a->obs; k.mask = a->mask; k.term_obs = a->term_obs; k.doy_inc = std::fmod(h->dt / 86400.0, 365.0); k.hod_inc = h->dt / 3600.0; k.nd = h->nd;
+    k.Np = a->Np; k.obs = a->obs; k.mask = a->mask; k.term_obs = a->term_obs; k.nd = h->nd;
+    obs_clock_increments(h, &k.doy_inc, &k.hod_inc);
     int blocks = (a->B + OBS_ROWS - 1) / OBS_ROWS;
     static const int cap = [] { const char* e = std::getenv("GLGYM_OBS_BLOCKS"); return e ? std::atoi(e) : 4096; }();
     if (blocks > cap) blocks = cap;
-    for (int m = 0; m < 6; ++m) k.moff[m] = -1;
-    k.dim = 0;
-    for (int i = 0; i < h->n_obs_modules; ++i) {
-        const int m = h->obs_modules[i];
-        k.moff[m] = k.dim;
-        k.dim += m == GLGYM_OBS_FORECAST ? 5 * a->Np : OBS_MODULE_SIZE[m];
-    }
+    obs_layout(h, a->Np, k.moff, &k.dim);
     const size_t lds = (size_t)OBS_ROWS * k.dim * sizeof(float);
     hipLaunchKernelGGL((obs_kernel<T>), dim3(blocks), dim3(256), lds, st, k);
     HIPCHK(hipGetLastError());
@@ -1809,16 +1939,35 @@
 
 extern "C" {
 
+static bool obs_args_ok(glgym_handle h, const glgym_obs_args* a)
+{
+    return h && a && a->B >= 1 && a->ld >= a->B && a->x && a->u && a->weather && a->w_off && a->timestep && a->start_day && a->obs &&
+           a->Np >= 0 && a->Np <= OBS_MAX_NP;
+}
+
 int glgym_obs(glgym_handle h, const glgym_obs_args* a, void* stream)
 {
     DeviceGuard dev_guard(h);
-    if (!h || !a || a->B < 1 || a->ld < a->B || !a->x || !a->u || !a->weather || !a->w_off || !a->timestep ||
-        !a->start_day || !a->obs || a->Np < 0 || a->Np > OBS_MAX_NP) {
+    if (!obs_args_ok(h, a)) {
         g_err = "glgym_obs: bad arguments (null pointer, ld < B, or Np outside 0..128)";
         return GLGYM_EINVAL;
     }
     hipStream_t st = (hipStream_t)stream;
     return h->dtype == GLGYM_F32 ? launch_obs<float>(h, a, st) : launch_obs<double>(h, a, st);
+}
+
+int glgym_step_obs(glgym_handle h, const glgym_step_args* a, const glgym_obs_args* oa, void* stream)
+{
+    if (!h || !a || !oa) { g_err = "glgym_step_obs: null handle / arguments"; return GLGYM_EINVAL; }
+    if (oa->mask) { g_err = "glgym_step_obs: full-mode observations only (glgym_obs_args.mask must be NULL)"; return GLGYM_EINVAL; }
+    if (!obs_args_ok(h, oa)) {
+        g_err = "glgym_step_obs: bad observation arguments (null pointer, ld < B, or Np outside 0..128)";
+        return GLGYM_EINVAL;
+    }
+    bool fused = false;
+    const int rc = step_impl(h, a, stream, oa, &fused);
+    if (rc != GLGYM_OK || fused) return rc;
+    return glgym_obs(h, oa, stream);
 }
 
 int glgym_set_obs_modules(glgym_handle h, const int32_t* modules, int n)
diff --git a/greenlight-gym2_amd/gl_gym_amd/_lib.py b/greenlight-gym2_amd/gl_gym_amd/_lib.py
--- a/greenlight-gym2_amd/gl_gym_amd/_lib.py
+++ b/greenlight-gym2_amd/gl_gym_amd/_lib.py
@@ -196,6 +196,7 @@
     "glgym_set_step_integrator": (C.c_int, [C.c_void_p, C.c_int]),
     "glgym_step": (C.c_int, [C.c_void_p, C.POINTER(StepArgs), C.c_void_p]),
     "glgym_obs": (C.c_int, [C.c_void_p, C.POINTER(ObsArgs), C.c_void_p]),
+    "glgym_step_obs": (C.c_int, [C.c_void_p, C.POINTER(StepArgs), C.POINTER(ObsArgs), C.c_void_p]),
     "glgym_set_obs_modules": (C.c_int, [C.c_void_p, C.POINTER(C.c_int32), C.c_int]),
     "glgym_obs_dim": (C.c_int, [C.c_void_p, C.c_int]),
     "glgym_set_control_limits": (C.c_int, [C.c_void_p, _DP, _DP, C.c_double]),
diff --git a/greenlight-gym2_amd/gl_gym_amd/tomato_env.py b/greenlight-gym2_amd/gl_gym_amd/tomato_env.py
--- a/greenlight-gym2_amd/gl_gym_amd/tomato_env.py
+++ b/greenlight-gym2_amd/gl_gym_amd/tomato_env.py
@@ -138,6 +138,21 @@
 
     def __iter__(self):
         return (self[i] for i in range(len(self)))
+
+
+class _EpochLib:
+
+    def __init__(self, lib, env):
+        self.__dict__["_lib"], self.__dict__["_env"] = lib, env
+
+    def __getattr__(self, name):
+        fn, env = getattr(self._lib, name), self._env
+
+        def call(*args):
+            env._epoch += 1
+            return fn(*args)
+        self.__dict__[name] = call
+        return call
 
 
 class TomatoVecEnv:
@@ -160,7 +175,13 @@
         if not torch.cuda.is_available():
             raise L.GlgymError("TomatoVecEnv needs a HIP device (torch.cuda.is_available() is False); "
                                "there is no CPU fallback")
-        self._lib = L.load()
+        self._epoch = 0
+        self._obs_token = None
+        self._obs_followed = False
+        self._stepped = False
+        self.n_fused_steps = 0
+        self.n_obs_elided = 0
+        self._lib = _EpochLib(L.load(), self)
         self.torch = torch
         self.device = torch.device(device)
         torch.cuda.set_device(self.device)
@@ -361,20 +382,35 @@
                         len(self.start_rows), self.start_day_t.data_ptr(), self.episode_t.data_ptr(), self.seed_value)
         L.check(self._lib.glgym_reset(self._h, C.byref(a), self._stream()), "glgym_reset")
 
+    def _obs_args(self, out_t, mask_t=None, term_t=None):
+        return L.ObsArgs(self.B, self.ld, self.x_T.data_ptr(), self.u_T.data_ptr(), self.weather_t.data_ptr(),
+                         self.weather_rows, self.w_off_t.data_ptr(), self.timestep_t.data_ptr(),
+                         self.start_day_t.data_ptr(), self.Np, out_t.data_ptr(),
+                         mask_t.data_ptr() if mask_t is not None else None,
+                         term_t.data_ptr() if term_t is not None else None)
+
+    def _obs_deps(self):
+        return tuple((t.data_ptr(), t._version) for t in (self.x_T, self.u_T, self.timestep_t, self.w_off_t, self.start_day_t,
+                                                          self.weather_t, self.obs_t))
+
     def _launch_obs(self, out_t, mask_t=None, term_t=None):
-        a = L.ObsArgs(self.B, self.ld, self.x_T.data_ptr(), self.u_T.data_ptr(), self.weather_t.data_ptr(),
-                      self.weather_rows, self.w_off_t.data_ptr(), self.timestep_t.data_ptr(),
-                      self.start_day_t.data_ptr(), self.Np, out_t.data_ptr(),
-                      mask_t.data_ptr() if mask_t is not None else None,
-                      term_t.data_ptr() if term_t is not None else None)
-        L.check(self._lib.glgym_obs(self._h, C.byref(a), self._stream()), "glgym_obs")
-
-    def _launch_step(self, raw_control: bool):
+        if mask_t is None:
+            token, self._obs_token = self._obs_token, None
+            if out_t is self.obs_t:
+                self._obs_followed = self._stepped
+                if token is not None and token == (id(out_t), self._epoch, self._obs_deps()):
+                    self.n_obs_elided += 1
+                    return
+        L.check(self._lib.glgym_obs(self._h, C.byref(self._obs_args(out_t, mask_t, term_t)), self._stream()), "glgym_obs")
+
+    def _launch_step(self, raw_control: bool, want_obs: Optional[bool] = None):
         if self._env_at_create is not None and tuple(os.environ.get(k) for k in ("GLGYM_LAYOUT", "GLGYM_OCC", "GLGYM_VERIFY")) != self._env_at_create:
             import warnings
             warnings.warn("GLGYM_LAYOUT / GLGYM_OCC / GLGYM_VERIFY changed after this TomatoVecEnv was created: they are read once, at glgym_create, "
                           "and have no effect on an existing handle -- use set_layout() / set_occupancy() / set_verify()", RuntimeWarning, stacklevel=3)
             self._env_at_create = None
+        fuse = self._obs_followed if want_obs is None else bool(want_obs)
+        self._obs_followed, self._obs_token, self._stepped = False, None, True
         if self.rng == "numpy":
             if not getattr(self, "freeze_crop_noise", False):
                 L.check(self._lib.glgym_rng_crop_noise(self._h, self.crop_T.data_ptr() if self.crop_T is not None else None, self.B, self.ld,
@@ -392,7 +428,12 @@
                        self.crop_T.data_ptr() if self.crop_T is not None else None, self.N,
                        self.reward_t.data_ptr(), self.info_T.data_ptr(), self.done_t.data_ptr(),
                        self.metrics_t.data_ptr() if self.metrics_t is not None else None, self.step_flags_t.data_ptr())
-        L.check(self._lib.glgym_step(self._h, C.byref(a), self._stream()), "glgym_step")
+        if not fuse:
+            L.check(self._lib.glgym_step(self._h, C.byref(a), self._stream()), "glgym_step")
+            return
+        L.check(self._lib.glgym_step_obs(self._h, C.byref(a), C.byref(self._obs_args(self.obs_t)), self._stream()), "glgym_step_obs")
+        self.n_fused_steps += 1
+        self._obs_token = (id(self.obs_t), self._epoch, self._obs_deps())
 
     def reset_tensor(self, seed: Optional[int] = None):
         if seed is not None:
@@ -428,7 +469,7 @@
             self.ctrl_T[:, :self.B].copy_(controls_t.reshape(self.B, L.NU).t())
         else:
             self._launch_rule_based(controller)
-        self._launch_step(raw_control=actions_t is None)
+        self._launch_step(raw_control=actions_t is None, want_obs=want_obs)
         if want_obs:
             self._launch_obs(self.obs_t)
         if self.auto_reset:
@@ -563,6 +604,7 @@
             raise ValueError(f"weather_data has {table.shape[0]} rows, an episode needs {need}")
         self._weather_data = table
         self.weather_rows = int(table.shape[0])
+        self._epoch += 1
         self.weather_t = torch.as_tensor(table, dtype=self.tdtype, device=self.device).contiguous()
         self.start_rows = np.zeros(1, dtype=np.int64)
         self.start_days = np.asarray(self.start_days[:1], dtype=np.float32)
@@ -623,7 +665,7 @@
         def seq():
             self.action_t.copy_(static_a)
             self._action_src = self.action_t
-            self._launch_step(raw_control=False)
+            self._launch_step(raw_control=False, want_obs=want_obs)
             if want_obs:
                 self._launch_obs(self.obs_t)
             if self.auto_reset:
diff --git a/include/glgym.h b/include/glgym.h
--- a/include/glgym.h
+++ b/include/glgym.h
@@ -149,6 +149,7 @@
 
 int glgym_step(glgym_handle h, const glgym_step_args* a, void* stream);
 int glgym_obs(glgym_handle h, const glgym_obs_args* a, void* stream);
+int glgym_step_obs(glgym_handle h, const glgym_step_args* step, const glgym_obs_args* obs, void* stream);
 int glgym_reset(glgym_handle h, const glgym_reset_args* a, void* stream);
 int glgym_crop_noise(glgym_handle h, void* crop_p, int B, int ld, double scale, uint64_t seed, uint64_t draw_index,
                      void* stream);
```

Result: faster. 102.8 million (median of 6 runs) (+2.5%).
